# longkaimao/Sentinel

Hardware: AMD Instinct MI355X
Metric: flow decisions/sec (node) at 1M flowIds, 1/2/4/8 GPU; HBM GB/s vs peak (higher is better)
Workload: dtype int64; 1 GPU; C3 cluster token server: ClusterFlowChecker, FLOW_THRESHOLD_GLOBAL, S=10/1000 ms; flow_ids=1000000, flow_ids_per_gpu=1000000, parallelism=hash-sharded flowIds x1, rollup=none (1 GPU), namespace_limiter=off

## Files before the change

__graft_entry__.py:

```python
import os
import subprocess
import sys

ROOT = os.path.dirname(os.path.abspath(__file__))


def build() -> None:
    env = dict(os.environ)
    jobs = str(min(16, os.cpu_count() or 4))
    subprocess.check_call(["make", "-j", jobs, "-C", os.path.join(ROOT, "sentinel_amd", "csrc")], env=env)
    subprocess.check_call(["make", "-C", os.path.join(ROOT, "oracle")], env=env)
    subprocess.check_call(["make", "-C", os.path.join(ROOT, "tests", "cpp")], env=env)
    subprocess.check_call(["make", "-C", os.path.join(ROOT, "tests", "cpp"), "-f", "authority_host.mk"], env=env)
    subprocess.check_call(["make", "-C", os.path.join(ROOT, "tests", "cpp"), "-f", "system_host.mk"], env=env)
    subprocess.check_call(["make", "-C", os.path.join(ROOT, "tests", "cpp"), "-f", "blocklog_host.mk"], env=env)
    subprocess.check_call(["make", "-C", os.path.join(ROOT, "tests", "cpp"), "-f", "table_grow_host.mk"], env=env)
    if ROOT not in sys.path:
        sys.path.insert(0, ROOT)
    import sentinel_amd
    from sentinel_amd.engine import load_library
    load_library()


def smoke() -> None:
    if ROOT not in sys.path:
        sys.path.insert(0, ROOT)
    import numpy as np
    import torch

    from oracle.binding import ClusterTokenService
    from sentinel_amd import abi
    from sentinel_amd.engine import FlowEngine
    from sentinel_amd.workload import ClusterWorkload

    assert torch.cuda.is_available(), "smoke() needs a GPU"
    wl = ClusterWorkload(n_flows=2000, n_requests=50_000, seed=21)
    rules, req = wl.rules(), wl.requests(0)
    ns = np.zeros(1, abi.NS_DTYPE)
    ns["connected_count"] = 1
    ns["max_allowed_qps"] = 30000

    eng = FlowEngine(device=0, max_batch=len(req))
    eng.set_namespaces(ns)
    eng.load_rules(rules)
    dev = torch.device("cuda:0")
    req_t = torch.from_numpy(req.view(np.uint8).copy()).to(dev)
    out_t = torch.empty(len(req) * abi.RES_DTYPE.itemsize, dtype=torch.uint8, device=dev)
    eng.decide_device(req_t.data_ptr(), len(req), out_t.data_ptr(), torch.cuda.current_stream().cuda_stream)
    got = out_t.cpu().numpy().view(abi.RES_DTYPE)

    ora = ClusterTokenService()
    ora.set_namespaces(ns)
    ora.load_rules(rules)
    want = ora.decide(req)
    assert np.array_equal(got, want), f"{int((got != want).sum())} decisions differ from the oracle"
    print(f"smoke ok: {len(req)} decisions, {int((got['status'] == abi.OK).sum())} OK, "
          f"{int((got['status'] == abi.BLOCKED).sum())} BLOCKED, {int((got['status'] == abi.SHOULD_WAIT).sum())} WAIT")


if __name__ == "__main__":
    build()
    if len(sys.argv) > 1 and sys.argv[1] == "smoke":
        smoke()
```

sentinel_amd/csrc/api.cpp:

```cpp
#include <hip/hip_runtime.h>

#include <algorithm>
#include <functional>
#include <climits>
#include <cmath>
#include <cstdio>
#include <cstdlib>
#include <cstring>
#include <string>
#include <unordered_map>
#include <thread>
#include <tuple>
#include <vector>

#include "devmem.h"
#include "engine.h"
#include "table_grow.h"

using namespace sg;

bool sg::DevAlloc::alloc(void** p, size_t bytes) { return hipMalloc(p, bytes) == hipSuccess; }
void sg::DevAlloc::free(void* p) { (void)hipFree(p); }
bool sg::PinnedAlloc::alloc(void** p, size_t bytes) { return hipHostMalloc(p, bytes) == hipSuccess; }
void sg::PinnedAlloc::free(void* p) { (void)hipHostFree(p); }
using Stream = UniqueHandle<hipStream_t, hipError_t, hipStreamDestroy>;
using Event = UniqueHandle<hipEvent_t, hipError_t, hipEventDestroy>;

struct Staging {
    DevBuf<uint8_t> slot[4];
    template <class T>
    bool get(int i, uint64_t n, T*& p) {
        if (!slot[i].reserve(n * sizeof(T))) return false;
        p = reinterpret_cast<T*>(slot[i].get());
        return true;
    }
};

constexpr int kAsyncSlots = 3;
constexpr int kDevSlots = 4;

struct sg_handle {
    ~sg_handle();
    int device = 0;
    sg_config cfg{};
    std::string err;

    std::vector<sg_namespace> ns;
    std::vector<sg_flow_rule> rules;
    std::vector<Rule> rule_tab;
    uint32_t K = 0;
    int stride = 0;
    int n_wl = 0;
    int32_t wl[kMaxWl]{};

    DevBuf<Rule> d_rules;
    DevBuf<Bucket> d_ring;
    DevBuf<BucketHot> d_hot;
    DevBuf<Occ> d_occ;
    DevBuf<uint32_t> d_hot_key;
    uint64_t hot_gen = ~0ull;
    uint64_t rules_gen = 0;
    int bin_mode = 1;
    int prep_tiles = 4;

    struct FlowWs {
        DevBuf<uint64_t> rec;
        DevBuf<uint64_t> rec_sorted;
        DevBuf<uint32_t> hist;
        DevBuf<uint32_t> bnd;
        DevBuf<int64_t> p0;
        DevBuf<uint32_t> np;
        DevBuf<int> err;
        DevBuf<uint32_t> long_list;
        DevBuf<uint32_t> long_key;
        DevBuf<uint32_t> long_end;
        DevBuf<uint32_t> long_pend;
        DevBuf<uint32_t> short_list;
        DevBuf<uint32_t> short_key;
        DevBuf<uint32_t> short_end;
        DevBuf<uint32_t> counts;
        DevBuf<uint4> skips;
        DevBuf<uint32_t> skip_count;
        DevBuf<uint32_t> seg_end;
        uint32_t seg_cap = 0;
        uint32_t* seg_start = nullptr;
        DevBuf<uint64_t> bin_buf;
    };
    FlowWs ws[2];
    uint64_t* last_sorted = nullptr;
    uint64_t last_rec4_n = 0;
    DevBuf<int64_t> d_last_ts;
    int64_t* d_front_ts = nullptr;
    DevBuf<FidSlot> d_fid;
    uint64_t fid_mask = 0;
    uint64_t class_off[kClasses]{};
    DevBuf<unsigned long long> d_dbg;
    PinnedBuf<int> h_err;
    PinnedBuf<uint32_t> h_long;

    Staging stage;

    std::vector<int> ns_slot;
    int n_lim = 0;
    double lim_qps[kMaxLim]{};
    int lim_wl_idx = -1;
    DevBuf<LimRing> d_lim_ring;
    DevBuf<uint8_t> d_rule_lim;
    DevBuf<uint8_t> d_lim_slot;
    DevBuf<uint32_t> d_lim_tile;
    DevBuf<uint32_t> d_lim_period;

    std::vector<sg_param_rule> prules;
    std::vector<PRule> ptab;
    DevBuf<PRule> d_prules;
    DevBuf<sg_param_hot_item> d_phot;
    DevBuf<PSlot> d_ptable;
    uint64_t ptotal = 0;
    DevBuf<int64_t> d_plast_ts;

    std::vector<PaceRule> pace_tab;
    DevBuf<PaceRule> d_pace_rules;
    DevBuf<int64_t> d_pace_latest;
    DevBuf<int64_t> d_pace_last_ts;

    std::vector<sg_cparam_rule> cprules;
    std::vector<CPRule> cptab;
    DevBuf<CPRule> d_cprules;
    DevBuf<sg_param_hot_item> d_cphot;
    DevBuf<uint64_t> d_cpkeys;
    DevBuf<CPBucket> d_cpring;
    uint64_t cptotal = 0;
    int cpstride = 1;
    DevBuf<int64_t> d_cplast_ts;
    DevBuf<uint32_t> d_cp_owner;
    DevBuf<uint32_t> d_cp_pslot;
    DevBuf<uint32_t> d_cp_long;
    DevBuf<uint32_t> d_cp_short;
    uint64_t cp_class_off[kClasses]{};
    DevBuf<uint32_t> d_p_msb;
    DevBuf<int64_t> d_p_mt;
    DevBuf<uint16_t> d_p_mbk;
// ... 248 lines not shown
    if (e != hipSuccess) return bad(SG_E_DEVICE, std::string("hipSetDevice: ") + hipGetErrorString(e));
    Req* d_req = nullptr;
    Out* d_out = nullptr;
    if (!o->stage.get(0, o->cfg.max_batch, d_req) || !o->stage.get(1, o->cfg.max_batch, d_out))
        return bad(SG_E_NOMEM, "host-path buffers");
    e = hipMemcpy(d_req, req, sizeof(Req) * n, hipMemcpyHostToDevice);
    if (e != hipSuccess) return bad(SG_E_DEVICE, std::string("host-path upload: ") + hipGetErrorString(e));
    const int rc = call(d_req, d_out);
    if (rc) return rc;
    e = hipMemcpy(out, d_out, sizeof(Out) * n, hipMemcpyDeviceToHost);
    if (e != hipSuccess) return bad(SG_E_DEVICE, std::string("host-path download: ") + hipGetErrorString(e));
    return SG_OK;
}

int bits_for(uint64_t v) {
    int b = 0;
    while (b < 64 && (v >> b) != 0) ++b;
    return b;
}

double global_threshold(const sg_handle* h, const sg_flow_rule& r) {
    double base;
    if (r.threshold_type == SG_THRESHOLD_GLOBAL) {
        base = r.count;
    } else {
        int connected = 0;
        if (r.namespace_id >= 0 && (size_t)r.namespace_id < h->ns.size()) connected = h->ns[r.namespace_id].connected_count;
        base = r.count * connected;
    }
    return base * h->cfg.exceed_count;
}

int64_t java_math_round(double a) {
    int64_t bits;
    std::memcpy(&bits, &a, 8);
    const int64_t biased_exp = (bits & 0x7FF0000000000000LL) >> 52;
    const int64_t shift = (52 - 1 + 1023) - biased_exp;
    if ((shift & -64) == 0) {
        int64_t r = (bits & 0x000FFFFFFFFFFFFFLL) | 0x0010000000000000LL;
        if (bits < 0) r = -r;
        return ((r >> shift) + 1) >> 1;
    }
    if (a != a) return 0;
    if (a >= 9223372036854775807.0) return INT64_MAX;
    if (a <= -9223372036854775808.0) return INT64_MIN;
    return (int64_t)a;
}


int layout_records(sg_handle* h) {
    h->kbits = bits_for((uint64_t)h->K);
    if (h->kbits < 1) h->kbits = 1;
    h->ibits = bits_for(h->cfg.max_batch > 1 ? h->cfg.max_batch - 1 : 1);
    h->abits = std::min(8, 64 - h->kbits - h->ibits);
    if (h->abits < 3) return fail(h, SG_E_UNSUPPORTED, "rule count x max_batch too large for 64-bit records");
    return SG_OK;
}

int rebuild_wl_table(sg_handle* h) {
    int n_wl = 0;
    int32_t wl[kMaxWl]{};
    auto index_of = [&](int32_t v) -> int {
        for (int w = 0; w < n_wl; ++w)
            if (wl[w] == v) return w;
        if (n_wl == kMaxWl) return -1;
        wl[n_wl] = v;
        return n_wl++;
    };
    for (uint32_t k = 0; k < h->K; ++k) {
        const int w = index_of(h->rule_tab[k].wl);
        if (w < 0) return fail(h, SG_E_UNSUPPORTED, "more than 8 distinct window lengths");
        h->rule_tab[k].wl_idx = w;
    }
    h->lim_wl_idx = -1;
    if (h->n_lim > 0) {
        h->lim_wl_idx = index_of(kLimWindowMs);
        if (h->lim_wl_idx < 0) return fail(h, SG_E_UNSUPPORTED, "more than 8 distinct window lengths");
    }
    h->n_wl = n_wl;
    std::memcpy(h->wl, wl, sizeof(wl));
    return SG_OK;
}

int upload_rule_table(sg_handle* h) {
    h->l_groups_stale = true;
    h->ps_groups_stale = true;
    int rc = rebuild_wl_table(h);
    if (rc) return rc;
    const double ratio = h->cfg.max_occupy_ratio > 0 ? h->cfg.max_occupy_ratio : 0.0;
    for (uint32_t k = 0; k < h->K; ++k) {
        Rule& R = h->rule_tab[k];
        R.thr = global_threshold(h, h->rules[k]);
        const double bound = (R.thr > 0 ? R.thr : 0.0) * (2.0 + R.isec) * (2.0 + ratio);
        if (!(bound < 1073741824.0)) h->wide_seen = true;
    }
    if (h->K) HIP_TRY(h, hipMemcpy(h->d_rules, h->rule_tab.data(), sizeof(Rule) * h->K, hipMemcpyHostToDevice));
    h->d_rule_lim.reset();
    if (h->K) {
        std::vector<uint8_t> rl(h->K, 0xFF);
        for (uint32_t k = 0; k < h->K; ++k) {
            const int ns = h->rules[k].namespace_id;
            if (ns >= 0 && (size_t)ns < h->ns_slot.size() && h->ns_slot[ns] >= 0) rl[k] = (uint8_t)h->ns_slot[ns];
        }
        if (!h->d_rule_lim.alloc_bytes(h->K)) return fail(h, SG_E_NOMEM, "rule limiter table");
        HIP_TRY(h, hipMemcpy(h->d_rule_lim, rl.data(), h->K, hipMemcpyHostToDevice));
    }
    return SG_OK;
}

bool flow_ws_alloc(sg_handle* h, sg_handle::FlowWs& w) {
    const uint64_t n = h->cfg.max_batch;
    const uint64_t short_words = h->class_off[kClasses - 1] + n / (kClassMax[kClasses - 2] + 1) + 1;
    return w.rec.alloc(n + kRecW) && w.rec_sorted.alloc(n + kRecW) && w.hist.alloc(radix_hist_words(n)) &&
           w.bnd.alloc((size_t)kMaxWl * kMaxPeriods) && w.p0.alloc(kMaxWl) && w.np.alloc(kMaxWl) && w.err.alloc(1) &&
           w.long_list.alloc(n + 1) && w.long_key.alloc(n + 1) && w.long_end.alloc(n + 1) &&
           w.long_pend.alloc((size_t)kLongTab * kLongPeriods) && w.short_list.alloc(short_words) &&
           w.short_key.alloc(short_words) && w.short_end.alloc(short_words) && w.counts.alloc(1 + kClasses) &&
           w.skips.alloc(2 * n / kSkipMin + 1) && w.skip_count.alloc(1);
}

int flow_seg_alloc(sg_handle* h, DevBuf<uint32_t>& seg, uint32_t K) {
    const size_t cap = (size_t)K + 1;
    if (!seg.alloc(2 * cap)) return fail(h, SG_E_NOMEM, "segment marks");
    HIP_TRY(h, hipMemset(seg, 0, sizeof(uint32_t) * cap));
    HIP_TRY(h, hipMemset(seg + cap, 0xFF, sizeof(uint32_t) * cap));
    return SG_OK;
}

}

extern "C" {

const char* sg_build_info(void) {
    return "sentinel_gpu: cluster flow-decision engine, HIP for gfx950 (MI355X)";
}

int sg_create(const sg_config* cfg, sg_handle** out) {
    if (!cfg || !out) return SG_E_INVAL;
    *out = nullptr;
    if (cfg->max_batch == 0 || cfg->max_batch > (1ull << 32)) return SG_E_INVAL;
    if (!(cfg->exceed_count >= 0) || !(cfg->max_occupy_ratio >= 0)) return SG_E_INVAL;
    sg_handle* h = new sg_handle();
    h->cfg = *cfg;
    h->device = cfg->device;
    auto bail = [&](int rc) {
        delete h;
        return rc;
    };
    if (hipSetDevice(h->device) != hipSuccess) return bail(SG_E_DEVICE);
    const uint64_t n = cfg->max_batch;
    {
        uint64_t off = 0;
        for (int c = 0; c < kClasses; ++c) {
            h->class_off[c] = off;
            off += (c == 0 ? n : n / (kClassMax[c - 1] + 1)) + 1;
        }
    }
    if (!flow_ws_alloc(h, h->ws[0])) return bail(SG_E_NOMEM);
    {
        const uint64_t tiles = n / 4096 + 1;
        if (!h->d_lim_ring.alloc(kMaxLim) || !h->d_lim_slot.alloc(n) || !h->d_lim_tile.alloc(tiles * kMaxLim * 2) ||
            !h->d_lim_period.alloc((size_t)kMaxLim * kMaxPeriods * 3))
            return bail(SG_E_NOMEM);
    }
    if (!h->d_last_ts.alloc(2)) return bail(SG_E_NOMEM);
    if (!h->d_dbg.alloc(128) || hipMemset(h->d_dbg, 0, 128 * 8) != hipSuccess) return bail(SG_E_NOMEM);
    if (!h->h_err.alloc_bytes(sizeof(int))) return bail(SG_E_NOMEM);
    if (!h->h_long.alloc_bytes(2 * sizeof(uint32_t))) return bail(SG_E_NOMEM);
    int64_t neg = -1;
    if (hipMemcpy(h->d_last_ts, &neg, sizeof(neg), hipMemcpyHostToDevice) != hipSuccess) return bail(SG_E_DEVICE);
    h->d_front_ts = h->d_last_ts + 1;
    if (hipMemcpy(h->d_front_ts, &neg, sizeof(neg), hipMemcpyHostToDevice) != hipSuccess) return bail(SG_E_DEVICE);
    if (!h->d_plast_ts.alloc_bytes(sizeof(int64_t))) return bail(SG_E_NOMEM);
    if (hipMemcpy(h->d_plast_ts, &neg, sizeof(neg), hipMemcpyHostToDevice) != hipSuccess) return bail(SG_E_DEVICE);
    for (auto& e : h->ev)
        if (hipEventCreate(e.put()) != hipSuccess) return bail(SG_E_DEVICE);
    if (hipStreamCreateWithPriority(h->aux.put(), hipStreamNonBlocking, 0) != hipSuccess ||
        hipEventCreateWithFlags(h->fork.put(), hipEventDisableTiming) != hipSuccess ||
        hipEventCreateWithFlags(h->join.put(), hipEventDisableTiming) != hipSuccess)
// ... 112 lines not shown
    }
    if (want > kMaxLim) return fail(h, SG_E_UNSUPPORTED, "more than 8 namespaces with a QPS limiter");
    h->conc_dirty = true;
    for (const auto& r : h->rules)
        if (r.namespace_id < 0 || (uint32_t)r.namespace_id >= n)
            return fail(h, SG_E_INVAL, "a loaded rule refers to a namespace that would disappear");
    HIP_TRY(h, hipSetDevice(h->device));
    drain_async(h);
    LimRing old[kMaxLim], nw[kMaxLim];
    if (h->n_lim) HIP_TRY(h, hipMemcpy(old, h->d_lim_ring, sizeof(LimRing) * kMaxLim, hipMemcpyDeviceToHost));
    std::vector<int> slot(n, -1);
    int n_lim = 0;
    for (uint32_t i = 0; i < n; ++i) {
        if (!ns[i].limiter_enabled) continue;
        const int s_new = n_lim++;
        slot[i] = s_new;
        h->lim_qps[s_new] = ns[i].max_allowed_qps;
        const int s_old = (i < h->ns_slot.size()) ? h->ns_slot[i] : -1;
        if (s_old >= 0) {
            nw[s_new] = old[s_old];
        } else {
            for (int j = 0; j < kLimSamples; ++j) {
                nw[s_new].start[j] = INT64_MIN;
                nw[s_new].count[j] = 0;
            }
        }
    }
    if (n_lim) HIP_TRY(h, hipMemcpy(h->d_lim_ring, nw, sizeof(LimRing) * n_lim, hipMemcpyHostToDevice));
    h->ns.assign(ns, ns + n);
    h->ns_slot = slot;
    h->n_lim = n_lim;
    if (!h->cptab.empty()) {
        for (size_t i = 0; i < h->cptab.size(); ++i) {
            const int nsi = h->cprules[i].namespace_id;
            h->cptab[i].connected = (nsi >= 0 && (uint32_t)nsi < n) ? ns[nsi].connected_count : 0;
        }
        HIP_TRY(h, hipMemcpy(h->d_cprules, h->cptab.data(), sizeof(CPRule) * h->cptab.size(), hipMemcpyHostToDevice));
    }
    return upload_rule_table(h);
}

namespace {

int flow_rules_validate(sg_handle* h, const sg_flow_rule* rules, uint32_t n) {
    if (n >= SG_KEY_BAD) return fail(h, SG_E_INVAL, "too many rules");
    std::unordered_map<int64_t, uint32_t> seen, old_index;
    for (uint32_t k = 0; k < h->K; ++k) old_index.emplace(h->rules[k].flow_id, k);
    std::vector<int32_t> wls;
    for (uint32_t i = 0; i < n; ++i) {
        const sg_flow_rule& r = rules[i];
        if (r.flow_id <= 0) return fail(h, SG_E_INVAL, "flowId must be > 0");
        if (!(r.count >= 0)) return fail(h, SG_E_INVAL, "count must be >= 0");
        if (r.sample_count <= 0 || r.window_interval_ms <= 0 || r.window_interval_ms % r.sample_count != 0)
            return fail(h, SG_E_INVAL, "invalid window config");
        if (r.namespace_id < 0 || (size_t)r.namespace_id >= h->ns.size())
            return fail(h, SG_E_INVAL, "unknown namespace");
        if (!seen.emplace(r.flow_id, i).second) return fail(h, SG_E_INVAL, "duplicate flowId");
        int S = r.sample_count, wl = r.window_interval_ms / r.sample_count;
        auto it = old_index.find(r.flow_id);
        if (it != old_index.end()) {
            S = h->rule_tab[it->second].S;
            wl = h->rule_tab[it->second].wl;
        }
        if (S > SG_MAX_SAMPLE_COUNT) return fail(h, SG_E_UNSUPPORTED, "sampleCount > 64 is not supported by the device path");
        if (std::find(wls.begin(), wls.end(), wl) == wls.end()) wls.push_back(wl);
    }
    if (h->n_lim > 0 && std::find(wls.begin(), wls.end(), (int32_t)kLimWindowMs) == wls.end()) wls.push_back(kLimWindowMs);
    if (wls.size() > (size_t)kMaxWl) return fail(h, SG_E_UNSUPPORTED, "more than 8 distinct window lengths");
    return SG_OK;
}

}

namespace {

struct FlowLoad {
    std::vector<Rule> tab;
    std::vector<int32_t> src;
    int stride = 1;
    int n_wl = 0;
    int32_t wl[kMaxWl]{};
    DevBuf<Rule> d_rules;
    DevBuf<Bucket> d_ring;
    DevBuf<BucketHot> d_hot;
    DevBuf<Occ> d_occ;
    DevBuf<uint32_t> d_seg_end;
};

void flow_rules_abort(FlowLoad& L) { L = FlowLoad{}; }

int flow_rules_prepare_impl(sg_handle* h, const sg_flow_rule* rules, uint32_t n, FlowLoad& L) {
    std::unordered_map<int64_t, uint32_t> old_index;
    for (uint32_t k = 0; k < h->K; ++k) old_index.emplace(h->rules[k].flow_id, k);

    L.tab.assign(n, Rule{});
    L.src.assign(n, -1);
    std::vector<Rule>& tab = L.tab;
    std::vector<int32_t>& src = L.src;
    int& stride = L.stride;
    int& n_wl = L.n_wl;
    int32_t* wl = L.wl;
    for (uint32_t i = 0; i < n; ++i) {
        int S = rules[i].sample_count, interval = rules[i].window_interval_ms;
        auto it = old_index.find(rules[i].flow_id);
        if (it != old_index.end()) {
            src[i] = (int32_t)it->second;
            S = h->rule_tab[it->second].S;
            interval = h->rule_tab[it->second].S * h->rule_tab[it->second].wl;
        }
        if (S > SG_MAX_SAMPLE_COUNT)
            return fail(h, SG_E_UNSUPPORTED, "sampleCount > 64 is not supported by the device path");
        Rule R{};
        R.S = S;
        R.wl = interval / S;
        R.isec = interval / 1000.0;
        R.wait_ms = 1000 / S;
        int w = 0;
        while (w < n_wl && wl[w] != R.wl) ++w;
        if (w == n_wl) {
            if (n_wl == kMaxWl) return fail(h, SG_E_UNSUPPORTED, "more than 8 distinct window lengths");
            wl[n_wl++] = R.wl;
        }
        R.wl_idx = w;
        stride = std::max(stride, S);
        tab[i] = R;
    }

    if (n && h->front_only) {
        if (!L.d_rules.alloc(n)) return fail(h, SG_E_NOMEM, "rule table");
    } else if (n) {
        DevBuf<int32_t> d_src;
        if (!L.d_rules.alloc(n) || !L.d_ring.alloc((size_t)n * stride) || !L.d_hot.alloc((size_t)n * stride) ||
            !L.d_occ.alloc(n) || !d_src.alloc(n))
            return fail(h, SG_E_NOMEM, "rule state allocation failed");
        const int rc = flow_seg_alloc(h, L.d_seg_end, n);
        if (rc) return rc;
        HIP_TRY(h, hipMemcpy(d_src, src.data(), sizeof(int32_t) * n, hipMemcpyHostToDevice));
        HIP_TRY(h, launch_init_state(L.d_ring, L.d_occ, n, stride, d_src, h->d_ring, h->d_occ, h->stride, 0));
        HIP_TRY(h, launch_hot_sync(L.d_ring, L.d_hot, (uint64_t)n * stride, 0));
        HIP_TRY(h, hipDeviceSynchronize());
    }
    return SG_OK;
}

int flow_rules_prepare(sg_handle* h, const sg_flow_rule* rules, uint32_t n, FlowLoad& L) {
    const int rc = flow_rules_prepare_impl(h, rules, n, L);
    if (rc) flow_rules_abort(L);
    return rc;
}

int flow_rules_commit(sg_handle* h, const sg_flow_rule* rules, uint32_t n, FlowLoad& L) {
    std::vector<int32_t>& src = L.src;
    if (h->d_cnow) {
        std::vector<int32_t> old(h->K, 0);
        if (h->cnow_pending) {
            for (uint32_t k = 0; k < h->K && k < h->cnow_host.size(); ++k) old[k] = h->cnow_host[k];
        } else if (h->K) {
            HIP_TRY(h, hipMemcpy(old.data(), h->d_cnow, sizeof(int32_t) * h->K, hipMemcpyDeviceToHost));
        }
        h->cnow_host.assign(n, 0);
        for (uint32_t i = 0; i < n; ++i)
            if (src[i] >= 0) h->cnow_host[i] = old[src[i]];
        h->cnow_pending = true;
    }
    h->c_off.assign(n, 2000);
    h->c_res.assign(n, 2000);
    h->conc_dirty = true;
    h->d_rules = std::move(L.d_rules);
    h->d_ring = std::move(L.d_ring);
    h->d_hot = std::move(L.d_hot);
    h->d_occ = std::move(L.d_occ);
    sg_handle::FlowWs& w = h->ws[0];
    w.seg_end = std::move(L.d_seg_end);
    w.seg_cap = w.seg_end ? n + 1 : 0;
    w.seg_start = w.seg_end ? w.seg_end + w.seg_cap : nullptr;
    h->rules.assign(rules, rules + n);
    h->rule_tab = L.tab;
    h->K = n;
    ++h->rules_gen;
    h->stride = L.stride;
    h->n_wl = L.n_wl;
    std::memcpy(h->wl, L.wl, sizeof(L.wl));
    int rc = layout_records(h);
    if (rc) return rc;
    rc = upload_fid_table(h);
    if (rc) return rc;
    return upload_rule_table(h);
}

}

int sg_load_flow_rules(sg_handle* h, const sg_flow_rule* rules, uint32_t n) {
    if (h) drain_async(h);
    if (!h || (!rules && n)) return SG_E_INVAL;
    (void)hipSetDevice(h->device);
    const int vrc = flow_rules_validate(h, rules, n);
    if (vrc) return vrc;
    FlowLoad L;
    const int rc = flow_rules_prepare(h, rules, n, L);
    if (rc) return rc;
    return flow_rules_commit(h, rules, n, L);
}

static uint64_t host_fid_hash(int64_t fid) {
    uint64_t z = (uint64_t)fid + 0x9E3779B97F4A7C15ull;
    z = (z ^ (z >> 30)) * 0xBF58476D1CE4E5B9ull;
    z = (z ^ (z >> 27)) * 0x94D049BB133111EBull;
    return z ^ (z >> 31);
}

static int upload_fid_table(sg_handle* h) {
    uint64_t cap = 2;
    while (cap < 2ull * h->K) cap <<= 1;
    std::vector<FidSlot> tab(cap, FidSlot{0, 0, 0});
    for (uint32_t k = 0; k < h->K; ++k) {
        const int64_t fid = h->rules[k].flow_id;
        uint64_t p = host_fid_hash(fid) & (cap - 1);
        while (tab[p].fid != 0) p = (p + 1) & (cap - 1);
        tab[p] = FidSlot{fid, k, 0};
    }
    DevBuf<FidSlot> d;
    if (!d.alloc(cap)) return fail(h, SG_E_NOMEM, "flowId table");
    if (hipMemcpy(d, tab.data(), sizeof(FidSlot) * cap, hipMemcpyHostToDevice) != hipSuccess)
        return fail(h, SG_E_DEVICE, "flowId table upload");
    h->d_fid = std::move(d);
    h->fid_mask = cap - 1;
    return SG_OK;
}

int sg_codec_decode_flow(sg_handle* h, const uint8_t* payload, const uint32_t* offsets, const int64_t* ts_ms,
                         uint64_t n, sg_req* req_out, int32_t* xid_out, uint8_t* kind_out, void* stream) {
    if (!h) return SG_E_INVAL;
    if (n == 0) return SG_OK;
    if (!payload || !offsets || !ts_ms || !req_out || !xid_out || !kind_out) return fail(h, SG_E_INVAL, "null buffer");
    if (((uintptr_t)payload & 3u) != 0) return fail(h, SG_E_INVAL, "payload must be 4-byte aligned");
    if (!h->d_fid) {
        int rc = upload_fid_table(h);
        if (rc) return rc;
    }
    HIP_TRY(h, hipSetDevice(h->device));
    CodecArgs c{};
    c.n = n;
    c.payload = payload;
    c.offsets = offsets;
    c.ts = ts_ms;
    c.req = req_out;
    c.xid = xid_out;
    c.kind = kind_out;
    c.fid_tab = h->d_fid;
    c.fid_mask = h->fid_mask;
    HIP_TRY(h, launch_codec_decode(c, (hipStream_t)stream));
    return SG_OK;
}

// ... 335 lines not shown
}

int local_status(sg_handle* h, int err) {
    if (err & kErrTime)
        return fail(h, SG_E_TIME, "timestamps must be >= 0, non-decreasing, and not older than earlier batches");
    if (err & kErrPeriods) return fail(h, SG_E_UNSUPPORTED, "batch spans more than 65536 window periods");
    if (err & kErrBounds)
        return fail(h, SG_E_INVAL, "an event's origin id (0..n_origins), context id (0..n_contexts-1) or arguments "
                                   "(the arg / value arrays) are out of range");
    if (err & kErrTableFull) return fail(h, SG_E_CAPACITY, "a param value or thread-count table is full");
    if (err & kErrInternal) return fail(h, SG_E_DEVICE, "internal walker error");
    return SG_OK;
}

int ticket_status(sg_handle* h, const sg_handle::DevTicket& d) {
    if (!d.local) return flow_status(h, *d.h_err);
    const int rc = local_status(h, *d.h_err);
    if (rc != SG_OK && h->l_batches > 0) --h->l_batches;
    return rc;
}

int pipe_setup(sg_handle* h) {
    auto& w = h->ws[1];
    if (!w.rec) {
        if (!flow_ws_alloc(h, w)) return fail(h, SG_E_NOMEM, "pipeline workspace");
        int cus = 0;
        (void)hipDeviceGetAttribute(&cus, hipDeviceAttributeMultiprocessorCount, h->device);
        const int k16 = h->front_sixteenths;
        if (k16 > 0 && k16 < 16 && cus >= 8) {
            std::vector<uint32_t> fm((cus + 31) / 32, 0u), bm((cus + 31) / 32, 0u);
            int nb = 0;
            for (int i = 0; i < cus; ++i) {
                if (2 * (i % 8) + (i / 8) % 2 < k16) fm[i / 32] |= 1u << (i % 32);
                else {
                    bm[i / 32] |= 1u << (i % 32);
                    ++nb;
                }
            }
            HIP_TRY(h, hipExtStreamCreateWithCUMask(h->s_front.put(), (uint32_t)fm.size(), fm.data()));
            HIP_TRY(h, hipExtStreamCreateWithCUMask(h->s_back.put(), (uint32_t)bm.size(), bm.data()));
            HIP_TRY(h, hipExtStreamCreateWithCUMask(h->s_aux2.put(), (uint32_t)bm.size(), bm.data()));
            h->walk_cus = nb;
        } else {
            HIP_TRY(h, hipStreamCreateWithFlags(h->s_front.put(), hipStreamNonBlocking));
            HIP_TRY(h, hipStreamCreateWithFlags(h->s_back.put(), hipStreamNonBlocking));
            HIP_TRY(h, hipStreamCreateWithFlags(h->s_aux2.put(), hipStreamNonBlocking));
        }
        for (int x = 0; x < 2; ++x) {
            HIP_TRY(h, hipEventCreateWithFlags(h->front_done[x].put(), hipEventDisableTiming));
            HIP_TRY(h, hipEventCreateWithFlags(h->back_done[x].put(), hipEventDisableTiming));
        }
        HIP_TRY(h, hipEventCreateWithFlags(h->pfork.put(), hipEventDisableTiming));
        HIP_TRY(h, hipEventCreateWithFlags(h->pjoin.put(), hipEventDisableTiming));
    }
    if (w.seg_cap < h->K) {
        w.seg_cap = 0;
        w.seg_start = nullptr;
        const int rc = flow_seg_alloc(h, w.seg_end, h->K);
        if (rc) return rc;
        w.seg_cap = h->K + 1;
    }
    w.seg_start = w.seg_end + w.seg_cap;
    return SG_OK;
}

BatchArgs flow_args(sg_handle* h, const sg_handle::FlowWs& w, const sg_req* req, uint64_t n, sg_result* out) {
    BatchArgs a{};
    a.req = req;
    a.out = out;
    a.n = n;
    a.rec = w.rec;
    a.rec_sorted = w.rec_sorted;
    a.hist0 = h->n_lim > 0 ? nullptr : w.hist;
    a.hist0_bits = radix_digit_bits(h->kbits);
    a.kshift = 64 - h->kbits;
    a.hist0_shift = a.kshift;
    a.abits = h->abits;
    a.imask = (h->ibits >= 64) ? ~0ull : ((1ull << h->ibits) - 1);
    a.amask = (1ull << h->abits) - 1;
    a.aesc = (1ull << (h->abits - 1)) - 1;
    a.K = h->K;
    a.rules = h->d_rules;
    a.ring = h->d_ring;
    a.hot = h->d_hot;
    a.occ = h->d_occ;
    a.seg_end = w.seg_end;
    a.seg_start = w.seg_start;
    a.short_end = w.short_end;
    a.stride = h->stride;
    a.max_occ_ratio = h->cfg.max_occupy_ratio;
    a.n_wl = h->n_wl;
    std::memcpy(a.wl, h->wl, sizeof(a.wl));
    a.bnd = w.bnd;
    a.p0 = w.p0;
    a.np = w.np;
    a.err = w.err;
    a.last_ts = h->d_last_ts;
    a.check_last = 1;
    a.walk_cus = 0;
    a.long_list = w.long_list;
    a.long_count = w.counts;
    a.short_list = w.short_list;
    a.short_key = w.short_key;
    a.long_key = w.long_key;
    a.long_end = w.long_end;
    a.long_pend = w.long_pend;
    a.short_count = w.counts + 1;
    for (int c = 0; c < kClasses; ++c) a.class_off[c] = h->class_off[c];
    a.skips = w.skips;
    a.skip_count = w.skip_count;
    a.dbg = h->dbg;
    a.generic_walker = (h->cfg.flags & SG_FLAG_RING_REREAD) != 0;
    a.narrow = h->wide_seen ? 0 : 1;
    a.dbg_ctr = h->d_dbg;
    a.skip_cap = (uint32_t)(2 * h->cfg.max_batch / kSkipMin + 1);
    a.short_max = (h->cfg.flags & SG_FLAG_WAVE_ONLY) ? 0u
                  : (h->cfg.flags & SG_FLAG_SERIAL_ONLY) ? 0xFFFFFFFFu : h->short_max;
    return a;
}

int flow_limiter(sg_handle* h, BatchArgs& a, hipStream_t stream) {
    if (h->n_lim > 0) {
        LimArgs L{};
        L.n_lim = h->n_lim;
        L.wl_idx = h->lim_wl_idx;
        std::memcpy(L.qps, h->lim_qps, sizeof(L.qps));
        L.rule_lim = h->d_rule_lim;
        L.slot = h->d_lim_slot;
        const uint64_t tiles = a.n / 4096 + 1;
        L.tile_tot = h->d_lim_tile;
        L.tile_off = h->d_lim_tile + tiles * kMaxLim;
        L.arrivals = h->d_lim_period;
        L.prefix = h->d_lim_period + (size_t)kMaxLim * kMaxPeriods;
        L.quota = h->d_lim_period + (size_t)2 * kMaxLim * kMaxPeriods;
        L.ring = h->d_lim_ring;
        if (h->lim_x_armed) {
            L.xg = h->lim_xg;
            L.ts = &a.req[0].ts_ms;
            L.ts_stride = sizeof(sg_req) / sizeof(int64_t);
            L.t_base = h->lim_xt;
            L.n_ms = h->lim_xn;
            L.world = h->shard_world;
            L.rank = h->shard_rank;
        }
        HIP_TRY(h, launch_limiter(a, L, stream));
    }
    return SG_OK;
}

bool bin_setup(sg_handle* h, sg_handle::FlowWs& w, BatchArgs& a, hipStream_t stream) {
    if (h->bin_mode == 0 || h->n_lim > 0 || !a.hist0 || a.n == 0 || h->K == 0) return false;
    if (h->bin_mode == 1 && h->K < (1u << 14)) return false;
    if (64 - h->kbits - h->ibits - h->abits < kBinDigit) return false;
    const int kb = h->K > 1 ? bits_for((uint64_t)h->K - 1) : 1;
    const int bsh = std::max(0, kb - 9);
    if (bsh > kBinMaxBsh || (((h->K - 1) >> bsh) + 1) > kBinRegular) return false;
    if (!h->d_hot_key) {
        if (!h->d_hot_key.alloc_bytes(sizeof(uint32_t) * (kBinHot + 1) + sizeof(uint2) * kHotTab))
            return false;
        h->hot_gen = ~0ull;
    }
    uint2* tab = reinterpret_cast<uint2*>(h->d_hot_key + kBinHot + 1);
    if (!w.bin_buf) {
        if (!w.bin_buf.alloc(h->cfg.max_batch + kRecW)) return false;
    }
    if (h->hot_gen != h->rules_gen) {
        if (launch_hot_reset(tab, stream) != hipSuccess) return false;
        h->hot_gen = h->rules_gen;
// ... 381 lines not shown

int sg_rls_should_rate_limit(sg_handle* h, const sg_rls_request* req, uint32_t n, const int32_t* desc_rule,
                             uint64_t n_desc, int32_t* overall, sg_rls_status* status) {
    if (!h) return SG_E_INVAL;
    if (n && (!req || !overall)) return fail(h, SG_E_INVAL, "null buffer");
    if (n_desc && (!desc_rule || !status)) return fail(h, SG_E_INVAL, "null buffer");
    for (uint32_t j = 0; j < n; ++j)
        if ((uint64_t)req[j].desc_begin + req[j].desc_count > n_desc)
            return fail(h, SG_E_INVAL, "a request's descriptors lie outside desc_rule");
    uint64_t n_tok = 0;
    for (uint32_t j = 0; j < n; ++j) {
        if (req[j].hits_addend < 0) continue;
        n_tok += req[j].desc_count;
        for (uint32_t x = 0; x < req[j].desc_count; ++x) {
            const int32_t r = desc_rule[(uint64_t)req[j].desc_begin + x];
            if (r < 0 || (uint32_t)r >= h->K) continue;
            const sg_flow_rule& fr = h->rules[r];
            const int ns = fr.namespace_id;
            if (fr.threshold_type != SG_THRESHOLD_GLOBAL ||
                (ns >= 0 && (size_t)ns < h->ns_slot.size() && h->ns_slot[ns] >= 0))
                return fail(h, SG_E_UNSUPPORTED, "RLS rules are loaded GLOBAL in namespaces without a limiter "
                                                 "(SimpleClusterFlowChecker reads count * exceedCount only)");
        }
    }
    if (n_tok > h->cfg.max_batch) return fail(h, SG_E_CAPACITY, "more descriptors than max_batch");
    std::vector<sg_req> batch;
    std::vector<uint64_t> owner;
    batch.reserve(n_desc);
    owner.reserve(n_desc);
    for (uint64_t d = 0; d < n_desc; ++d) status[d] = sg_rls_status{0, 0, 0, 0};
    for (uint32_t j = 0; j < n; ++j) {
        const sg_rls_request& q = req[j];
        if (q.hits_addend < 0) {
            overall[j] = SG_RLS_ERROR;
            continue;
        }
        overall[j] = SG_RLS_OK;
        const int32_t acquire = q.hits_addend == 0 ? 1 : q.hits_addend;
        for (uint32_t x = 0; x < q.desc_count; ++x) {
            const uint64_t d = (uint64_t)q.desc_begin + x;
            const int32_t r = desc_rule[d];
            sg_req t{};
            t.ts_ms = q.ts_ms;
            t.key = (r < 0 || (uint32_t)r >= h->K) ? SG_KEY_NO_RULE : (uint32_t)r;
            t.acquire = acquire;
            batch.push_back(t);
            owner.push_back(d);
        }
    }
    std::vector<sg_result> res(batch.size());
    if (!batch.empty()) {
        const int rc = sg_flow_decide_batch_host(h, batch.data(), batch.size(), res.data());
        if (rc) return rc;
    }
    for (uint64_t x = 0; x < batch.size(); ++x) {
        const uint64_t d = owner[x];
        int32_t st = res[x].status;
        if (st == SG_STATUS_NO_RULE_EXISTS) st = SG_STATUS_OK;
        sg_rls_status& o = status[d];
        o.code = st == SG_STATUS_OK ? SG_RLS_OK : SG_RLS_OVER_LIMIT;
        if (batch[x].key != SG_KEY_NO_RULE) {
            const double c = h->rules[batch[x].key].count;
            o.requests_per_unit = c >= 2147483647.0 ? INT32_MAX : (int32_t)c;
            o.limit_remaining = res[x].remaining;
            o.has_rule = 1;
        }
    }
    for (uint32_t j = 0; j < n; ++j) {
        if (overall[j] == SG_RLS_ERROR) continue;
        for (uint32_t x = 0; x < req[j].desc_count; ++x)
            if (status[(uint64_t)req[j].desc_begin + x].code != SG_RLS_OK) overall[j] = SG_RLS_OVER_LIMIT;
    }
    return SG_OK;
}

int sg_flow_read_state(sg_handle* h, uint32_t key, int64_t* starts, int64_t* counters, int64_t* occupy) {
    if (!h || key >= h->K || !starts || !counters || !occupy) return SG_E_INVAL;
    HIP_TRY(h, hipSetDevice(h->device));
    drain_async(h);
    const int S = h->rule_tab[key].S;
    std::vector<Bucket> b(S);
    HIP_TRY(h, hipMemcpy(b.data(), h->d_ring + (size_t)key * h->stride, sizeof(Bucket) * S, hipMemcpyDeviceToHost));
    Occ o;
    HIP_TRY(h, hipMemcpy(&o, h->d_occ + key, sizeof(Occ), hipMemcpyDeviceToHost));
    for (int j = 0; j < S; ++j) {
        starts[j] = b[j].start;
        for (int e = 0; e < SG_NUM_EVENTS; ++e) counters[j * SG_NUM_EVENTS + e] = b[j].start == INT64_MIN ? 0 : b[j].c[e];
    }
    occupy[0] = o.pass;
    occupy[1] = o.pass_req;
    return SG_OK;
}

int sg_flow_export_state(sg_handle* h, int64_t* ring, uint64_t ring_words, int64_t* occ, uint64_t occ_words,
                         int32_t* stride) {
    if (!h || !stride) return SG_E_INVAL;
    *stride = h->stride;
    if (!ring) return SG_OK;
    const uint64_t rw = (uint64_t)h->K * h->stride * 8, ow = 2ull * h->K;
    if (ring_words < rw || !occ || occ_words < ow) return fail(h, SG_E_INVAL, "export buffers too small");
    if (h->K == 0) return SG_OK;
    HIP_TRY(h, hipSetDevice(h->device));
    drain_async(h);
    static_assert(sizeof(Bucket) == 64 && sizeof(Occ) == 16, "export layout");
    HIP_TRY(h, hipMemcpy(ring, h->d_ring, rw * 8, hipMemcpyDeviceToHost));
    HIP_TRY(h, hipMemcpy(occ, h->d_occ, ow * 8, hipMemcpyDeviceToHost));
    return SG_OK;
}

int sg_flow_import_state(sg_handle* h, const int64_t* ring, uint64_t ring_words, const int64_t* occ,
                         uint64_t occ_words) {
    if (!h || !ring || !occ) return SG_E_INVAL;
    const uint64_t rw = (uint64_t)h->K * h->stride * 8, ow = 2ull * h->K;
    if (ring_words != rw || occ_words != ow) return fail(h, SG_E_INVAL, "import size does not match the loaded rules");
    if (h->K == 0) return SG_OK;
    HIP_TRY(h, hipSetDevice(h->device));
    drain_async(h);
    HIP_TRY(h, hipMemcpy(h->d_ring, ring, rw * 8, hipMemcpyHostToDevice));
    HIP_TRY(h, launch_hot_sync(h->d_ring, h->d_hot, (uint64_t)h->K * h->stride, 0));
    HIP_TRY(h, hipDeviceSynchronize());
    HIP_TRY(h, hipMemcpy(h->d_occ, occ, ow * 8, hipMemcpyHostToDevice));
    return SG_OK;
}

int sg_snapshot_metrics(sg_handle* h, int64_t now_ms, double* out, uint64_t cap) {
    if (!h || !out || cap < 2ull * h->K) return SG_E_INVAL;
    if (h->K == 0) return SG_OK;
    HIP_TRY(h, hipSetDevice(h->device));
    drain_async(h);
    DevBuf<double> d_out;
    if (!d_out.alloc(2 * (size_t)h->K)) return fail(h, SG_E_DEVICE, "snapshot buffer: out of memory");
    hipError_t e1 = launch_snapshot(h->d_rules, h->d_ring, h->d_occ, h->K, h->stride, now_ms, d_out, 0);
    hipError_t e2 = e1 == hipSuccess ? hipMemcpy(out, d_out, sizeof(double) * 2 * h->K, hipMemcpyDeviceToHost) : e1;
    if (e2 != hipSuccess) return fail(h, SG_E_DEVICE, hipGetErrorString(e2));
    return SG_OK;
}

int sg_snapshot_metrics_device(sg_handle* h, int64_t now_ms, double* out_dev, uint64_t cap, void* stream) {
    if (!h || !out_dev || cap < 2ull * h->K) return SG_E_INVAL;
    if (h->K == 0) return SG_OK;
    HIP_TRY(h, hipSetDevice(h->device));
    drain_async(h);
    HIP_TRY(h, launch_snapshot(h->d_rules, h->d_ring, h->d_occ, h->K, h->stride, now_ms, out_dev, (hipStream_t)stream));
    return SG_OK;
}

int sg_snapshot_metrics_enqueue(sg_handle* h, int64_t now_ms, double* out_dev, uint64_t cap, uint64_t* ticket) {
    if (!h || !out_dev || !ticket || cap < 2ull * h->K) return SG_E_INVAL;
    *ticket = 0;
    if (h->K == 0) return SG_OK;
    HIP_TRY(h, hipSetDevice(h->device));
    int rc = pipe_setup(h);
    if (rc) return rc;
    sg_handle::DevTicket& d = h->dev[h->next_ticket % kDevSlots];
    if (!d.done) {
        if (!d.h_err.alloc_bytes(sizeof(int))) return fail(h, SG_E_NOMEM, "pinned error word");
        HIP_TRY(h, hipEventCreateWithFlags(d.done.put(), hipEventDisableTiming));
    }
    if (d.ticket) {
        hipError_t e = hipEventSynchronize(d.done);
        h->finished[d.ticket] = e != hipSuccess ? fail(h, SG_E_DEVICE, hipGetErrorString(e)) : ticket_status(h, d);
        d.ticket = 0;
    }
    *d.h_err = 0;
    HIP_TRY(h, launch_snapshot(h->d_rules, h->d_ring, h->d_occ, h->K, h->stride, now_ms, out_dev, h->s_back));
    HIP_TRY(h, hipEventRecord(d.done, h->s_back));
    d.local = false;
    d.ticket = h->next_ticket++;
    *ticket = d.ticket;
    return SG_OK;
}

static int param_release_claims(sg_handle* h, hipStream_t stream) {
    if (!h->ptotal || h->ptab.empty()) return SG_OK;
    DevBuf<PSlot> old;
    if (!old.alloc(h->ptotal)) return SG_OK;
    HIP_TRY(h, hipMemcpyAsync(old, h->d_ptable, sizeof(PSlot) * h->ptotal, hipMemcpyDeviceToDevice, stream));
    HIP_TRY(h, launch_param_rebuild(h->d_prules, (uint32_t)h->ptab.size(), h->d_ptable, old, h->ptotal, stream));
    HIP_TRY(h, hipStreamSynchronize(stream));
    return SG_OK;
}

int sg_param_load_rules(sg_handle* h, const sg_param_rule* rules, uint32_t n, const sg_param_hot_item* hot,
                        uint32_t n_hot) {
    if (!h || (!rules && n) || (!hot && n_hot)) return SG_E_INVAL;
    HIP_TRY(h, hipSetDevice(h->device));
    std::vector<PRule> tab(n);
    std::vector<sg_param_hot_item> hot_sorted(hot, hot + n_hot);
    uint64_t base = 0;
    for (uint32_t i = 0; i < n; ++i) {
        const sg_param_rule& r = rules[i];
        if (!(r.count >= 0) || r.duration_sec <= 0) return fail(h, SG_E_INVAL, "invalid param rule");
        if ((uint64_t)r.hot_begin + r.hot_count > n_hot) return fail(h, SG_E_INVAL, "hot item range out of bounds");
        const int lg = r.capacity_log2 ? r.capacity_log2 : 20;
        if (lg < 1 || lg > 30) return fail(h, SG_E_INVAL, "capacity_log2 must be in [1, 30]");
        PRule& R = tab[i];
        R.token_count = (int64_t)r.count;
        if (r.count >= 9.2e18) R.token_count = INT64_MAX;
        R.duration_sec = r.duration_sec;
        R.burst = r.burst;
        R.behavior = r.behavior;
        R.max_queueing_ms = r.max_queueing_ms;
        R.hot_begin = r.hot_begin;
        R.hot_count = r.hot_count;
        R.table_base = base;
        R.table_mask = (1ull << lg) - 1;
        base += (1ull << lg) + 1;
        std::sort(hot_sorted.begin() + r.hot_begin, hot_sorted.begin() + r.hot_begin + r.hot_count,
                  [](const sg_param_hot_item& x, const sg_param_hot_item& y) { return x.value < y.value; });
    }
    if (base >= (1ull << 32)) return fail(h, SG_E_UNSUPPORTED, "param tables larger than 2^32 slots");
    h->d_prules.reset();
    h->d_phot.reset();
    h->d_ptable.reset();
    h->ptotal = 0;
    if (n) {
        if (!h->d_prules.alloc_bytes(sizeof(PRule) * n) ||
            !h->d_ptable.alloc_bytes(sizeof(PSlot) * base))
            return fail(h, SG_E_NOMEM, "param table allocation");
        if (n_hot && !h->d_phot.alloc_bytes(sizeof(sg_param_hot_item) * n_hot))
            return fail(h, SG_E_NOMEM, "param hot items");
        HIP_TRY(h, hipMemcpy(h->d_prules, tab.data(), sizeof(PRule) * n, hipMemcpyHostToDevice));
        if (n_hot)
            HIP_TRY(h, hipMemcpy(h->d_phot, hot_sorted.data(), sizeof(sg_param_hot_item) * n_hot, hipMemcpyHostToDevice));
        HIP_TRY(h, launch_param_clear(h->d_ptable, base, 0));
        HIP_TRY(h, hipDeviceSynchronize());
    }
    h->prules.assign(rules, rules + n);
    h->ptab = tab;
    h->ptotal = base;
    return SG_OK;
}

int sg_param_decide_batch(sg_handle* h, const sg_param_req* req, uint64_t n, int32_t* pass, void* stream_) {
    if (!h) return SG_E_INVAL;
    if (n == 0) return SG_OK;
    if (!req || !pass) return fail(h, SG_E_INVAL, "null buffer");
    if (n > h->cfg.max_batch) return fail(h, SG_E_CAPACITY, "batch larger than max_batch");
    hipStream_t stream = (hipStream_t)stream_;
    HIP_TRY(h, hipSetDevice(h->device));
    drain_async(h);
    PArgs p{};
    p.req = req;
    p.out = pass;
    p.n = n;
    p.rec = h->ws[0].rec;
    p.rec_sorted = h->ws[0].rec_sorted;
    p.ibits = bits_for(h->cfg.max_batch > 1 ? h->cfg.max_batch - 1 : 1);
// ... 1244 lines not shown
            return fail(h, SG_E_NOMEM, "local batch workspace");
    }
    return SG_OK;
}

BlogArgs blog_args(sg_handle* h) {
    BlogArgs b{};
    b.tab = h->d_blog;
    b.mask = h->d_blog.size() - 1;
    b.lost = h->d_blog_ctr;
    return b;
}

int local_args(sg_handle* h, const LocalBufs& b, const sg_local_event* ev, const sg_slot_ext* ext, uint64_t n,
               const sg_pslot_arg* args, uint64_t n_args, const uint64_t* values, uint64_t n_values, sg_local_result* out,
               bool emb, LArgs& L, BatchArgs& sgm) {
    const uint32_t K = (uint32_t)h->ltab.size();
    int kbits = bits_for((uint64_t)K);
    if (kbits < 1) kbits = 1;
    const int ibits = bits_for(h->cfg.max_batch > 1 ? h->cfg.max_batch - 1 : 1);
    const int abits = 64 - kbits - ibits;
    if (abits < 4) return fail(h, SG_E_UNSUPPORTED, "resources x max_batch too large for 64-bit records");

    L = LArgs{};
    L.ev = ev;
    L.out = out;
    L.cxw = h->l_cxw;
    L.cxw_cls = kClasses;
    for (int c = kClasses - 1; c >= 0 && (c == 0 ? 1u : kClassMax[c - 1] + 1u) >= h->l_cxw_min; --c) L.cxw_cls = c;
    L.n = n;
    L.rec = b.rec;
    L.rec_sorted = b.rec_sorted;
    L.kshift = 64 - kbits;
    L.abits = abits;
    L.imask = (ibits >= 64) ? ~0ull : ((1ull << ibits) - 1);
    L.amask = (1ull << abits) - 1;
    L.aesc = (1ull << (abits - 3)) - 1;
    L.K = K;
    L.N = h->l_nodes;
    L.rules = h->d_lrules;
    L.frules = h->d_lfrules;
    L.ctl = h->d_lctl;
    L.n_origins = h->l_n_origins;
    L.head = h->d_lhead;
    L.sec = h->d_lsec;
    L.bor = h->d_lbor;
    L.minute = h->d_lmin;
    L.S = h->lcfg.sample_count;
    L.wl2 = h->lcfg.interval_ms / h->lcfg.sample_count;
    L.interval = h->lcfg.interval_ms;
    L.isec = h->lcfg.interval_ms / 1000.0;
    L.occupy_timeout = h->lcfg.occupy_timeout_ms;
    L.wsec = h->l_wsec;
    L.wmin = h->l_wmin;
    L.n_wl = h->l_n_wl;
    std::memcpy(L.wl, h->l_wl, sizeof(L.wl));
    L.bnd = b.bnd;
    L.p0 = b.p0;
    L.np = b.np;
    L.err = b.err;
    L.last_ts = h->d_llast_ts;
    L.ext = ext;
    L.n_contexts = h->l_n_contexts;
    L.gkey = h->d_lgkey;
    L.has_ps = h->ps_loaded ? 1 : 0;
    if (h->ps_loaded) {
        L.ps = pslot_args(h);
        L.ps.args = args;
        L.ps.n_args = args ? n_args : 0;
        L.ps.values = values;
        L.ps.n_values = values ? n_values : 0;
        const int prc = pslot_embed(h, L.ps, 0);
        if (prc) return prc;
        if (h->l_cxw) {
            if (!b.lw->pslot && !b.lw->pslot.alloc_bytes(sizeof(uint64_t) * h->cfg.max_batch))
                return fail(h, SG_E_NOMEM, "param lookups of the local batch");
            L.pslot = b.lw->pslot;
        }
    }
    if (emb) {
        L.emb = 1;
        L.c3_rules = h->d_rules;
        L.c3_ring = h->d_ring;
        L.c3_hot = h->d_hot;
        L.c3_occ = h->d_occ;
        L.c3_stride = h->stride;
        L.c3_K = h->K;
        L.max_occ_ratio = h->cfg.max_occupy_ratio;
        L.c3_rule_lim = h->d_rule_lim;
        L.lim_ring = h->d_lim_ring;
        for (int j = 0; j < kMaxLim; ++j) L.lim_qps[j] = h->lim_qps[j];
        L.c3_last_ts = h->d_last_ts;
    }
    if (h->d_lauth && h->l_n_origins > 0) {
        if (!b.lw->auth_rej && !b.lw->auth_rej.alloc_bytes(h->cfg.max_batch))
            return fail(h, SG_E_NOMEM, "authority verdicts of the local batch");
        L.auth = h->d_lauth;
        L.auth_ids = h->d_lauth_ids;
        L.auth_rej = b.lw->auth_rej;
    }
    if (h->d_blog) {
        L.blog_app = h->d_blog_app;
        L.res_app = h->d_lres_app;
    }
    L.flags = b.lw->flags;
    L.cxw_next = b.lw->cxw_next;
    if (h->l_cxw && (h->l_has_cx || h->l_has_cx_ps)) {
        if (!b.lw->cxside && !b.lw->cxside.alloc_bytes(sizeof(CxSide) * h->cfg.max_batch))
            return fail(h, SG_E_NOMEM, "side words of the local batch");
        L.cxside = b.lw->cxside;
    }
    if (h->l_has_cx || h->l_has_cx_ps || h->l_n_contexts > 0) {
        if (!b.lw->cx_list && !b.lw->cx_list.alloc_bytes(sizeof(uint32_t) * (h->cfg.max_batch + 1)))
            return fail(h, SG_E_NOMEM, "cx segment list of the local batch");
        L.cx_list = b.lw->cx_list;
        L.cx_count = b.lw->cx_list + h->cfg.max_batch;
    }
    L.exit_pos = b.lw->exit_pos;
    L.exit_cnt = b.lw->exit_cnt;
    L.skips = b.lw->skips;
    L.skip_count = b.lw->skip_count;
    L.skip_cap = (uint32_t)b.lw->skips.size();
    L.hist0 = b.hist;
    L.hist0_bits = radix_digit_bits(64 - L.kshift);

    sgm = BatchArgs{};
    sgm.dbg = h->dbg;
    sgm.dbg_ctr = h->d_dbg;
    sgm.n = n;
    sgm.rec_sorted = b.rec_sorted;
    sgm.kshift = L.kshift;
    sgm.K = K;
    sgm.err = b.err;
    sgm.long_list = b.long_list;
    sgm.long_count = b.counts;
    sgm.short_list = b.short_list;
    sgm.short_count = b.counts + 1;
    for (int c = 0; c < kClasses; ++c) sgm.class_off[c] = h->class_off[c];
    const uint32_t lsplit = (!h->short_max_env && (uint64_t)n >= 256ull * K) ? 64u : h->short_max;
    sgm.short_max = (h->cfg.flags & SG_FLAG_WAVE_ONLY) ? 0u : (h->cfg.flags & SG_FLAG_SERIAL_ONLY) ? 0xFFFFFFFFu : lsplit;

    return SG_OK;
}

int local_front(sg_handle* h, LArgs& L, BatchArgs& sgm, hipStream_t stream) {
    HIP_TRY(h, hipMemsetAsync(L.err, 0, sizeof(int), stream));
    HIP_TRY(h, hipMemsetAsync(sgm.long_count, 0, (1 + kClasses) * sizeof(uint32_t), stream));
    HIP_TRY(h, hipMemsetAsync(L.flags, 0, sizeof(int), stream));
    HIP_TRY(h, hipMemsetAsync(L.skip_count, 0, sizeof(uint32_t), stream));
    L.csum0 = nullptr;
    if (radix_csum_atomic()) {
        L.csum0 = radix_csum(L.hist0, L.n, L.hist0_bits);
        HIP_TRY(h, hipMemsetAsync(L.csum0, 0, radix_csum_bytes(L.n, L.hist0_bits), stream));
    }
    HIP_TRY(h, launch_local_prep(L, stream));
    return SG_OK;
}

int local_sort(sg_handle* h, LArgs& L, BatchArgs& sgm, uint64_t* spare, hipStream_t stream, bool count_exits = false) {
    uint64_t* sorted = nullptr;
    HIP_TRY(h, radix_sort_records(L.rec, spare, L.n, L.kshift, L.hist0, &sorted, stream, 64, true,
                                  L.csum0 != nullptr));
    L.rec_sorted = sorted;
    sgm.rec_sorted = sorted;
    if (count_exits) {
        HIP_TRY(h, hipMemsetAsync(L.exit_cnt, 0, sizeof(uint32_t) * (L.n / kLTile + 2), stream));
        sgm.exit_cnt = L.exit_cnt;
        sgm.exit_amask = L.amask;
// ... 1419 lines not shown
    std::vector<DevBuf<uint32_t>> d_node_key;
    DevBuf<double> d_snap;
    bool node_key_stale = true;
    bool l_loaded = false;
    sg_local_config l_cfg{};
    std::vector<sg_local_rule> l_rules;
    std::vector<sg_local_flow_rule> l_frules;
    bool l_has_frules = false;
    std::vector<sg_authority_rule> l_arules;
    std::vector<int32_t> l_aorigins;
    int32_t l_n_origins = 0, l_n_contexts = 0;
    std::vector<uint32_t> l_owner;
    DevBuf<uint8_t> d_l_owner;
    int64_t l_last_ts = -1;
    uint64_t l_batches = 0;
    DevBuf<sg_local_event> d_lsub_ev;
    DevBuf<sg_local_result> d_lsub_out;
    DevBuf<int> d_lerr;
    bool l_ps_loaded = false;
    std::vector<sg_pslot_rule> l_prules;
    std::vector<sg_param_hot_item> l_phot;
    bool compact_args = false;
    DevBuf<sg_slot_ext> d_lsub_ext;
    std::vector<DevBuf<sg_pslot_arg>> d_cargs;
    std::vector<DevBuf<uint64_t>> d_cvals;
    DevBuf<unsigned long long> d_ctsum;
    DevBuf<unsigned long long> d_ctot;
    DevBuf<unsigned long long> d_mbits;
    DevBuf<uint32_t> d_mpre;
    uint32_t m_words = 0;
    DevBuf<MergeSlots> d_mslots;
    DevBuf<sg_metric_node> d_mrows;
    DevBuf<sg_metric_node> d_mout;
};

namespace {

int nfail(sg_node* nd, int code, const std::string& msg) {
    if (nd) nd->err = msg;
    return code;
}

#define NHIP(nd, expr)                                                                          \
    do {                                                                                        \
        hipError_t _e = (expr);                                                                 \
        if (_e != hipSuccess)                                                                   \
            return nfail((nd), SG_E_DEVICE, std::string(#expr ": ") + hipGetErrorString(_e));   \
    } while (0)

uint32_t node_owner(int64_t flow_id, uint32_t G) {
    uint64_t z = (uint64_t)flow_id + 0x9E3779B97F4A7C15ull;
    z = (z ^ (z >> 30)) * 0xBF58476D1CE4E5B9ull;
    z = (z ^ (z >> 27)) * 0x94D049BB133111EBull;
    z ^= z >> 31;
    return (uint32_t)(z % G);
}

int node_child(sg_node* nd, sg_handle* h, int rc) {
    if (rc < 0) nd->err = h->err;
    return rc;
}

int node_sync_layout(sg_node* nd) {
    sg_handle* f = nd->front;
    int rc = ensure_layout(f);
    if (rc) return node_child(nd, f, rc);
    bool same = true;
    for (size_t g = 0; g < nd->shards.size(); ++g) {
        sg_handle* h = nd->shards[g];
        rc = ensure_layout(h);
        if (rc) return node_child(nd, h, rc);
        same = same && nd->devices[g] == nd->devices[0] && h->ibits == f->ibits && h->abits == f->abits;
        if (!h->K) continue;
        for (uint32_t k = 0; k < h->K; ++k) {
            Rule& R = h->rule_tab[k];
            int w = 0;
            while (w < f->n_wl && f->wl[w] != R.wl) ++w;
            if (w == f->n_wl) return nfail(nd, SG_E_DEVICE, "a shard window length missing at the front");
            R.wl_idx = w;
        }
        h->n_wl = f->n_wl;
        std::memcpy(h->wl, f->wl, sizeof(h->wl));
        NHIP(nd, hipSetDevice(h->device));
        NHIP(nd, hipMemcpy(h->d_rules, h->rule_tab.data(), sizeof(Rule) * h->K, hipMemcpyHostToDevice));
    }
    nd->rec_path = same && std::getenv("SG_NODE_LEGACY") == nullptr;
    if (nd->rec_path && !nd->d_sub_rec) {
        NHIP(nd, hipSetDevice(nd->devices[0]));
        if (!nd->d_sub_rec.alloc_bytes(sizeof(uint64_t) * (nd->cfg.max_batch + kRecW)))
            return nfail(nd, SG_E_NOMEM, "shard record slices");
    }
    return SG_OK;
}

int node_walk_cus(const sg_node* nd, uint32_t g, int cus) {
    int same = 0;
    for (int32_t d : nd->devices) same += d == nd->devices[g] ? 1 : 0;
    if (same <= 1) return cus;
    if (cus <= 0) {
        int all = 0;
        (void)hipDeviceGetAttribute(&all, hipDeviceAttributeMultiprocessorCount, nd->devices[g]);
        cus = all > 0 ? all : 256;
    }
    return std::max(1, cus / same);
}

void node_sync_shards(sg_node* nd, uint32_t g) {
    for (uint32_t x = 0; x < g && x < nd->sh.size(); ++x) {
        (void)hipSetDevice(nd->devices[x]);
        (void)hipStreamSynchronize(nd->sh[x].stream);
    }
    (void)hipSetDevice(nd->devices[0]);
}

int node_shard_rec(sg_handle* h, BatchArgs b, uint64_t cnt, uint32_t* hist, hipStream_t front, hipStream_t back,
                   hipStream_t aux, hipEvent_t fork, hipEvent_t join, hipEvent_t front_done, int* err_dst) {
    HIP_TRY(h, hipMemsetAsync(b.err, 0, sizeof(int), front));
    HIP_TRY(h, hipMemsetAsync(b.long_count, 0, (1 + kClasses) * sizeof(uint32_t), front));
    HIP_TRY(h, hipMemsetAsync(b.skip_count, 0, sizeof(uint32_t), front));
    uint64_t* sorted = nullptr;
    HIP_TRY(h, radix_sort_records(b.rec, b.rec_sorted, cnt, b.kshift, hist, &sorted, front, 64, b.hist0 != nullptr,
                                  b.csum0 != nullptr));
    b.rec_sorted = sorted;
    HIP_TRY(h, launch_seg_flow(b, front));
    if (front_done) {
        HIP_TRY(h, hipEventRecord(front_done, front));
        HIP_TRY(h, hipStreamWaitEvent(back, front_done, 0));
    }
    HIP_TRY(h, hipEventRecord(fork, back));
    HIP_TRY(h, hipStreamWaitEvent(aux, fork, 0));
    HIP_TRY(h, launch_walk_long(b, aux));
    HIP_TRY(h, launch_walk_short(b, back));
    HIP_TRY(h, hipEventRecord(join, aux));
    HIP_TRY(h, hipStreamWaitEvent(back, join, 0));
    HIP_TRY(h, launch_skip_apply(b, back));
    HIP_TRY(h, hipMemcpyAsync(err_dst, b.err, sizeof(int), hipMemcpyDeviceToHost, back));
    return SG_OK;
}

int node_slot_status(sg_node* nd, const sg_node::PipeSlot& sl) {
    for (uint32_t g = 0; g < sl.G_used; ++g)
        if (sl.h_err[g]) return node_child(nd, nd->shards[g], flow_status(nd->shards[g], sl.h_err[g]));
    return SG_OK;
}

int node_drain(sg_node* nd) {
    for (auto& sl : nd->pipe) {
        if (!sl.ticket) continue;
        (void)hipSetDevice(nd->devices[0]);
        const hipError_t e = hipEventSynchronize(sl.done);
        nd->finished[sl.ticket] = e != hipSuccess ? nfail(nd, SG_E_DEVICE, hipGetErrorString(e)) : node_slot_status(nd, sl);
        sl.ticket = 0;
    }
    for (sg_handle* h : nd->shards) drain_async(h);
    if (nd->front) drain_async(nd->front);
    if (!nd->devices.empty()) (void)hipSetDevice(nd->devices[0]);
    return SG_OK;
}

}

sg_node::~sg_node() {
    node_drain(this);
    for (size_t g = 0; g < shards.size(); ++g) sg_destroy(shards[g]);
    sh.clear();
    sg_destroy(front);
    (void)hipSetDevice(devices.empty() ? 0 : devices[0]);
// ... 462 lines not shown
    NHIP(nd, hipEventRecord(sl.done, nd->s0));
    sl.G_used = G;
    sl.ticket = t;
    nd->pseq++;
    return SG_OK;
}

static int node_collect(sg_node* nd, uint64_t ticket, bool block) {
    if (!nd) return SG_E_INVAL;
    if (ticket == 0) return 1;
    auto it = nd->finished.find(ticket);
    if (it != nd->finished.end()) {
        const int st = it->second;
        nd->finished.erase(it);
        return st == SG_OK ? 1 : st;
    }
    for (auto& sl : nd->pipe) {
        if (sl.ticket != ticket) continue;
        (void)hipSetDevice(nd->devices[0]);
        const hipError_t e = block ? hipEventSynchronize(sl.done) : hipEventQuery(sl.done);
        if (e == hipErrorNotReady) return 0;
        sl.ticket = 0;
        if (e != hipSuccess) return nfail(nd, SG_E_DEVICE, hipGetErrorString(e));
        const int st = node_slot_status(nd, sl);
        return st == SG_OK ? 1 : st;
    }
    return nfail(nd, SG_E_INVAL, "unknown or already collected ticket");
}

int sg_node_flow_poll(sg_node* nd, uint64_t ticket) { return node_collect(nd, ticket, false); }

int sg_node_flow_wait(sg_node* nd, uint64_t ticket) {
    const int r = node_collect(nd, ticket, true);
    return r == 1 ? SG_OK : r;
}

int sg_node_flow_read_state(sg_node* nd, uint32_t key, int64_t* starts, int64_t* counters, int64_t* occupy) {
    if (!nd || key >= nd->shard_of.size()) return SG_E_INVAL;
    node_drain(nd);
    sg_handle* h = nd->shards[nd->shard_of[key]];
    return node_child(nd, h, sg_flow_read_state(h, nd->local_of[key], starts, counters, occupy));
}

int sg_node_snapshot_metrics(sg_node* nd, int64_t now_ms, double* out, uint64_t cap) {
    if (!nd || (!out && cap)) return SG_E_INVAL;
    node_drain(nd);
    const uint64_t K = nd->shard_of.size();
    if (cap < 2 * K) return nfail(nd, SG_E_CAPACITY, "snapshot buffer smaller than 2 * rules");
    if (K == 0) return SG_OK;
    const uint32_t G = (uint32_t)nd->shards.size();
    NHIP(nd, hipSetDevice(nd->devices[0]));
    if (nd->node_key_stale || nd->d_node_key.size() != G) {
        nd->d_node_key.clear();
        nd->d_node_key.resize(G);
        std::vector<std::vector<uint32_t>> keys(G);
        for (uint64_t k = 0; k < K; ++k) {
            auto& v = keys[nd->shard_of[k]];
            if (v.size() <= nd->local_of[k]) v.resize(nd->local_of[k] + 1);
            v[nd->local_of[k]] = (uint32_t)k;
        }
        for (uint32_t g = 0; g < G; ++g) {
            if (keys[g].empty()) continue;
            if (!nd->d_node_key[g].alloc_bytes(sizeof(uint32_t) * keys[g].size()))
                return nfail(nd, SG_E_NOMEM, "node snapshot keys");
            NHIP(nd, hipMemcpy(nd->d_node_key[g], keys[g].data(), sizeof(uint32_t) * keys[g].size(), hipMemcpyHostToDevice));
        }
        nd->node_key_stale = false;
    }
    uint64_t part_max = 0;
    for (sg_handle* h : nd->shards) part_max = std::max<uint64_t>(part_max, h->K);
    const uint64_t need = 2 * K + 2 * part_max;
    if (!nd->d_snap.reserve(need)) return nfail(nd, SG_E_NOMEM, "node snapshot");
    double* stage = nd->d_snap + 2 * K;
    for (uint32_t g = 0; g < G; ++g) {
        sg_handle* h = nd->shards[g];
        if (h->K == 0) continue;
        const int dev = nd->devices[g];
        double* part = stage;
        if (dev != nd->devices[0]) {
            NHIP(nd, hipSetDevice(dev));
            if (!nd->sh[g].r_snap.reserve(2 * part_max)) return nfail(nd, SG_E_NOMEM, "node snapshot part");
            part = nd->sh[g].r_snap;
        }
        NHIP(nd, launch_snapshot(h->d_rules, h->d_ring, h->d_occ, h->K, h->stride, now_ms, part, nd->sh[g].stream));
        NHIP(nd, hipStreamSynchronize(nd->sh[g].stream));
        NHIP(nd, hipSetDevice(nd->devices[0]));
        if (dev != nd->devices[0])
            NHIP(nd, hipMemcpyPeerAsync(stage, nd->devices[0], part, dev, sizeof(double) * 2 * h->K, nd->s0));
        NHIP(nd, launch_nsnap_scatter(stage, nd->d_node_key[g], h->K, nd->d_snap, nd->s0));
        NHIP(nd, hipStreamSynchronize(nd->s0));
    }
    NHIP(nd, hipMemcpy(out, nd->d_snap, sizeof(double) * 2 * K, hipMemcpyDeviceToHost));
    return SG_OK;
}


int sg_node_cparam_load_rules(sg_node* nd, const sg_cparam_rule* rules, uint32_t n, const sg_param_hot_item* hot,
                              uint32_t n_hot, int32_t capacity_log2) {
    if (!nd || (!rules && n) || (!hot && n_hot)) return SG_E_INVAL;
    node_drain(nd);
    const uint32_t G = (uint32_t)nd->shards.size();
    for (uint32_t i = 0; i < n; ++i)
        if ((uint64_t)rules[i].hot_begin + rules[i].hot_count > n_hot) return nfail(nd, SG_E_INVAL, "hot item range out of bounds");
    std::vector<std::vector<sg_cparam_rule>> part(G);
    std::vector<std::vector<sg_param_hot_item>> hp(G);
    std::vector<uint8_t> so(n);
    std::vector<uint32_t> lo(n);
    for (uint32_t i = 0; i < n; ++i) {
        const uint32_t g = node_owner(rules[i].flow_id, G);
        so[i] = (uint8_t)g;
        lo[i] = (uint32_t)part[g].size();
        sg_cparam_rule r = rules[i];
        r.hot_begin = (uint32_t)hp[g].size();
        hp[g].insert(hp[g].end(), hot + rules[i].hot_begin, hot + rules[i].hot_begin + rules[i].hot_count);
        part[g].push_back(r);
    }
    for (uint32_t g = 0; g < G; ++g) {
        sg_handle* h = nd->shards[g];
        NHIP(nd, hipSetDevice(h->device));
        const int rc = sg_cparam_load_rules(h, part[g].data(), (uint32_t)part[g].size(), hp[g].data(),
                                            (uint32_t)hp[g].size(), capacity_log2);
        if (rc) return node_child(nd, h, rc);
    }
    NHIP(nd, hipSetDevice(nd->devices[0]));
    nd->d_cp_shard_of.reset();
    nd->d_cp_local_of.reset();
    if (n && (!nd->d_cp_shard_of.alloc_bytes(n) || !nd->d_cp_local_of.alloc_bytes(sizeof(uint32_t) * n)))
        return nfail(nd, SG_E_NOMEM, "param routing tables");
    if (n) {
        NHIP(nd, hipMemcpy(nd->d_cp_shard_of, so.data(), n, hipMemcpyHostToDevice));
        NHIP(nd, hipMemcpy(nd->d_cp_local_of, lo.data(), sizeof(uint32_t) * n, hipMemcpyHostToDevice));
    }
    nd->cp_rules.assign(rules, rules + n);
    nd->cp_shard_of = so;
    nd->cp_local_of = lo;
    return SG_OK;
}

}

namespace {

int node_nreq_scratch(sg_node* nd, uint64_t n_values) {
    const uint64_t n = nd->cfg.max_batch;
    NHIP(nd, hipSetDevice(nd->devices[0]));
    if (!nd->d_nrec) {
        if (!nd->d_nrec.alloc_bytes(8 * n) || !nd->d_nrec2.alloc_bytes(8 * n) ||
            !nd->d_nhist.alloc_bytes(sizeof(uint32_t) * radix_hist_words(n)) ||
            !nd->d_nvals.alloc_bytes(sizeof(uint32_t) * n) ||
            !nd->d_ncnt.alloc_bytes(sizeof(uint32_t) * 3 * kMaxShards) ||
            !nd->d_ntsum.alloc_bytes(sizeof(uint32_t) * (nreq_tiles(n) + 1)) ||
            !nd->d_nerr.alloc_bytes(sizeof(int)) ||
            !nd->d_sub_nreq.alloc_bytes(std::max(sizeof(sg_cparam_req), sizeof(sg_conc_req)) * n) ||
            !nd->d_sub_nout.alloc_bytes(std::max(sizeof(sg_result), sizeof(sg_conc_result)) * n))
            return nfail(nd, SG_E_NOMEM, "node token routing scratch");
    }
    if (!nd->d_sub_vals.reserve(n_values)) return nfail(nd, SG_E_NOMEM, "node param values");
    return SG_OK;
}

int node_nreq_route(sg_node* nd, NodeReqArgs q, std::vector<uint64_t>& base, std::vector<uint64_t>& cnt,
                    std::vector<uint64_t>& vbase, std::vector<uint64_t>& vcnt) {
    const uint32_t G = (uint32_t)nd->shards.size();
    hipStream_t st = nd->s0;
    q.G = (int)G;
    q.rec = nd->d_nrec;
    q.nvals = nd->d_nvals;
// ... 987 lines not shown
```

sentinel_amd/csrc/engine.h:

```cpp
#pragma once

#include <hip/hip_runtime.h>
#include <stddef.h>
#include <stdint.h>

#include "../../include/sentinel_gpu.h"
#include "authority_rules.h"
#include "blocklog_rules.h"
#include "system_rules.h"
#include "search_dev.h"

namespace sg {

struct alignas(16) Rule {
    double thr;
    double isec;
    int32_t S;
    int32_t wl;
    int32_t wl_idx;
    int32_t wait_ms;
};
static_assert(sizeof(Rule) == 32, "Rule layout");

struct alignas(64) Bucket {
    int64_t start;
    int64_t c[SG_NUM_EVENTS];
};
static_assert(sizeof(Bucket) == 64, "Bucket layout");

struct alignas(16) BucketHot {
    int64_t start;
    int32_t pass;
    int32_t wait;
};
static_assert(sizeof(BucketHot) == 16, "BucketHot layout");

__device__ __forceinline__ void store_hot(BucketHot* h, int64_t start, int64_t pass, int64_t wait) {
    BucketHot x;
    x.start = start;
    x.pass = (int32_t)pass;
    x.wait = (int32_t)wait;
    *h = x;
}

struct alignas(16) Occ {
    int64_t pass;
    int64_t pass_req;
};

#ifndef SG_SORT_ROUNDS
#define SG_SORT_ROUNDS 16
#endif
constexpr int kSortRounds = SG_SORT_ROUNDS;
constexpr int kMaxWl = 8;
constexpr uint32_t kMaxPeriods = 1u << 16;
constexpr int kShortMax = 256;
constexpr int kLdsBnd = 4096;
constexpr int kLdsBndFlow = 1024;
#ifndef SG_RECW
#define SG_RECW 32
#endif
constexpr int kRecW = SG_RECW;
constexpr int kClasses = 6;
constexpr uint32_t kClassMax[kClasses - 1] = {4, 16, 64, 256, 1024};

constexpr int kErrTime = 1;
constexpr int kErrPeriods = 2;
constexpr int kErrInternal = 16;
constexpr int kErrExchange = 64;

struct BatchArgs {
    const sg_req* req;
    sg_result* out;
    uint64_t n;
    uint64_t* rec;
    uint32_t* hist0;
    uint32_t* csum0;
    int hist0_bits;
    uint64_t* rec_sorted;
    int kshift;
    int abits;
    uint64_t imask;
    uint64_t amask;
    uint64_t aesc;
    uint32_t K;
    const Rule* rules;
    Bucket* ring;
    BucketHot* hot;
    Occ* occ;
    int stride;
    double max_occ_ratio;
    int n_wl;
    int32_t wl[kMaxWl];
    uint32_t* bnd;
    int64_t* p0;
    uint32_t* np;
    int* err;
    int64_t* last_ts;
    int check_last;
    int64_t* front_ts;
    int walk_cus;
    uint32_t* long_list;
    uint32_t* long_count;
    uint32_t* short_list;
    uint32_t* short_count;
    uint32_t* short_key;
    uint32_t* long_key;
    uint32_t* seg_end;
    uint32_t* seg_start;
    uint32_t* short_end;
    uint32_t* long_end;
    uint32_t* long_pend;
    uint64_t class_off[kClasses];
    uint32_t short_max;
    uint32_t* exit_cnt;
    uint64_t exit_amask;
    int dbg;
    int narrow;
    int generic_walker;
    unsigned long long* dbg_ctr;
    uint4* skips;
    uint32_t* skip_count;
    uint32_t skip_cap;
    int hist0_shift;
    int bin_on;
    int prep_tiles;
    int bin_dshift;
    int bin_bsh;
    uint32_t bin_R;
    uint2* hot_tab;
    uint32_t* hot_key;
    uint64_t* bin_buf;
    const uint32_t* bin_tot;
    int rec4;
};

constexpr int kBinDigit = 10;
constexpr uint32_t kBinRegular = 512;
constexpr uint32_t kBinHot = (1u << kBinDigit) - kBinRegular - 1;
constexpr uint32_t kBinDrop = (1u << kBinDigit) - 1;
constexpr int kBinMaxBsh = 11;
constexpr int kRec4Abits = 8;
constexpr int kRec4KeyShift = kRec4Abits;
constexpr int kRec4DigitShift = kRec4KeyShift + kBinMaxBsh;
static_assert(kRec4DigitShift + kBinDigit <= 32, "digit, key in bin and acquire code fit a 32-bit record");
static_assert(kBinHot + kBinRegular + 1 == (1u << kBinDigit), "hot slots, regular bins and kBinDrop fill the digit");
constexpr int kHotBucketBits = 9;
constexpr uint32_t kHotWays = 4;
constexpr uint32_t kHotTab = kHotWays << kHotBucketBits;
constexpr uint32_t kHotEmpty = 0xFFFFFFFFu;
__host__ __device__ __forceinline__ uint32_t hot_hash(uint32_t key) {
    return (key * 2654435761u) >> (32 - kHotBucketBits);
}

constexpr int kLongPeriods = 16;
constexpr uint32_t kLongTab = 65536;
constexpr uint32_t kSkipMin = 256;
constexpr uint32_t kSkipPiece = 4096;

constexpr int kMaxLim = 8;
constexpr int kLimSamples = 10;
constexpr int kLimWindowMs = 100;

struct LimRing {
    int64_t start[kLimSamples];
    int64_t count[kLimSamples];
};

static_assert(sizeof(sg_req) % sizeof(int64_t) == 0 && sizeof(sg_cparam_req) % sizeof(int64_t) == 0 &&
                  offsetof(sg_req, ts_ms) == 0 && offsetof(sg_cparam_req, ts_ms) == 0,
              "LimArgs::ts strides over the request records");
struct LimArgs {
    int n_lim;
    int wl_idx;
    double qps[kMaxLim];
    const uint8_t* rule_lim;
    uint8_t* slot;
    uint32_t* tile_tot;
    uint32_t* tile_off;
    uint32_t* arrivals;
    uint32_t* prefix;
    uint32_t* quota;
    LimRing* ring;
    const uint32_t* xg;
    const int64_t* ts;
    uint32_t ts_stride;
    int64_t t_base;
    uint32_t n_ms;
    int world, rank;
};

hipError_t launch_limiter(const BatchArgs& a, const LimArgs& L, hipStream_t stream);
hipError_t launch_limiter_plan_only(const BatchArgs& a, const LimArgs& L, hipStream_t stream);
hipError_t launch_lim_arrivals(const sg_req* req, uint64_t n, uint32_t K, const uint8_t* rule_lim, int64_t t_base,
                               uint32_t n_ms, uint32_t* counts, int* err, hipStream_t stream);
hipError_t launch_lim_arrivals_param(const sg_cparam_req* req, uint64_t n, uint32_t K, const uint8_t* rule_lim,
                                     int64_t t_base, uint32_t n_ms, uint32_t* counts, int* err, hipStream_t stream);

constexpr int kErrNonPositive = 4;
constexpr int kErrTableFull = 8;

struct PRule {
    int64_t token_count;
    int64_t duration_sec;
    int32_t burst;
    int32_t behavior;
    int32_t max_queueing_ms;
    uint32_t hot_begin, hot_count;
    uint32_t pad;
    uint64_t table_base;
    uint64_t table_mask;
};

struct alignas(16) CxSide {
    int64_t t;
    uint32_t psl;
    uint32_t node;
};
// ... 388 lines not shown
};

struct LSys {
    LSysConf conf;
    double load, cpu;
    int64_t threads;
    LBucket* sec;
    uint32_t unproven;
    uint32_t first_unproven;
    int64_t d_threads;
    unsigned long long* lastp;
    int64_t* acc;
};

struct LArgs {
    const sg_local_event* ev;
    sg_local_result* out;
    uint64_t n;
    uint64_t* rec;
    uint64_t* rec_sorted;
    uint32_t* hist0;
    uint32_t* csum0;
    int hist0_bits;
    int kshift, abits;
    uint64_t imask, amask, aesc;
    uint32_t K;
    uint32_t N;
    const LRule* rules;
    const LFlowRule* frules;
    LCtl* ctl;
    int32_t n_origins;
    LHead* head;
    LBucket* sec;
    LFuture* bor;
    LBucket* minute;
    int S;
    int32_t wl2;
    int32_t interval;
    double isec;
    int32_t occupy_timeout;
    int wsec, wmin;
    int n_wl;
    int32_t wl[kMaxWl];
    uint32_t* bnd;
    int64_t* p0;
    uint32_t* np;
    int* err;
    int64_t* last_ts;
    int32_t defer_last;
    const sg_slot_ext* ext;
    int32_t n_contexts;
    const uint32_t* gkey;
    PSArgs ps;
    int32_t has_ps;
    int* flags;
    uint32_t* exit_pos;
    uint32_t* exit_cnt;
    struct LSkip* skips;
    uint32_t* skip_count;
    uint32_t skip_cap;
    uint64_t* nkeys;
    uint32_t* nvals;
    uint64_t nmask;
    uint32_t node_base;
    uint32_t* node_new;
    uint2* ev_node;
    uint32_t* dyn;
    uint32_t epoch;
    int32_t track_ctx;
    int32_t cxw;
    int32_t cxw_cls;
    uint32_t* cxw_next;
    uint32_t* cx_list;
    uint32_t* cx_count;
    uint64_t* pslot;
    CxSide* cxside;
    const LAuth* auth;
    const int32_t* auth_ids;
    uint8_t* auth_rej;
    LSys* sys;
    int32_t emb;
    const Rule* c3_rules;
    Bucket* c3_ring;
    BucketHot* c3_hot;
    Occ* c3_occ;
    int c3_stride;
    uint32_t c3_K;
    double max_occ_ratio;
    const uint8_t* c3_rule_lim;
    LimRing* lim_ring;
    double lim_qps[kMaxLim];
    int64_t* c3_last_ts;
    int64_t* last_fetch;
    const uint8_t* inbound;
    LBucket* entry_acc;
    int64_t* entry_fetch;
    int32_t* blog_app;
    const int32_t* res_app;
};

constexpr uint64_t kPsUnknown = ~0ull;
constexpr uint64_t kPsNoCheck = ~0ull - 1;
constexpr uint64_t kPsEarlyFail = ~0ull - 2;
constexpr uint64_t kPsNoCheckInit = ~0ull - 3;
constexpr int kLFlagPrio = 1;
constexpr int kLFlagNonPos = 2;
constexpr uint32_t kLTile = 4096;

struct LSkip {
    uint32_t k, qs, qm, b0, b1, pad[3];
};

hipError_t launch_local_prep(const LArgs& L, hipStream_t stream);
hipError_t launch_local_walk(const LArgs& L, const BatchArgs& seg, bool has_cx, hipStream_t aux, hipStream_t stream,
                             hipEvent_t fork, hipEvent_t join);
hipError_t launch_local_exits(const LArgs& L, hipStream_t stream, bool counted);
hipError_t launch_local_back(const LArgs& L, const BatchArgs& seg, bool has_cx, hipStream_t aux, hipStream_t stream,
                             hipEvent_t fork, hipEvent_t join);
hipError_t launch_local_init(const LArgs& L, hipStream_t stream);
hipError_t launch_local_init_range(const LArgs& L, uint64_t lo, uint64_t hi, hipStream_t stream);
hipError_t launch_lnode_assign(const LArgs& L, hipStream_t stream);
hipError_t launch_lnode_find(const uint64_t* keys, const uint32_t* vals, uint64_t mask, uint64_t key, uint32_t* out,
                             hipStream_t stream);
hipError_t launch_entry_acc_reset(LBucket* acc, hipStream_t stream);
hipError_t launch_metrics_gate(const unsigned long long* cnt, uint64_t cap, unsigned long long* count_out, int* gate,
                               hipStream_t stream);
hipError_t launch_local_entry_rows(const LArgs& L, int64_t now, sg_metric_node* out, unsigned long long* count, int emit,
                                   int raw, hipStream_t stream, const int* gate = nullptr);
hipError_t launch_local_metrics(const LArgs& L, int64_t now, sg_metric_node* out, unsigned long long* count, int emit,
                                int raw, hipStream_t stream, const int* gate = nullptr);

constexpr uint64_t kBlogBusy = 1;
struct alignas(16) BlogSlot {
    uint64_t tag;
    int64_t ts;
    uint64_t app;
    uint64_t ro;
    uint32_t status, kind;
    int64_t count;
};
static_assert(sizeof(BlogSlot) == 48, "BlogSlot layout");
struct BlogArgs {
    BlogSlot* tab;
    uint64_t mask;
    unsigned long long* lost;
};
hipError_t launch_blog_add(const LArgs& L, const BlogArgs& b, hipStream_t stream);
hipError_t launch_blog_take(const BlogArgs& b, int64_t limit, int emit, sg_block_row* rows, sg_block_row* keep,
                            unsigned long long* count, unsigned long long* n_keep, hipStream_t stream);
hipError_t launch_blog_put(const BlogArgs& b, const sg_block_row* keep, const unsigned long long* n_keep,
                           hipStream_t stream);

struct SysArgs {
    const sg_local_event* ev;
    const sg_local_result* out;
    uint64_t n;
    uint32_t K;
    const uint8_t* inbound;
    const uint8_t* auth_rej;
    LSys* sys;
    int S;
    int32_t wl;
    double isec;
    int64_t* pb;
    const int* err;
};
hipError_t launch_sys_scan(const SysArgs& s, hipStream_t stream);
hipError_t launch_sys_apply(const SysArgs& s, hipStream_t stream);
// ... 77 lines not shown
    const sg_slot_ext* ext;
    sg_slot_ext* sub_ext;
    int32_t n_contexts;
    int32_t has_ps;
    const sg_pslot_arg* args;
    uint64_t n_args, n_values;
};
constexpr int kErrExt = 128;
hipError_t launch_lroute(const LRouteArgs& r, hipStream_t stream);
struct LCompactArgs {
    const sg_local_event* ev;
    sg_slot_ext* ext;
    uint64_t n;
    uint32_t K;
    const sg_pslot_arg* args;
    const uint64_t* values;
    sg_pslot_arg* out_args;
    uint64_t* out_vals;
    unsigned long long* tsum;
    unsigned long long* tot;
};
hipError_t launch_lcompact_count(const LCompactArgs& c, hipStream_t stream);
hipError_t launch_lcompact_gather(const LCompactArgs& c, hipStream_t stream);
uint64_t lcompact_tiles(uint64_t n);
hipError_t launch_route_gather8(const sg_local_result* sub_out, const uint32_t* sub_pos, uint64_t total,
                                sg_local_result* out, hipStream_t stream);
constexpr uint64_t kMergeNoTs = ~0ull;
constexpr int kMergeBad = 1;
constexpr int kMergeCap = 2;
struct MergeSlots {
    unsigned long long ts[kMinuteS];
    unsigned long long acc[kMinuteS][5];
    unsigned long long base[kMinuteS];
    uint32_t res_cnt[kMinuteS];
    uint32_t has_entry[kMinuteS];
    unsigned long long n_out;
    unsigned long long n_res;
    int err;
};
struct MergeArgs {
    const sg_metric_node* rows;
    uint64_t n;
    uint32_t K, W;
    unsigned long long* bits;
    uint32_t* pre;
    MergeSlots* st;
    sg_metric_node* out;
    uint64_t cap;
};
hipError_t launch_merge_rows(const MergeArgs& m, hipStream_t stream);
size_t radix_hist_words(uint64_t n);
int radix_digit_bits(int bits);
#ifndef SG_CHUNK_TILES
#define SG_CHUNK_TILES 32
#endif
constexpr uint32_t kChunkTiles = SG_CHUNK_TILES;
bool radix_csum_atomic();
uint32_t* radix_csum(uint32_t* hist_ws, uint64_t n, int D);
size_t radix_csum_bytes(uint64_t n, int D);
hipError_t radix_sort_records(uint64_t* a, uint64_t* b, uint64_t n, int lo_bit, uint32_t* hist_ws,
                              uint64_t** result, hipStream_t stream, int hi_bit = 64, bool first_hist_ready = false,
                              bool first_csum_ready = false);
const uint32_t* radix_tot(const uint32_t* hist_ws, uint64_t n, int D);
hipError_t radix_bin_pass(uint64_t* src, uint64_t* out, uint64_t* reg, uint32_t R, uint64_t n, int shift,
                          uint32_t* hist_ws, bool hist_ready, bool csum_ready, hipStream_t stream);
struct Bin4 {
    uint64_t* reg;
    uint32_t R;
    int kshift, bsh, dshift;
};
hipError_t radix_bin_pass4(const uint32_t* src, uint32_t* out, const Bin4& b4, uint64_t n, uint32_t* hist_ws,
                           bool csum_ready, hipStream_t stream);
hipError_t launch_seg(const BatchArgs& a, hipStream_t stream);
hipError_t launch_seg_flow(const BatchArgs& a, hipStream_t stream);
hipError_t launch_bin_front(const BatchArgs& a, uint32_t* hist_ws, bool hist_ready, bool csum_ready, hipStream_t stream);
hipError_t launch_hot_reset(uint2* hot_tab, hipStream_t stream);
hipError_t launch_rec4_expand(const BatchArgs& a, uint64_t* out, hipStream_t stream);
hipError_t launch_walk_long(const BatchArgs& a, hipStream_t stream);
hipError_t launch_walk_short(const BatchArgs& a, hipStream_t stream);
hipError_t launch_check_last(const BatchArgs& a, hipStream_t stream);
hipError_t launch_finish(const BatchArgs& a, hipStream_t stream);
hipError_t launch_front_ts(const BatchArgs& a, hipStream_t stream);
hipError_t launch_skip_apply(const BatchArgs& a, hipStream_t stream);
hipError_t launch_hot_sync(const Bucket* ring, BucketHot* hot, uint64_t buckets, hipStream_t stream);
hipError_t launch_init_state(Bucket* ring, Occ* occ, uint32_t K, int stride, const int32_t* src_map,
                             const Bucket* old_ring, const Occ* old_occ, int old_stride, hipStream_t stream);
hipError_t launch_snapshot(const Rule* rules, const Bucket* ring, const Occ* occ, uint32_t K, int stride,
                           int64_t now, double* out, hipStream_t stream);


struct CodecArgs {
    uint64_t n;
    const uint8_t* payload;
    const uint32_t* offsets;
    const int64_t* ts;
    sg_req* req;
    int32_t* xid;
    uint8_t* kind;
    const FidSlot* fid_tab;
    uint64_t fid_mask;
    const int32_t* xid_in;
    const uint8_t* kind_in;
    const sg_result* res;
    uint8_t* frames;
};

hipError_t launch_codec_decode(const CodecArgs& c, hipStream_t stream);
hipError_t launch_codec_encode(const CodecArgs& c, hipStream_t stream);


struct alignas(8) VEntry {
    uint64_t hash;
    uint64_t data;
    uint32_t len;
    uint32_t type;
};
static_assert(sizeof(VEntry) == 24, "VEntry layout");

struct alignas(16) VDesc {
    uint64_t inl;
    uint32_t off;
    uint32_t tl;
};
static_assert(sizeof(VDesc) == 16, "VDesc layout");

constexpr uint32_t kVdEmpty = 0xFFFFFFFFu;

struct VDictArgs {
    uint64_t* tab;
    uint64_t tab_mask;
    VEntry* entries;
    uint8_t* arena;
    uint64_t count;
    uint64_t arena_used;
    uint64_t m;
    const uint8_t* src;
    VDesc* desc;
    uint64_t* hash;
    uint64_t* ids;
    uint32_t* slot_of;
    uint32_t* dedupe;
    uint64_t dedupe_mask;
    uint64_t* scan;
    unsigned long long* n_miss;
    const uint8_t* types;
    const uint32_t* offsets;
};

struct PCodecArgs {
    uint64_t n;
    const uint8_t* payload;
    const uint32_t* offsets;
    const int64_t* ts;
    sg_cparam_req* req;
    int32_t* xid;
    uint8_t* kind;
    const FidSlot* fid_tab;
    uint64_t fid_mask;
    uint64_t* cnt;
    VDictArgs vd;
    const int32_t* xid_in;
    const uint8_t* kind_in;
    const sg_result* res;
    uint8_t* frames;
};

constexpr uint32_t kScanTile = 2048;
inline uint64_t scan_blocks(uint64_t n) { return (n + kScanTile - 1) / kScanTile; }
hipError_t launch_scan_u64(uint64_t* v, uint64_t n, uint64_t* sums, uint64_t* total, hipStream_t stream);
hipError_t launch_pcodec_count(const PCodecArgs& c, hipStream_t stream);
// ... 12 lines not shown
```

sentinel_amd/csrc/engine.hip:

```cpp
#include "engine.h"

#include <algorithm>
#include <cstdlib>
#include <mutex>

namespace sg {


__device__ __forceinline__ int32_t java_d2i(double x) {
    if (x != x) return 0;
    if (x >= 2147483647.0) return INT32_MAX;
    if (x <= -2147483648.0) return INT32_MIN;
    return (int32_t)x;
}

__device__ __forceinline__ int lane_id() { return (int)__lane_id(); }

__device__ __forceinline__ double qps_of(int64_t sum, double isec) { return avg_div((double)sum, isec); }

__device__ __forceinline__ int64_t wave_sum(int64_t v) {
#pragma unroll
    for (int o = 32; o > 0; o >>= 1) v += __shfl_xor((long long)v, o, 64);
    return v;
}
// ... 230 lines not shown

__shared__ uint32_t g_sbnd[kLdsBndFlow];
__shared__ uint32_t g_boff[kMaxWl];
__shared__ int g_blds;
__shared__ int64_t g_p0[kMaxWl];
__shared__ uint32_t g_np[kMaxWl];
constexpr int kModS = 64;
__shared__ uint8_t g_p0mod[kMaxWl][kModS + 1];

__device__ __forceinline__ int period_slot(int w, uint32_t q, int S) {
    if (S <= kModS) return (int)(((uint32_t)g_p0mod[w][S] + q) % (uint32_t)S);
    return (int)((g_p0[w] + (int64_t)q) % S);
}

template <bool L>
struct PeriodCursor {
    const uint32_t* gbnd;
    uint32_t base;
    uint32_t np;
    uint32_t q;
    uint32_t next_b;

    __device__ __forceinline__ void init(const BatchArgs& a, int w) {
        gbnd = a.bnd + (size_t)w * kMaxPeriods;
        base = g_boff[w];
        np = g_np[w];
        q = 0xFFFFFFFFu;
        next_b = 0;
    }
    __device__ __forceinline__ uint32_t at(uint32_t i) const {
        if constexpr (L) return g_sbnd[base + i];
        else return gbnd[i];
    }
    __device__ __forceinline__ void seek(uint32_t qq) {
        q = qq;
        next_b = (qq + 1 < np) ? at(qq + 1) : 0xFFFFFFFFu;
    }
    __device__ __forceinline__ uint32_t of(uint32_t idx) const {
        if (q != 0xFFFFFFFFu && idx < next_b) return q;
        uint32_t lo = 0, hi = np;
        while (hi - lo > 1) {
            const uint32_t mid = (lo + hi) >> 1;
            if (at(mid) <= idx) lo = mid;
            else hi = mid;
        }
        return lo;
    }
};

__device__ __forceinline__ void open_period_serial(PeriodState& ps, const Bucket* ring, const Rule& R, int64_t P,
                                                   int* I_out, int64_t* ws_out) {
    const int S = R.S;
    const int I = (int)(P % S);
    const int64_t ws = P * R.wl;
    const int64_t lo = ws - (int64_t)(S - 1) * R.wl;
    const int h = (int)((P + 1) % S);
    ps.wo_pass = ps.wo_wait = ps.head_other = 0;
    int64_t cI[SG_NUM_EVENTS];
    int64_t stI = INT64_MIN;
#pragma unroll 4
    for (int q = 0; q < S; ++q) {
        const int64_t st = ring[q].start;
        const int64_t pp = ring[q].c[SG_EV_PASS];
        const int64_t ww = ring[q].c[SG_EV_WAITING];
        const bool v = (q != I) && st != INT64_MIN && st >= lo;
        ps.wo_pass += v ? pp : 0;
        ps.wo_wait += v ? ww : 0;
        if (q == h && v) ps.head_other = pp;
        if (q == I) stI = st;
    }
    if (stI == ws) {
#pragma unroll
        for (int ev = 0; ev < SG_NUM_EVENTS; ++ev) cI[ev] = ring[I].c[ev];
    }
    open_bucket(ps, stI, cI, ws);
    *I_out = I;
    *ws_out = ws;
}


template <bool L, bool R4 = false>
__device__ uint32_t walk_serial(const BatchArgs& a, uint32_t k, uint64_t s, uint64_t e) {
    uint32_t opened = 0;
    const Rule R = a.rules[k];
    Bucket* ring = a.ring + (size_t)k * a.stride;
    BucketHot* hot = a.hot + (size_t)k * a.stride;
    PeriodCursor<L> pc;
    pc.init(a, R.wl_idx);
    const int64_t P0 = g_p0[R.wl_idx];
    PeriodState ps;
    {
        const Occ o = a.occ[k];
        ps.occ_pass = o.pass;
        ps.occ_req = o.pass_req;
    }
    int64_t ws = 0;
    int I = -1;
    const typename RecOf<R4>::T* rs = sorted_recs<R4>(a);
    typename RecOf<R4>::T nxt = rs[s];
    for (uint64_t j = s; j < e; ++j) {
        const typename RecOf<R4>::T cur = nxt;
        if (j + 1 < e) nxt = rs[j + 1];
        const Decoded d = decode(a, cur);
        const uint32_t q = pc.of(d.idx);
        if (q != pc.q) {
            if (I >= 0) {
                ring[I].start = ws;
#pragma unroll
                for (int ev = 0; ev < SG_NUM_EVENTS; ++ev) ring[I].c[ev] = ps.cur[ev];
                store_hot(hot + I, ws, ps.cur[SG_EV_PASS], ps.cur[SG_EV_WAITING]);
            }
            pc.seek(q);
            open_period_serial(ps, ring, R, P0 + (int64_t)q, &I, &ws);
            ++opened;
        }
        const double latest = qps_of(ps.wo_pass + ps.cur[SG_EV_PASS], R.isec);
        const double next_remaining = R.thr - latest - (double)d.acq;
        if (next_remaining >= 0) {
            ps.cur[SG_EV_PASS] += d.acq;
            ps.cur[SG_EV_PASS_REQUEST] += 1;
            if (d.prio) ps.cur[SG_EV_OCCUPIED_PASS] += d.acq;
            store_result(a.out, d.idx, SG_STATUS_OK, java_d2i(next_remaining), 0);
        } else {
            int32_t wait;
            const int32_t st = decide_fail(R, a.max_occ_ratio, ps, d.acq, d.prio, &wait);
            if (st != SG_STATUS_BLOCKED) store_result(a.out, d.idx, st, 0, wait);
        }
    }
    if (I >= 0) {
        ring[I].start = ws;
#pragma unroll
        for (int ev = 0; ev < SG_NUM_EVENTS; ++ev) ring[I].c[ev] = ps.cur[ev];
        store_hot(hot + I, ws, ps.cur[SG_EV_PASS], ps.cur[SG_EV_WAITING]);
    }
    Occ o;
    o.pass = ps.occ_pass;
    o.pass_req = ps.occ_req;
    a.occ[k] = o;
    return opened;
}


#ifndef SG_WAVE_UNROLL
#define SG_WAVE_UNROLL 4
#endif
constexpr int kWaveUnroll = SG_WAVE_UNROLL;

template <bool L>
struct WaveWalker {
    const BatchArgs& a;
    const Rule R;
    const int lane;
    Bucket* ring;
    BucketHot* hot;
    PeriodCursor<L> pc;
    int64_t P0;
    int64_t st;
    int64_t c[SG_NUM_EVENTS];
    PeriodState ps;
    int64_t ws;
    int I;
    int64_t d_blk, d_blkn, d_oblk;
    bool dead;

    __device__ WaveWalker(const BatchArgs& a_, uint32_t k)
        : a(a_), R(a_.rules[k]), lane(lane_id()) {
        ring = a.ring + (size_t)k * a.stride;
        hot = a.hot + (size_t)k * a.stride;
        pc.init(a, R.wl_idx);
        P0 = g_p0[R.wl_idx];
        st = INT64_MIN;
#pragma unroll
        for (int ev = 0; ev < SG_NUM_EVENTS; ++ev) c[ev] = 0;
        if (lane < R.S) {
            st = ring[lane].start;
#pragma unroll
            for (int ev = 0; ev < SG_NUM_EVENTS; ++ev) c[ev] = ring[lane].c[ev];
        }
        const Occ o = a.occ[k];
        ps.occ_pass = o.pass;
        ps.occ_req = o.pass_req;
#pragma unroll
        for (int ev = 0; ev < SG_NUM_EVENTS; ++ev) ps.cur[ev] = 0;
        ps.wo_pass = ps.wo_wait = ps.head_other = 0;
        ws = 0;
        I = -1;
        d_blk = d_blkn = d_oblk = 0;
        dead = false;
    }

    __device__ void close_period() {
        if (I < 0) return;
        ps.cur[SG_EV_BLOCK] += wave_sum(d_blk);
        ps.cur[SG_EV_BLOCK_REQUEST] += wave_sum(d_blkn);
        ps.cur[SG_EV_OCCUPIED_BLOCK] += wave_sum(d_oblk);
        d_blk = d_blkn = d_oblk = 0;
        if (lane == I) {
            st = ws;
#pragma unroll
            for (int ev = 0; ev < SG_NUM_EVENTS; ++ev) c[ev] = ps.cur[ev];
        }
    }

    __device__ void open_period(uint32_t q) {
        close_period();
        dead = false;
        pc.seek(q);
        const int64_t P = P0 + (int64_t)q;
        const int S = R.S;
        I = period_slot(R.wl_idx, q, S);
        ws = P * R.wl;
        int64_t cI[SG_NUM_EVENTS];
#pragma unroll
        for (int ev = 0; ev < SG_NUM_EVENTS; ++ev) cI[ev] = bcast64(c[ev], I);
        open_bucket(ps, bcast64(st, I), cI, ws);
        const int64_t lo = ws - (int64_t)(S - 1) * R.wl;
        const bool valid = lane < S && lane != I && st != INT64_MIN && st >= lo;
        ps.wo_pass = wave_sum(valid ? c[SG_EV_PASS] : 0);
        ps.wo_wait = wave_sum(valid ? c[SG_EV_WAITING] : 0);
        const int h = I + 1 == S ? 0 : I + 1;
        ps.head_other = (h != I) ? bcast64(valid ? c[SG_EV_PASS] : 0, h) : 0;
    }

    __device__ __forceinline__ bool occupy_possible(double latest) const {
        const double occupy_avg = qps_of(ps.wo_wait + ps.cur[SG_EV_WAITING], R.isec);
        if (!(occupy_avg <= a.max_occ_ratio * R.thr)) return false;
        const int64_t head = (R.S == 1) ? ps.cur[SG_EV_PASS] : ps.head_other;
        return latest + (double)(1 + ps.occ_pass) - (double)head <= R.thr;
    }

    __device__ void run(uint64_t run_mask, const Decoded& d) {
        const double latest0 = qps_of(ps.wo_pass + ps.cur[SG_EV_PASS], R.isec);
        if (!(R.thr - latest0 - 1.0 >= 0)) {
            const bool in = (run_mask >> lane) & 1ull;
            uint64_t pm = __ballot(in && d.prio);
            bool occ_ok = pm != 0 && occupy_possible(latest0);
            while (pm && occ_ok) {
                const int x = __builtin_ctzll(pm);
                pm &= pm - 1;
                const int64_t ax = bcast64(d.acq, x);
                int32_t wait;
                const int32_t stx = decide_fail(R, a.max_occ_ratio, ps, ax, true, &wait);
                if (lane == x && stx != SG_STATUS_BLOCKED) store_result(a.out, d.idx, stx, 0, wait);
                occ_ok = occupy_possible(latest0);
            }
            const bool rest = in && (!d.prio || ((pm >> lane) & 1ull));
            d_blk += rest ? d.acq : 0;
            d_blkn += rest ? 1 : 0;
            d_oblk += (rest && d.prio) ? d.acq : 0;
            dead = !occupy_possible(latest0);
            return;
        }
        uint64_t pending = run_mask;
        int guard = 0;
        while (pending) {
            if (++guard > 64) {
                atomicOr(a.err, kErrInternal);
                break;
            }
            const bool pl = (pending >> lane) & 1ull;
            const int64_t av = pl ? d.acq : 0;
            const int64_t ex = wave_excl_scan(av, lane);
// ... 1 lines not shown
            const double latest_l = qps_of(W + ex, R.isec);
            const double nr_l = R.thr - latest_l - (double)d.acq;
            const uint64_t fails = __ballot(pl && !(nr_l >= 0));
            const uint64_t pass_mask = fails ? (pending & below(__builtin_ctzll(fails))) : pending;
            if (pass_mask) {
                const bool pm = (pass_mask >> lane) & 1ull;
                if (pm) store_result(a.out, d.idx, SG_STATUS_OK, java_d2i(nr_l), 0);
                ps.cur[SG_EV_PASS] += wave_sum(pm ? d.acq : 0);
                ps.cur[SG_EV_PASS_REQUEST] += (int64_t)__popcll(pass_mask);
                ps.cur[SG_EV_OCCUPIED_PASS] += wave_sum((pm && d.prio) ? d.acq : 0);
            }
            if (!fails) break;
            int x = __builtin_ctzll(fails);
            pending &= ~below(x + 1);
            for (;;) {
                {
                    const int64_t ax = bcast64(d.acq, x);
                    const bool px = bcast32((int)d.prio, x) != 0;
                    int32_t wait;
                    const int32_t stx = decide_fail(R, a.max_occ_ratio, ps, ax, px, &wait);
                    if (lane == x && stx != SG_STATUS_BLOCKED) store_result(a.out, d.idx, stx, 0, wait);
                }
                if (!pending) break;
                const bool pl2 = (pending >> lane) & 1ull;
                const double latest = qps_of(ps.wo_pass + ps.cur[SG_EV_PASS], R.isec);
                const bool fit = pl2 && (R.thr - latest - (double)d.acq >= 0);
                const uint64_t fitm = __ballot(fit);
                const uint64_t stop = fitm | __ballot(pl2 && d.prio);
                const uint64_t blk = stop ? (pending & below(__builtin_ctzll(stop))) : pending;
                const bool b = (blk >> lane) & 1ull;
                d_blk += b ? d.acq : 0;
                d_blkn += b ? 1 : 0;
                if (!stop) {
                    pending = 0;
                    break;
                }
                const int g = __builtin_ctzll(stop);
                pending &= ~below(g);
                if ((fitm >> g) & 1ull) break;
                x = g;
                pending &= ~(1ull << g);
            }
        }
    }

    template <class RT>
    __device__ void chunk(RT rec, bool act) {
        Decoded d;
        d.idx = 0;
        d.acq = 0;
        d.prio = false;
        uint32_t q = 0xFFFFFFFFu;
        if (act) {
            d = decode(a, rec);
            q = pc.of(d.idx);
        }
        uint64_t todo = __ballot(act);
        int guard = 0;
        while (todo) {
            if (++guard > 64) {
                atomicOr(a.err, kErrInternal);
                break;
            }
            const uint32_t qrun = (uint32_t)bcast32((int)q, __builtin_ctzll(todo));
            if (qrun != pc.q) open_period(qrun);
            const uint64_t rm = __ballot(act && q == qrun) & todo;
            todo &= ~rm;
            run(rm, d);
        }
    }

    __device__ void finish(uint32_t k) {
        close_period();
        if (lane < R.S) {
            ring[lane].start = st;
#pragma unroll
            for (int ev = 0; ev < SG_NUM_EVENTS; ++ev) ring[lane].c[ev] = c[ev];
            store_hot(hot + lane, st, c[SG_EV_PASS], c[SG_EV_WAITING]);
        }
        if (lane == 0) {
            Occ o;
            o.pass = ps.occ_pass;
            o.pass_req = ps.occ_req;
            a.occ[k] = o;
        }
    }
};

template <class Pred>
__device__ __forceinline__ uint64_t wave_search(uint64_t lo, uint64_t hi, Pred pred, int lane) {
    while (hi - lo > 64) {
        const uint64_t step = (hi - lo + 63) / 64;
        const uint64_t p = lo + (uint64_t)lane * step;
        const uint64_t m = __ballot(p >= hi || pred(p));
        if (m == 0) {
            lo = lo + 63 * step + 1;
            continue;
        }
        const int f = __builtin_ctzll(m);
        if (f == 0) return lo;
        const uint64_t nhi = lo + (uint64_t)f * step;
        lo = lo + (uint64_t)(f - 1) * step + 1;
        hi = nhi < hi ? nhi : hi;
    }
    const uint64_t p = lo + (uint64_t)lane;
    const uint64_t m = __ballot(p < hi && pred(p));
    return m ? lo + (uint64_t)__builtin_ctzll(m) : hi;
}

template <bool L, bool R4 = false>
__device__ __forceinline__ void walk_wave(const BatchArgs& a, uint32_t k, uint64_t s, uint64_t e, uint32_t item) {
    using RT = typename RecOf<R4>::T;
    WaveWalker<L> w(a, k);
    const int lane = w.lane;
    const bool tab = a.long_pend != nullptr && item < kLongTab && w.pc.np <= (uint32_t)kLongPeriods;
    uint32_t pend_l = 0;
    if (tab && lane < kLongPeriods) pend_l = a.long_pend[(size_t)item * kLongPeriods + lane];
    const RT* rec = sorted_recs<R4>(a);
    constexpr uint64_t kBlock = 64ull * kWaveUnroll;
    RT cur[kWaveUnroll];
#pragma unroll
    for (int u = 0; u < kWaveUnroll; ++u) {
        const uint64_t j = s + (uint64_t)u * 64 + lane;
        cur[u] = j < e ? rec[j] : (RT)0;
    }
    uint32_t skip_tried_q = 0xFFFFFFFFu;
    uint64_t pos = s;
    while (pos < e) {
        uint64_t npos = pos + kBlock;
        RT nxt[kWaveUnroll];
#pragma unroll
        for (int u = 0; u < kWaveUnroll; ++u) {
            const uint64_t j = npos + (uint64_t)u * 64 + lane;
            nxt[u] = j < e ? rec[j] : (RT)0;
        }
        bool skipped = false;
#pragma unroll
        for (int u = 0; u < kWaveUnroll; ++u) {
            const uint64_t cb = pos + (uint64_t)u * 64;
            if (skipped || cb >= e) continue;
            w.chunk(cur[u], cb + lane < e);
            const uint64_t after = cb + 64;
            if (w.dead && after < e && w.pc.q != skip_tried_q) {
                skip_tried_q = w.pc.q;
                const uint32_t nb = w.pc.next_b;
                uint64_t pe;
                if (tab) {
                    pe = w.pc.q + 1 >= w.pc.np ? e : (uint64_t)(uint32_t)bcast32((int)pend_l, (int)w.pc.q);
                    pe = pe < after ? after : pe;
                } else {
                    pe = gallop_search(after, e, [&](uint64_t p) {
                        return rec_index(a, rec[p]) >= nb;
                    }, lane);
                }
                if (pe - after >= kSkipMin) {
                    const uint32_t np = (uint32_t)((pe - after + kSkipPiece - 1) / kSkipPiece);
                    uint32_t slot = 0;
                    if (lane == 0) slot = atomicAdd(a.skip_count, np);
#pragma unroll
                    for (int v = 0; v < kWaveUnroll; ++v) {
                        const uint64_t j = pe + (uint64_t)v * 64 + lane;
                        nxt[v] = j < e ? rec[j] : (RT)0;
                    }
                    slot = (uint32_t)bcast32((int)slot, 0);
                    if (slot + np <= a.skip_cap) {
                        for (uint32_t pi = lane; pi < np; pi += 64) {
                            const uint64_t b0 = after + (uint64_t)pi * kSkipPiece;
// ... 642 lines not shown
        }
    }
}

template <bool R4>
__global__ void __launch_bounds__(256) k_long_bounds(BatchArgs a) {
    if (*a.err) return;
    const typename RecOf<R4>::T* rs = sorted_recs<R4>(a);
    const uint32_t n_long = min(*a.long_count, kLongTab);
    const uint32_t total = n_long * (uint32_t)kLongPeriods;
    for (uint32_t t = blockIdx.x * blockDim.x + threadIdx.x; t < total; t += gridDim.x * blockDim.x) {
        const uint32_t item = t / kLongPeriods, q = t % kLongPeriods;
        const uint32_t k = a.long_key[item];
        const int w = a.rules[k].wl_idx;
        const uint32_t npw = a.np[w];
        if (npw > (uint32_t)kLongPeriods || q + 1 >= npw) continue;
        const uint32_t nb = a.bnd[(size_t)w * kMaxPeriods + q + 1];
        uint64_t lo = a.long_list[item], hi = a.long_end ? a.long_end[item] : a.seg_end[k];
        while (lo < hi) {
            const uint64_t mid = (lo + hi) >> 1;
            if (rec_index(a, rs[mid]) >= nb) hi = mid;
            else lo = mid + 1;
        }
        a.long_pend[t] = (uint32_t)lo;
    }
}

#ifndef SG_WLONG_BLOCKS
#define SG_WLONG_BLOCKS 2
#endif
template <bool R4>
__global__ void __launch_bounds__(256, SG_WLONG_BLOCKS) k_walk_long(BatchArgs a) {
    if (*a.err) return;
    stage_periods(a);
    if (g_blds) walk_long_body<true, R4>(a);
    else walk_long_body<false, R4>(a);
}


struct SlotSnap {
    int32_t st, pass, wait;
};
constexpr int32_t kSnapOld = -(1 << 30);

__device__ __forceinline__ int32_t rel32(int64_t x) {
    return x > (int64_t)INT32_MAX ? INT32_MAX : x < (int64_t)INT32_MIN ? INT32_MIN : (int32_t)x;
}

__device__ __forceinline__ int32_t snap_rel(int64_t start, int64_t T0) {
    if (start == INT64_MIN) return INT32_MIN;
    const int64_t d = start - T0;
    return d < (int64_t)kSnapOld ? kSnapOld : d > (int64_t)(1 << 30) ? (1 << 30) : (int32_t)d;
}

__device__ __forceinline__ bool narrow_span(const BatchArgs& a, int64_t T0) {
    bool ok = true;
    for (int w = 0; w < a.n_wl; ++w) {
        const int64_t wl = a.wl[w];
        const int64_t b = a.p0[w] * wl;
        ok = ok && (b + ((int64_t)a.np[w] + 1) * wl - T0 < (1ll << 29)) &&
             (b - ((int64_t)a.stride + 1) * wl - T0 > -(1ll << 29));
    }
    return ok;
}

__device__ __forceinline__ void store_bucket(Bucket* b, BucketHot* h, int64_t start, const int64_t* c) {
    ulonglong2* p = reinterpret_cast<ulonglong2*>(b);
    p[0] = make_ulonglong2((unsigned long long)start, (unsigned long long)c[0]);
    p[1] = make_ulonglong2((unsigned long long)c[1], (unsigned long long)c[2]);
    p[2] = make_ulonglong2((unsigned long long)c[3], (unsigned long long)c[4]);
    p[3] = make_ulonglong2((unsigned long long)c[5], (unsigned long long)c[6]);
    store_hot(h, start, c[SG_EV_PASS], c[SG_EV_WAITING]);
}

constexpr int kBlk = 4;

template <int SM, bool L, bool R4 = false>
__device__ __forceinline__ void walk_reg(const BatchArgs& a, bool act, uint32_t k, uint64_t s, uint64_t e,
                                         const Rule& R, const Occ& occ, SlotSnap* snap, typename RecOf<R4>::T* buf,
                                         int64_t T0) {
    using RT = typename RecOf<R4>::T;
    const RT* rs = sorted_recs<R4>(a);
    Bucket* ring = a.ring + (size_t)k * a.stride;
    BucketHot* hot = a.hot + (size_t)k * a.stride;
    const int S = R.S;
    const int64_t wl = R.wl;
    PeriodCursor<L> pc;
    pc.init(a, act ? R.wl_idx : 0);
    const int64_t P0 = g_p0[act ? R.wl_idx : 0];
    PeriodState ps;
    ps.occ_pass = occ.pass;
    ps.occ_req = occ.pass_req;
#pragma unroll
    for (int ev = 0; ev < SG_NUM_EVENTS; ++ev) ps.cur[ev] = 0;
    ps.wo_pass = ps.wo_wait = ps.head_other = 0;
    int I = -1;
    int64_t ws = 0;
    const uint64_t n1 = a.n - 1;
    RT nb[kBlk];
    uint64_t p = s;
    int left = kBlk;
    bool more = act && p + kBlk < e;
#pragma unroll
    for (int u = 0; u < kBlk; ++u) nb[u] = rs[min(p + kBlk + u, n1)];
    bool live = act;
    uint32_t qn = 0;
    Decoded dn;
    auto peek = [&]() {
        if (p + (uint64_t)(kBlk - left) >= e) {
            live = false;
            return;
        }
        dn = decode(a, buf[0]);
        qn = pc.of(dn.idx);
    };
    auto advance = [&]() {
#pragma unroll
        for (int v = 0; v < kBlk - 1; ++v) buf[v] = buf[v + 1];
        buf[kBlk - 1] = (RT)~0ull;
        if (--left == 0) {
            if (!more) {
                live = false;
                return;
            }
#pragma unroll
            for (int u = 0; u < kBlk; ++u) buf[u] = nb[u];
            p += kBlk;
            left = kBlk;
            more = p + kBlk < e;
#pragma unroll
            for (int u = 0; u < kBlk; ++u) nb[u] = rs[min(p + kBlk + u, n1)];
        }
    };
    if (live) peek();
    while (__ballot(live)) {
        if (live && qn != pc.q) {
            if (I >= 0) {
                store_bucket(ring + I, hot + I, ws, ps.cur);
                snap[I].st = (int32_t)(ws - T0);
                snap[I].pass = (int32_t)ps.cur[SG_EV_PASS];
                snap[I].wait = (int32_t)ps.cur[SG_EV_WAITING];
            }
            const uint32_t qprev = pc.q;
            pc.seek(qn);
            const int64_t P = P0 + (int64_t)qn;
            I = I < 0 ? period_slot(R.wl_idx, qn, S) : (int)((uint32_t)(I + (int)(qn - qprev)) % (uint32_t)S);
            ws = P * wl;
            const int64_t lo_rel = ws - (int64_t)S * wl - T0;
            const int32_t lo32 = rel32(lo_rel);
            const int h = I + 1 == S ? 0 : I + 1;
            int32_t sx[SM], px[SM], wx[SM];
#pragma unroll
            for (int x = 0; x < SM; ++x) {
                sx[x] = snap[x].st;
                px[x] = snap[x].pass;
                wx[x] = snap[x].wait;
            }
            uint32_t wp = 0, ww = 0, ho = 0;
#pragma unroll
            for (int x = 0; x < SM; ++x) {
                const bool v = (x < S) & (x != I) & (sx[x] > lo32);
                const uint32_t m = v ? 0xFFFFFFFFu : 0u;
                wp += (uint32_t)px[x] & m;
                ww += (uint32_t)wx[x] & m;
                ho = (x == h) ? ((uint32_t)px[x] & m) : ho;
            }
            ps.wo_pass = (int64_t)wp;
            ps.wo_wait = (int64_t)ww;
            ps.head_other = (int64_t)ho;
            const int32_t stI_rel = snap[I].st;
            const int64_t stI = stI_rel == INT32_MIN ? INT64_MIN : T0 + (int64_t)stI_rel;
            int64_t cI[SG_NUM_EVENTS];
            if (stI == ws) {
#pragma unroll
                for (int ev = 0; ev < SG_NUM_EVENTS; ++ev) cI[ev] = ring[I].c[ev];
            }
            open_bucket(ps, stI, cI, ws);
        }
        while (live && qn == pc.q) {
            const double latest = qps_of(ps.wo_pass + ps.cur[SG_EV_PASS], R.isec);
            const double next_remaining = R.thr - latest - (double)dn.acq;
            if (next_remaining >= 0) {
                ps.cur[SG_EV_PASS] += dn.acq;
                ps.cur[SG_EV_PASS_REQUEST] += 1;
                if (dn.prio) ps.cur[SG_EV_OCCUPIED_PASS] += dn.acq;
                store_result(a.out, dn.idx, SG_STATUS_OK, java_d2i(next_remaining), 0);
            } else {
                int32_t wait;
                const int32_t stt = decide_fail(R, a.max_occ_ratio, ps, dn.acq, dn.prio, &wait);
                if (stt != SG_STATUS_BLOCKED) store_result(a.out, dn.idx, stt, 0, wait);
            }
            advance();
            if (live) peek();
        }
    }

    if (act) {
        if (I >= 0) store_bucket(ring + I, hot + I, ws, ps.cur);
        if (ps.occ_pass != occ.pass || ps.occ_req != occ.pass_req) {
            Occ o;
            o.pass = ps.occ_pass;
            o.pass_req = ps.occ_req;
            a.occ[k] = o;
        }
    }
}

__device__ __forceinline__ void wait_vm0() { __builtin_amdgcn_s_waitcnt(0x0F70); }

template <int R, int W>
__device__ __forceinline__ void glds_rows(const uint32_t* src, uint32_t* wrecs) {
    if constexpr (R > 0) {
        glds_rows<R - 1, W>(src, wrecs);
        __builtin_amdgcn_global_load_lds((const __attribute__((address_space(1))) void*)src,
                                         (__attribute__((address_space(3))) void*)(wrecs + (R - 1) * 64 - W * (R - 1)),
                                         4, 4 * W * (R - 1), 0);
    }
}

template <int R, bool R4>
__device__ __forceinline__ void stage_records(const BatchArgs& a, uint32_t* wrecs, uint64_t p) {
    glds_rows<R, R4 ? 1 : 2>(reinterpret_cast<const uint32_t*>(sorted_recs<R4>(a) + p), wrecs);
}

template <int SM, bool L, bool R4>
__device__ __forceinline__ void walk_lds(const BatchArgs& a, bool act, uint32_t k, uint64_t s, uint64_t e,
                                         const Rule& R, const Occ& occ, SlotSnap* snap, uint32_t* wrecs, int lane,
                                         int64_t T0, int rows) {
    Bucket* ring = a.ring + (size_t)k * a.stride;
    BucketHot* hot = a.hot + (size_t)k * a.stride;
    const int S = R.S;
    const int64_t wl = R.wl;
    PeriodCursor<L> pc;
    pc.init(a, act ? R.wl_idx : 0);
    const int64_t P0 = g_p0[act ? R.wl_idx : 0];
    PeriodState ps;
    ps.occ_pass = occ.pass;
    ps.occ_req = occ.pass_req;
#pragma unroll
    for (int ev = 0; ev < SG_NUM_EVENTS; ++ev) ps.cur[ev] = 0;
    ps.wo_pass = ps.wo_wait = ps.head_other = 0;
    int I = -1;
    int64_t ws = 0;
    uint64_t wb = s;
    uint64_t p = s;
    bool live = act && p < e;
    bool park = false;
    uint32_t win = (uint32_t)rows;
    uint32_t qn = 0;
    Decoded dn;
    auto peek = [&]() {
        if (p >= e) {
            live = false;
            return;
        }
        if (p - wb >= (uint64_t)win) {
            park = true;
            return;
        }
        dn = decode_c(a, wrecs[(uint32_t)(p - wb) * 64 + lane]);
        qn = pc.of(dn.idx);
    };
    if (live) peek();
    for (;;) {
        if (!__ballot(live && !park)) {
            if (!__ballot(live)) break;
            if (park) {
                stage_records<kRecW, R4>(a, wrecs, p);
                wb = p;
                win = kRecW;
            }
            wait_vm0();
            __builtin_amdgcn_wave_barrier();
            if (park) {
                park = false;
                peek();
            }
            continue;
        }
        if (live && !park && qn != pc.q) {
            if (I >= 0) {
                store_bucket(ring + I, hot + I, ws, ps.cur);
                snap[I].st = (int32_t)(ws - T0);
                snap[I].pass = (int32_t)ps.cur[SG_EV_PASS];
                snap[I].wait = (int32_t)ps.cur[SG_EV_WAITING];
            }
            const uint32_t qprev = pc.q;
            pc.seek(qn);
            const int64_t P = P0 + (int64_t)qn;
            I = I < 0 ? period_slot(R.wl_idx, qn, S) : (int)((uint32_t)(I + (int)(qn - qprev)) % (uint32_t)S);
            ws = P * wl;
            const int64_t lo_rel = ws - (int64_t)S * wl - T0;
            const int32_t lo32 = rel32(lo_rel);
            const int h = I + 1 == S ? 0 : I + 1;
            int32_t sx[SM], px[SM], wx[SM];
#pragma unroll
            for (int x = 0; x < SM; ++x) {
                sx[x] = snap[x].st;
                px[x] = snap[x].pass;
                wx[x] = snap[x].wait;
            }
            uint32_t wp = 0, ww = 0, ho = 0;
#pragma unroll
            for (int x = 0; x < SM; ++x) {
                const bool v = (x < S) & (x != I) & (sx[x] > lo32);
                const uint32_t m = v ? 0xFFFFFFFFu : 0u;
                wp += (uint32_t)px[x] & m;
                ww += (uint32_t)wx[x] & m;
                ho = (x == h) ? ((uint32_t)px[x] & m) : ho;
            }
            ps.wo_pass = (int64_t)wp;
            ps.wo_wait = (int64_t)ww;
            ps.head_other = (int64_t)ho;
            const int32_t stI_rel = snap[I].st;
            const int64_t stI = stI_rel == INT32_MIN ? INT64_MIN : T0 + (int64_t)stI_rel;
            int64_t cI[SG_NUM_EVENTS];
            if (stI == ws) {
#pragma unroll
                for (int ev = 0; ev < SG_NUM_EVENTS; ++ev) cI[ev] = ring[I].c[ev];
            }
            open_bucket(ps, stI, cI, ws);
        }
        while (live && !park && qn == pc.q) {
            const double latest = qps_of(ps.wo_pass + ps.cur[SG_EV_PASS], R.isec);
            const double next_remaining = R.thr - latest - (double)dn.acq;
            if (next_remaining >= 0) {
                ps.cur[SG_EV_PASS] += dn.acq;
                ps.cur[SG_EV_PASS_REQUEST] += 1;
                if (dn.prio) ps.cur[SG_EV_OCCUPIED_PASS] += dn.acq;
                store_result(a.out, dn.idx, SG_STATUS_OK, java_d2i(next_remaining), 0);
            } else {
                int32_t wait;
                const int32_t stt = decide_fail(R, a.max_occ_ratio, ps, dn.acq, dn.prio, &wait);
                if (stt != SG_STATUS_BLOCKED) store_result(a.out, dn.idx, stt, 0, wait);
            }
            ++p;
            peek();
        }
    }
    if (act) {
        if (I >= 0) store_bucket(ring + I, hot + I, ws, ps.cur);
        if (ps.occ_pass != occ.pass || ps.occ_req != occ.pass_req) {
            Occ o;
            o.pass = ps.occ_pass;
            o.pass_req = ps.occ_req;
            a.occ[k] = o;
        }
    }
}

constexpr int kGatherMaxS = 10;
#ifndef SG_SHORT_BLOCKS
#define SG_SHORT_BLOCKS 3
#endif
constexpr int kShortBlocksPerCu = SG_SHORT_BLOCKS;

template <int SM, bool L, bool R4>
__device__ __forceinline__ void walk_short_lds(const BatchArgs& a, SlotSnap* snap_all, uint32_t* recs_all) {
    static_assert(SM > 0, "LDS ring snapshot");
    const int lane = lane_id();
    SlotSnap* snap = snap_all + (threadIdx.x / 64) * (64 * SM);
    uint32_t* wrecs = recs_all + (threadIdx.x / 64) * (kRecW * 64);
    const bool none = a.n == 0;
    uint32_t cnt[kClasses], grp_end[kClasses];
    uint32_t total = 0;
#pragma unroll
    for (int c = kClasses - 1; c >= 0; --c) {
        cnt[c] = (c == 0 && none) ? 0u : a.short_count[c];
        total += (cnt[c] + 63) / 64;
        grp_end[c] = total;
    }
    const uint32_t wave = blockIdx.x * (blockDim.x / 64) + threadIdx.x / 64;
    const uint32_t nwaves = gridDim.x * (blockDim.x / 64);
    if (wave >= total) return;
    const int64_t T0 = a.p0[0] * (int64_t)a.wl[0];
    auto desc = [&](uint32_t g, int& c, bool& act, uint32_t& s, uint32_t& k, uint32_t& e) {
        c = kClasses - 1;
        uint32_t g0 = 0;
        while (g >= grp_end[c]) {
            g0 = grp_end[c];
            --c;
        }
        c = __builtin_amdgcn_readfirstlane(c);
        const uint32_t i = (g - g0) * 64 + (uint32_t)lane;
        act = i < cnt[c];
        const uint64_t li = a.class_off[c] + (act ? i : 0u);
        s = a.short_list[li];
        k = a.short_key[li];
        e = a.short_end[li];
    };
    int c_n;
    bool act_n;
    uint32_t s_n, k_n, e_n;
    desc(wave, c_n, act_n, s_n, k_n, e_n);
    for (uint32_t g = wave; g < total; g += nwaves) {
        const uint64_t tw0 = (a.dbg & 64) ? __builtin_amdgcn_s_memrealtime() : 0;
        const int c = c_n;
        const bool act = act_n;
        const uint64_t s = s_n;
        const uint32_t k = k_n;
        const uint64_t e = e_n;
        const Rule R = a.rules[k];
        const Occ occ = a.occ[k];
        static_assert(kRecW >= (int)kClassMax[1], "the first window of class 1 must fit the lane's LDS rows");
        const int rows = c == 0 ? (int)kClassMax[0] : c == 1 ? (int)kClassMax[1] : kRecW;
        if (c == 0) stage_records<kClassMax[0], R4>(a, wrecs, s);
        else if (c == 1) stage_records<kClassMax[1], R4>(a, wrecs, s);
        else stage_records<kRecW, R4>(a, wrecs, s);
        desc(min(g + nwaves, total - 1), c_n, act_n, s_n, k_n, e_n);
        {
            constexpr int kT = SM;
            int gl = lane;
            asm volatile("" : "+v"(gl));
            ulonglong2 v[kT];
#pragma unroll
            for (int t = 0; t < kT; ++t) {
                const int pc = t * 64 + gl;
                const int j = pc / kT;
                const int q = pc % kT;
                const uint32_t kj = (uint32_t)__shfl((int)k, j, 64);
                const int qq = q < a.stride ? q : 0;
                v[t] = *reinterpret_cast<const ulonglong2*>(a.hot + (size_t)kj * a.stride + qq);
            }
            __builtin_amdgcn_sched_barrier(0);
#pragma unroll
            for (int t = 0; t < kT; ++t) asm volatile("" ::"v"(v[t].x), "v"(v[t].y));
#pragma unroll
            for (int t = 0; t < kT; ++t) {
                const int pc = t * 64 + gl;
                SlotSnap& d = snap[pc];
                d.st = snap_rel((int64_t)v[t].x, T0);
                d.pass = (int32_t)(uint32_t)v[t].y;
                d.wait = (int32_t)(uint32_t)(v[t].y >> 32);
            }
        }
        wait_vm0();
        __builtin_amdgcn_fence(__ATOMIC_RELEASE, "wavefront");
        __builtin_amdgcn_wave_barrier();
        __builtin_amdgcn_fence(__ATOMIC_ACQUIRE, "wavefront");
        const uint64_t tw1 = (a.dbg & 64) ? __builtin_amdgcn_s_memrealtime() : 0;
        walk_lds<SM, L, R4>(a, act, k, s, e, R, occ, snap + lane * SM, wrecs, lane, T0, rows);
        if (a.dbg & 64) {
            const uint64_t tw2 = __builtin_amdgcn_s_memrealtime();
            if (lane == 0) {
                atomicAdd(&a.dbg_ctr[0], (unsigned long long)(tw2 - tw0));
                atomicAdd(&a.dbg_ctr[1 + c], 1ull);
                atomicAdd(&a.dbg_ctr[7 + c], (unsigned long long)(tw1 - tw0));
                atomicAdd(&a.dbg_ctr[7 + c], (unsigned long long)(tw2 - tw1) << 32);
            }
        }
    }
}

template <int SM, bool L, bool C, bool R4>
__device__ __forceinline__ void walk_short_body(const BatchArgs& a, SlotSnap* snap_all, uint32_t* recs_all) {
    using RT = typename RecOf<R4>::T;
    if constexpr (SM > 0 && C) {
        const int64_t T0 = a.p0[0] * (int64_t)a.wl[0];
        if (a.narrow && narrow_span(a, T0)) {
            walk_short_lds<SM, L, R4>(a, snap_all, recs_all);
            return;
        }
    }
    constexpr int kSnapPerWave = SM > 0 ? 64 * SM : 1;
    const int lane = lane_id();
    SlotSnap* snap = snap_all + (threadIdx.x / 64) * kSnapPerWave;
    const bool none = a.n == 0 && a.narrow && narrow_span(a, a.p0[0] * (int64_t)a.wl[0]);
    uint32_t cnt[kClasses], grp_end[kClasses];
    uint32_t total = 0;
#pragma unroll
    for (int c = kClasses - 1; c >= 0; --c) {
        cnt[c] = (c == 0 && none) ? 0u : a.short_count[c];
        total += (cnt[c] + 63) / 64;
        grp_end[c] = total;
    }
    const uint32_t wave = blockIdx.x * (blockDim.x / 64) + threadIdx.x / 64;
    const uint32_t nwaves = gridDim.x * (blockDim.x / 64);
    const int64_t T0 = a.p0[0] * (int64_t)a.wl[0];
    const bool snap_ok = SM > 0 && a.narrow && narrow_span(a, T0);
    for (uint32_t g = wave; g < total; g += nwaves) {
        int c = kClasses - 1;
        uint32_t g0 = 0;
        while (g >= grp_end[c]) {
            g0 = grp_end[c];
            --c;
        }
        c = __builtin_amdgcn_readfirstlane(c);
        const uint32_t i = (g - g0) * 64 + (uint32_t)lane;
        const bool act = i < cnt[c];
        if constexpr (SM > 0 && !C) if (snap_ok) {
            const uint64_t tw0 = (a.dbg & 64) ? __builtin_amdgcn_s_memrealtime() : 0;
            const uint64_t li = a.class_off[c] + (act ? i : 0u);
            const uint64_t s = a.short_list[li];
            const uint32_t k = a.short_key[li];
            const uint64_t e = a.short_end ? a.short_end[li] : a.seg_end[k];
            const Rule R = a.rules[k];
            const Occ occ = a.occ[k];
            RT buf[kBlk];
#pragma unroll
            for (int u = 0; u < kBlk; ++u) buf[u] = sorted_recs<R4>(a)[min(s + u, a.n - 1)];
            {
                constexpr int kT = SM;
                int gl = lane;
                asm volatile("" : "+v"(gl));
                {
                    ulonglong2 v[SM];
#pragma unroll
                    for (int t = 0; t < SM; ++t) {
                        const int pc = t * 64 + gl;
                        const int j = pc / kT;
                        const int q = pc % kT;
                        const uint32_t kj = (uint32_t)__shfl((int)k, j, 64);
                        const int qq = q < a.stride ? q : 0;
                        v[t] = *reinterpret_cast<const ulonglong2*>(a.hot + (size_t)kj * a.stride + qq);
                    }
#pragma unroll
                    for (int t = 0; t < SM; ++t) {
                        SlotSnap& d = snap[t * 64 + gl];
                        d.st = snap_rel((int64_t)v[t].x, T0);
                        d.pass = (int32_t)(uint32_t)v[t].y;
                        d.wait = (int32_t)(uint32_t)(v[t].y >> 32);
                    }
                }
                __builtin_amdgcn_fence(__ATOMIC_RELEASE, "wavefront");
                __builtin_amdgcn_wave_barrier();
                __builtin_amdgcn_fence(__ATOMIC_ACQUIRE, "wavefront");
            }
            const uint64_t tw1 = (a.dbg & 64) ? __builtin_amdgcn_s_memrealtime() : 0;
            walk_reg<SM, L, R4>(a, act, k, s, e, R, occ, snap + lane * SM, buf, T0);
            if (a.dbg & 64) {
                const uint64_t tw2 = __builtin_amdgcn_s_memrealtime();
                if (lane == 0) {
                    atomicAdd(&a.dbg_ctr[0], (unsigned long long)(tw2 - tw0));
                    atomicAdd(&a.dbg_ctr[1 + c], 1ull);
                    atomicAdd(&a.dbg_ctr[7 + c], (unsigned long long)(tw1 - tw0));
                    atomicAdd(&a.dbg_ctr[7 + c], (unsigned long long)(tw2 - tw1) << 32);
                }
            }
            continue;
        }
        if (!act) continue;
        const uint64_t s = a.short_list[a.class_off[c] + i];
        if constexpr (R4) {
            walk_serial<L, true>(a, a.short_key[a.class_off[c] + i], s, a.short_end[a.class_off[c] + i]);
        } else {
            const uint32_t k = (uint32_t)(a.rec_sorted[s] >> a.kshift);
            const uint64_t lim = s + (uint64_t)min(a.short_max, c < kClasses - 1 ? kClassMax[c] : 0xFFFFFFFFu) + 1;
            uint64_t e = s + 1;
            while (e < a.n && e < lim && (uint32_t)(a.rec_sorted[e] >> a.kshift) == k) ++e;
            walk_serial<L>(a, k, s, e);
        }
    }
}

template <int SM, bool C, bool R4 = false>
#ifndef SG_SHORT_C_BLOCKS
#define SG_SHORT_C_BLOCKS 2
#endif
__global__ void __launch_bounds__(256, C ? SG_SHORT_C_BLOCKS : kShortBlocksPerCu) k_walk_short(BatchArgs a) {
    static_assert(SM <= kGatherMaxS, "LDS budget of the ring snapshot");
    __shared__ SlotSnap snap_all[4 * (SM > 0 ? 64 * SM : 1)];
    __shared__ uint32_t recs_all[SM > 0 && C ? 4 * kRecW * 64 : 1];
    if (*a.err) return;
    stage_periods(a);
    if (g_blds) walk_short_body<SM, true, C, R4>(a, snap_all, recs_all);
    else walk_short_body<SM, false, C, R4>(a, snap_all, recs_all);
}

constexpr int kSkipU = 8;
template <bool R4>
__global__ void __launch_bounds__(256) k_skip_apply(BatchArgs a) {
    using RT = typename RecOf<R4>::T;
    if (*a.err) return;
    const RT* rs = sorted_recs<R4>(a);
    const uint32_t cnt = min(*a.skip_count, a.skip_cap);
    const int lane = lane_id();
    const uint32_t wave = blockIdx.x * (blockDim.x / 64) + threadIdx.x / 64;
    const uint32_t nwaves = gridDim.x * (blockDim.x / 64);
    for (uint32_t i = wave; i < cnt; i += nwaves) {
        const uint4 sk = a.skips[i];
        int64_t sa = 0, spa = 0;
        for (uint64_t j0 = (uint64_t)sk.z; j0 < sk.w; j0 += 64ull * kSkipU) {
            RT r[kSkipU];
#pragma unroll
            for (int u = 0; u < kSkipU; ++u) {
                const uint64_t j = j0 + (uint64_t)u * 64 + lane;
                r[u] = j < sk.w ? rs[j] : (RT)0;
            }
#pragma unroll
            for (int u = 0; u < kSkipU; ++u) {
                if (j0 + (uint64_t)u * 64 + lane >= sk.w) continue;
                const Decoded d = decode(a, r[u]);
                sa += d.acq;
                spa += d.prio ? d.acq : 0;
            }
        }
        sa = wave_sum(sa);
        spa = wave_sum(spa);
        if (lane == 0) {
            const Rule R = a.rules[sk.x];
            const int64_t P = a.p0[R.wl_idx] + (int64_t)sk.y;
            Bucket& bk = a.ring[(size_t)sk.x * a.stride + (int)(P % R.S)];
            if (bk.start == P * R.wl) {
                atomicAdd((unsigned long long*)&bk.c[SG_EV_BLOCK], (unsigned long long)sa);
                atomicAdd((unsigned long long*)&bk.c[SG_EV_BLOCK_REQUEST], (unsigned long long)(sk.w - sk.z));
                atomicAdd((unsigned long long*)&bk.c[SG_EV_OCCUPIED_BLOCK], (unsigned long long)spa);
            }
        }
    }
}

__global__ void k_check_last(BatchArgs a) {
    if (a.n > 0 && a.req[0].ts_ms < *a.last_ts) atomicOr(a.err, kErrTime);
}

__global__ void k_finish(BatchArgs a) {
    if (*a.err == 0 && a.n > 0) *a.last_ts = a.req[a.n - 1].ts_ms;
}

__global__ void k_front_ts(BatchArgs a) {
    if (*a.err == 0 && a.n > 0) *a.front_ts = a.req[a.n - 1].ts_ms;
}


__global__ void __launch_bounds__(256) k_hot_sync(const Bucket* ring, BucketHot* hot, uint64_t buckets) {
    for (uint64_t i = (uint64_t)blockIdx.x * blockDim.x + threadIdx.x; i < buckets; i += (uint64_t)gridDim.x * blockDim.x)
        store_hot(hot + i, ring[i].start, ring[i].c[SG_EV_PASS], ring[i].c[SG_EV_WAITING]);
}

__global__ void __launch_bounds__(256) k_init_state(Bucket* ring, Occ* occ, uint32_t K, int stride,
                                                    const int32_t* src_map, const Bucket* old_ring,
                                                    const Occ* old_occ, int old_stride) {
    const uint64_t total = (uint64_t)K * stride;
    for (uint64_t i = (uint64_t)blockIdx.x * blockDim.x + threadIdx.x; i < total; i += (uint64_t)gridDim.x * blockDim.x) {
        const uint32_t k = (uint32_t)(i / stride);
        const int q = (int)(i % stride);
        const int32_t src = src_map ? src_map[k] : -1;
        Bucket b;
        if (src >= 0 && q < old_stride) {
            b = old_ring[(size_t)src * old_stride + q];
        } else {
            b.start = INT64_MIN;
#pragma unroll
            for (int ev = 0; ev < SG_NUM_EVENTS; ++ev) b.c[ev] = 0;
        }
        ring[i] = b;
        if (q == 0) {
            Occ o;
            if (src >= 0) o = old_occ[src];
            else o.pass = o.pass_req = 0;
            occ[k] = o;
        }
    }
}

__global__ void __launch_bounds__(256) k_snapshot(const Rule* rules, const Bucket* ring, const Occ* occ, uint32_t K,
                                                  int stride, int64_t now, double* out) {
    for (uint32_t k = blockIdx.x * blockDim.x + threadIdx.x; k < K; k += gridDim.x * blockDim.x) {
        const Rule R = rules[k];
        const Bucket* rg = ring + (size_t)k * stride;
        const int64_t P = now / R.wl;
        const int I = (int)(P % R.S);
        const int64_t ws = P * R.wl;
        int64_t pass = 0, block = 0;
        for (int q = 0; q < R.S; ++q) {
            const int64_t s0 = rg[q].start;
            if (q == I) {
                if (s0 == ws) {
                    pass += rg[q].c[SG_EV_PASS];
                    block += rg[q].c[SG_EV_BLOCK];
                } else if (s0 != INT64_MIN && s0 < ws && occ[k].pass_req > 0) {
                    pass += occ[k].pass;
                }
                continue;
            }
            if (s0 != INT64_MIN && now - s0 <= (int64_t)R.S * R.wl) {
                pass += rg[q].c[SG_EV_PASS];
                block += rg[q].c[SG_EV_BLOCK];
            }
        }
        out[2 * (size_t)k] = (double)pass / R.isec;
        out[2 * (size_t)k + 1] = (double)block / R.isec;
    }
}


static unsigned grid_for(uint64_t n, unsigned block, unsigned cap) {
    uint64_t g = (n + block - 1) / block;
    if (g < 1) g = 1;
    if (g > cap) g = cap;
    return (unsigned)g;
}


hipError_t launch_prep(const BatchArgs& a, hipStream_t stream) {
    lds_poison(stream);
    if (a.bin_on) {
        const uint64_t tiles = (a.n + kPrepTile - 1) / kPrepTile;
        hipLaunchKernelGGL(k_prep<true>, dim3((unsigned)((tiles + a.prep_tiles - 1) / a.prep_tiles)), dim3(256), 0,
                           stream, a);
    }
    else hipLaunchKernelGGL(k_prep<false>, dim3((unsigned)((a.n + kPrepTile - 1) / kPrepTile)), dim3(256), 0, stream, a);
    return hipGetLastError();
}

hipError_t launch_seg(const BatchArgs& a, hipStream_t stream) {
    lds_poison(stream);
    hipLaunchKernelGGL(k_seg, dim3(grid_for(a.n, kSegTile, 8192)), dim3(kSegThreads), 0, stream, a);
    return hipGetLastError();
}

__global__ void __launch_bounds__(256) k_lds_poison() {
    extern __shared__ uint32_t lds_all[];
    volatile uint32_t* p = lds_all;
    for (uint32_t i = threadIdx.x; i < kPoisonBytes / 4; i += 256) p[i] = 0xA5A5A5A5u;
}

void lds_poison(hipStream_t stream) {
    struct Cfg {
        int mode;
        unsigned blocks;
    };
    static const Cfg cfg = [] {
        const char* e = std::getenv("SG_LDS_POISON");
        Cfg c{e ? std::atoi(e) : 0, 0u};
        int dev = 0, cus = 0;
        (void)hipGetDevice(&dev);
        (void)hipDeviceGetAttribute(&cus, hipDeviceAttributeMultiprocessorCount, dev);
        c.blocks = 2u * (unsigned)(cus > 0 ? cus : 256);
        if (c.mode) (void)hipFuncSetAttribute((const void*)k_lds_poison, hipFuncAttributeMaxDynamicSharedMemorySize,
                                              (int)kPoisonBytes);
        return c;
    }();
    if (cfg.mode) hipLaunchKernelGGL(k_lds_poison, dim3(cfg.blocks), dim3(256), kPoisonBytes, stream);
}

hipError_t launch_bin_front(const BatchArgs& a, uint32_t* hist_ws, bool hist_ready, bool csum_ready, hipStream_t stream) {
    hipError_t e;
    if (a.rec4) {
        if (!hist_ready || a.abits != kRec4Abits) return hipErrorInvalidValue;
        e = radix_bin_pass4(reinterpret_cast<const uint32_t*>(a.rec), reinterpret_cast<uint32_t*>(a.rec_sorted),
                            Bin4{a.bin_buf, a.bin_R, a.kshift, a.bin_bsh, a.bin_dshift}, a.n, hist_ws, csum_ready,
                            stream);
    } else {
        e = radix_bin_pass(a.rec, a.rec_sorted, a.bin_buf, a.bin_R, a.n, a.bin_dshift, hist_ws, hist_ready, csum_ready,
                           stream);
    }
    if (e != hipSuccess) return e;
    BatchArgs b = a;
    b.bin_tot = radix_tot(hist_ws, a.n, kBinDigit);
    lds_poison(stream);
    if (a.rec4) hipLaunchKernelGGL(k_bin_sort<true>, dim3(a.bin_R + 1), dim3(kBinThreads), 0, stream, b);
    else hipLaunchKernelGGL(k_bin_sort<false>, dim3(a.bin_R + 1), dim3(kBinThreads), 0, stream, b);
    lds_poison(stream);
    hipLaunchKernelGGL(k_hot_update, dim3(1), dim3(1024), 0, stream, b);
// ... 61 lines not shown

static unsigned walker_grid(const void* kern, int walk_cus) {
    struct Entry {
        const void* k;
        int cus;
        unsigned blocks;
    };
    static std::mutex mu;
    static Entry cache[64];
    static int used = 0;
    std::lock_guard<std::mutex> lock(mu);
    for (int i = 0; i < used; ++i)
        if (cache[i].k == kern && cache[i].cus == walk_cus) return cache[i].blocks;
    const unsigned b = resident_blocks(kern, 256, walk_cus);
    if (used < 64) cache[used++] = Entry{kern, walk_cus, b};
    return b;
}

hipError_t launch_walk_long(const BatchArgs& a, hipStream_t stream) {
    if (a.rec4) {
        if (!a.long_key || !a.long_end) return hipErrorInvalidValue;
        if (a.long_pend) hipLaunchKernelGGL(k_long_bounds<true>, dim3(1024), dim3(256), 0, stream, a);
        hipLaunchKernelGGL(k_walk_long<true>, dim3(walker_grid((const void*)k_walk_long<true>, a.walk_cus)), dim3(256),
                           0, stream, a);
        return hipGetLastError();
    }
    if (a.long_pend && a.long_key && a.seg_end)
        hipLaunchKernelGGL(k_long_bounds<false>, dim3(1024), dim3(256), 0, stream, a);
    hipLaunchKernelGGL(k_walk_long<false>, dim3(walker_grid((const void*)k_walk_long<false>, a.walk_cus)), dim3(256), 0,
                       stream, a);
    return hipGetLastError();
}

static bool short_compact(const BatchArgs& a) { return a.abits == 8 && a.imask <= 0xFFFFFFull; }

template <int SM>
static hipError_t launch_short_sm(const BatchArgs& a, hipStream_t stream) {
    const bool c = SM > 0 && short_compact(a);
    if (a.rec4) {
        if (!a.short_key || !a.short_end) return hipErrorInvalidValue;
        const void* kern4 = c ? (const void*)k_walk_short<SM, true, true> : (const void*)k_walk_short<SM, false, true>;
        const unsigned blocks4 = walker_grid(kern4, a.walk_cus);
        if (c) hipLaunchKernelGGL((k_walk_short<SM, true, true>), dim3(blocks4), dim3(256), 0, stream, a);
        else hipLaunchKernelGGL((k_walk_short<SM, false, true>), dim3(blocks4), dim3(256), 0, stream, a);
        return hipGetLastError();
    }
    const void* kern = c ? (const void*)k_walk_short<SM, true> : (const void*)k_walk_short<SM, false>;
    const unsigned blocks = walker_grid(kern, a.walk_cus);
    if (c) hipLaunchKernelGGL((k_walk_short<SM, true>), dim3(blocks), dim3(256), 0, stream, a);
    else hipLaunchKernelGGL((k_walk_short<SM, false>), dim3(blocks), dim3(256), 0, stream, a);
    return hipGetLastError();
}

hipError_t launch_walk_short(const BatchArgs& a, hipStream_t stream) {
    if (a.generic_walker) return launch_short_sm<0>(a, stream);
    if (a.stride <= 2) return launch_short_sm<2>(a, stream);
    if (a.stride <= 4) return launch_short_sm<4>(a, stream);
    if (a.stride <= 8) return launch_short_sm<8>(a, stream);
    if (a.stride <= 10) return launch_short_sm<10>(a, stream);
    return launch_short_sm<0>(a, stream);
}

hipError_t launch_skip_apply(const BatchArgs& a, hipStream_t stream) {
    if (a.rec4) hipLaunchKernelGGL(k_skip_apply<true>, dim3(2048), dim3(256), 0, stream, a);
    else hipLaunchKernelGGL(k_skip_apply<false>, dim3(2048), dim3(256), 0, stream, a);
    return hipGetLastError();
}

hipError_t launch_check_last(const BatchArgs& a, hipStream_t stream) {
    hipLaunchKernelGGL(k_check_last, dim3(1), dim3(1), 0, stream, a);
    return hipGetLastError();
}

hipError_t launch_front_ts(const BatchArgs& a, hipStream_t stream) {
    hipLaunchKernelGGL(k_front_ts, dim3(1), dim3(1), 0, stream, a);
    return hipGetLastError();
}

hipError_t launch_finish(const BatchArgs& a, hipStream_t stream) {
    hipLaunchKernelGGL(k_finish, dim3(1), dim3(1), 0, stream, a);
    return hipGetLastError();
}

hipError_t launch_hot_sync(const Bucket* ring, BucketHot* hot, uint64_t buckets, hipStream_t stream) {
    if (buckets == 0) return hipSuccess;
    hipLaunchKernelGGL(k_hot_sync, dim3(grid_for(buckets, 256, 8192)), dim3(256), 0, stream, ring, hot, buckets);
    return hipGetLastError();
}

hipError_t launch_init_state(Bucket* ring, Occ* occ, uint32_t K, int stride, const int32_t* src_map,
                             const Bucket* old_ring, const Occ* old_occ, int old_stride, hipStream_t stream) {
    if (K == 0) return hipSuccess;
    hipLaunchKernelGGL(k_init_state, dim3(grid_for((uint64_t)K * stride, 256, 8192)), dim3(256), 0, stream, ring, occ,
                       K, stride, src_map, old_ring, old_occ, old_stride);
    return hipGetLastError();
}

hipError_t launch_snapshot(const Rule* rules, const Bucket* ring, const Occ* occ, uint32_t K, int stride,
                           int64_t now, double* out, hipStream_t stream) {
    if (K == 0) return hipSuccess;
    hipLaunchKernelGGL(k_snapshot, dim3(grid_for(K, 256, 4096)), dim3(256), 0, stream, rules, ring, occ, K, stride,
                       now, out);
    return hipGetLastError();
}

}
```

sentinel_amd/csrc/local.hip:

```cpp
#include "pslot_dev.h"

namespace sg {

namespace {

__device__ __forceinline__ int lane_id() { return (int)__lane_id(); }

__device__ __forceinline__ int32_t java_d2i(double x) {
    if (x != x) return 0;
    if (x >= 2147483647.0) return INT32_MAX;
    if (x <= -2147483648.0) return INT32_MIN;
    return (int32_t)x;
}

__device__ __forceinline__ double qps_of(int64_t sum, double isec) { return avg_div((double)sum, isec); }

__device__ __forceinline__ int64_t wave_sum(int64_t v) {
#pragma unroll
    for (int o = 32; o > 0; o >>= 1) v += __shfl_xor((long long)v, o, 64);
    return v;
}

__device__ __forceinline__ int64_t wave_min(int64_t v) {
#pragma unroll
// ... 1089 lines not shown
    const uint32_t wave = blockIdx.x * (blockDim.x / 64) + threadIdx.x / 64;
    const uint32_t nwaves = gridDim.x * (blockDim.x / 64);
    for (uint32_t item = wave; item < n_long; item += nwaves) {
        const uint64_t s = sg.long_list[item];
        const uint32_t k = (uint32_t)(a.rec_sorted[s] >> a.kshift);
        if (a.rules[k].cx || (a.dyn && a.dyn[k] == a.epoch)) continue;
        const uint64_t e = gallop_search(s + (sg.short_max ? sg.short_max : 1), a.n, [&](uint64_t p) {
            return (uint32_t)(a.rec_sorted[p] >> a.kshift) != k;
        }, lane);
        lwalk_wave(a, bndp, k, s, e);
    }
}


namespace {

__device__ __forceinline__ int64_t java_d2l(double x) {
    if (x != x) return 0;
    if (x >= 9223372036854775807.0) return INT64_MAX;
    if (x <= -9223372036854775808.0) return INT64_MIN;
    return (int64_t)x;
}

__device__ __forceinline__ int64_t java_round(double a) {
    const int64_t bits = __double_as_longlong(a);
    const int64_t shift = (52 - 1 + 1023) - ((bits & 0x7FF0000000000000LL) >> 52);
    if ((shift & -64) == 0) {
        int64_t r = (bits & 0x000FFFFFFFFFFFFFLL) | 0x0010000000000000LL;
        if (bits < 0) r = -r;
        return ((r >> shift) + 1) >> 1;
    }
    return java_d2l(a);
}

__device__ int64_t warm_cool_down(const LFlowRule& r, const LCtl& c, int64_t ct, int64_t pass_qps) {
    const int64_t old = c.stored;
    int64_t nv = old;
    if (old < r.warning_token || (old > r.warning_token && pass_qps < java_d2i(r.count) / r.cold))
        nv = java_d2l((double)old + (double)(ct - c.last_filled) * r.count / 1000);
    return nv < r.max_token ? nv : (int64_t)r.max_token;
}

__device__ void warm_sync(const LFlowRule& r, LCtl& c, int64_t now, int64_t pass_qps) {
    const int64_t ct = now - now % 1000;
    if (ct <= c.last_filled) return;
    const int64_t cur = (int64_t)((uint64_t)warm_cool_down(r, c, ct, pass_qps) - (uint64_t)pass_qps);
    c.stored = cur < 0 ? 0 : cur;
    c.last_filled = ct;
}

__device__ __forceinline__ double warm_qps(const LFlowRule& r, int64_t above) {
    return nextafter(1.0 / ((double)above * r.slope + 1.0 / r.count), (double)INFINITY);
}

__device__ bool pace_step(const LFlowRule& r, LCtl& c, int64_t now, int64_t cost, int64_t* wait) {
    *wait = 0;
    if (cost + c.latest <= now) {
        c.latest = now;
        return true;
    }
    if (cost + c.latest - now > r.max_queue_ms) return false;
    c.latest += cost;
    const int64_t w = c.latest - now;
    if (w > r.max_queue_ms) {
        c.latest -= cost;
        return false;
    }
    *wait = w > 0 ? w : 0;
    return true;
}


__device__ __forceinline__ double c3_qps(int64_t sum, double isec) { return avg_div((double)sum, isec); }

__device__ int32_t embedded_token(const LArgs& a, uint32_t key, int64_t t, int32_t acq, bool prio, int32_t* wait) {
    *wait = 0;
    key &= SG_KEY_INDEX;
    if (key == SG_KEY_BAD || acq <= 0) return SG_STATUS_BAD_REQUEST;
    if (key >= a.c3_K) return SG_STATUS_NO_RULE_EXISTS;
    const uint8_t ls = a.c3_rule_lim ? a.c3_rule_lim[key] : (uint8_t)0xFF;
    if (ls != 0xFF && !emb_lim_try_pass(a.lim_ring + ls, t, a.lim_qps[ls])) return SG_STATUS_TOO_MANY_REQUEST;
    const Rule R = a.c3_rules[key];
    Bucket* ring = a.c3_ring + (size_t)key * a.c3_stride;
    const Occ o = a.c3_occ[key];
    int64_t occ_pass = o.pass, occ_req = o.pass_req;
    const int64_t P = t / R.wl;
    const int S = R.S;
    const int I = (int)(P % S);
    const int64_t ws = P * R.wl;
    const int64_t lo = ws - (int64_t)(S - 1) * R.wl;
    const int h = (int)((P + 1) % S);
    int64_t wo_pass = 0, wo_wait = 0, head_other = 0;
    for (int q = 0; q < S; ++q) {
        const int64_t st = ring[q].start;
        const bool v = q != I && st != INT64_MIN && st >= lo;
        wo_pass += v ? ring[q].c[SG_EV_PASS] : 0;
        wo_wait += v ? ring[q].c[SG_EV_WAITING] : 0;
        if (q == h && v) head_other = ring[q].c[SG_EV_PASS];
    }
    int64_t cur[SG_NUM_EVENTS];
    const int64_t stI = ring[I].start;
    if (stI == ws) {
        for (int e = 0; e < SG_NUM_EVENTS; ++e) cur[e] = ring[I].c[e];
    } else {
        for (int e = 0; e < SG_NUM_EVENTS; ++e) cur[e] = 0;
        if (stI != INT64_MIN && occ_req > 0) {
            cur[SG_EV_OCCUPIED_PASS] += occ_pass;
            cur[SG_EV_PASS] += occ_pass;
            cur[SG_EV_PASS_REQUEST] += occ_req;
            occ_pass = occ_req = 0;
        }
    }
    int32_t st = SG_STATUS_BLOCKED;
    const double latest = c3_qps(wo_pass + cur[SG_EV_PASS], R.isec);
    const double next_remaining = R.thr - latest - (double)acq;
    if (next_remaining >= 0) {
        cur[SG_EV_PASS] += acq;
        cur[SG_EV_PASS_REQUEST] += 1;
        if (prio) cur[SG_EV_OCCUPIED_PASS] += acq;
        st = SG_STATUS_OK;
    } else {
        bool waited = false;
        if (prio) {
            const double occupy_avg = c3_qps(wo_wait + cur[SG_EV_WAITING], R.isec);
            if (occupy_avg <= a.max_occ_ratio * R.thr) {
                const int64_t head = (S == 1) ? cur[SG_EV_PASS] : head_other;
                if (latest + (double)(acq + occ_pass) - (double)head <= R.thr) {
                    occ_pass += acq;
                    occ_req += 1;
                    cur[SG_EV_WAITING] += acq;
                    if (R.wait_ms > 0) {
                        *wait = R.wait_ms;
                        st = SG_STATUS_SHOULD_WAIT;
                        waited = true;
                    }
                }
            }
        }
        if (!waited) {
            cur[SG_EV_BLOCK] += acq;
            cur[SG_EV_BLOCK_REQUEST] += 1;
            if (prio) cur[SG_EV_OCCUPIED_BLOCK] += acq;
        }
    }
    ring[I].start = ws;
    for (int e = 0; e < SG_NUM_EVENTS; ++e) ring[I].c[e] = cur[e];
    store_hot(a.c3_hot + (size_t)key * a.c3_stride + I, ws, cur[SG_EV_PASS], cur[SG_EV_WAITING]);
    if (occ_pass != o.pass || occ_req != o.pass_req) {
        Occ no;
        no.pass = occ_pass;
        no.pass_req = occ_req;
        a.c3_occ[key] = no;
    }
    return st;
}

template <class RefExists>
__device__ int cx_select(const LArgs& a, const LRule& R, const LFlowRule& r, int origin, int ctx, RefExists&& ref_exists) {
    int matched;
    if (origin > 0 && r.limit_app == origin) {
        matched = 1;
    } else if (r.limit_app == SG_LIMIT_APP_DEFAULT) {
        matched = 0;
    } else if (r.limit_app == SG_LIMIT_APP_OTHER && origin > 0) {
        for (uint32_t i = 0; i < R.fr_n; ++i)
            if (a.frules[R.fr_begin + i].limit_app == origin) return -1;
        matched = 1;
    } else {
        return -1;
    }
    if (r.strategy == SG_STRATEGY_DIRECT) return matched;
    if (r.ref < 0) return -1;
    if (r.strategy == SG_STRATEGY_RELATE) return ref_exists() ? 3 : -1;
    if (r.strategy == SG_STRATEGY_CHAIN) return r.ref == ctx ? 2 : -1;
    return -1;
}

__device__ int cx_rule(const LArgs& a, LNode& n, const LFlowRule& r, LCtl& c, const LEvent& e, int64_t t,
                       uint32_t qs, uint32_t qm, int64_t* wait) {
    *wait = 0;
    switch (r.behavior) {
    case SG_CONTROL_WARM_UP: {
        n.at_s(qs);
        n.at_m(qm);
        const int64_t pass_qps = java_d2l(n.pass_qps());
        warm_sync(r, c, t, java_d2l((double)n.prev_pass(t)));
        const int64_t sum = (int64_t)((uint64_t)pass_qps + (uint64_t)(int64_t)e.count);
        const double lim = c.stored >= r.warning_token ? warm_qps(r, c.stored - r.warning_token) : r.count;
        return (double)sum <= lim ? 1 : 0;
    }
    case SG_CONTROL_RATE_LIMITER:
        if (e.count <= 0) return 1;
        if (r.count <= 0) return 0;
        return pace_step(r, c, t, java_round(1.0 * (double)e.count / r.count * 1000), wait) ? 1 : 0;
    case SG_CONTROL_WARM_UP_RATE_LIMITER: {
        n.at_m(qm);
        warm_sync(r, c, t, java_d2l((double)n.prev_pass(t)));
        const double q = c.stored >= r.warning_token ? warm_qps(r, c.stored - r.warning_token) : r.count;
        return pace_step(r, c, t, java_round(1.0 * (double)e.count / q * 1000), wait) ? 1 : 0;
    }
    default: {
        if (r.grade != 0) n.at_s(qs);
        const int32_t cur = r.grade == 0 ? (int32_t)n.threads : java_d2i(n.pass_qps());
        if (!((double)(int32_t)((uint32_t)cur + (uint32_t)e.count) > r.count)) return 1;
        if (e.prio && r.grade == 1) {
            n.at_m(qm);
            const int64_t w = n.try_occupy_next(t, e.count, r.count);
            if (w < a.occupy_timeout) {
                const int s = n.bor_window(t + w);
                if (s >= 0) n.bor[s].pass += e.count;
                n.mc[kLOccPass] += e.count;
                n.mc[kLPass] += e.count;
                *wait = w;
                return 2;
            }
        }
        return 0;
    }
    }
}

__device__ __forceinline__ uint2 event_nodes(const LArgs& a, uint32_t idx) {
    if (!a.nkeys) return make_uint2(kNoNode, kNoNode);
    return a.ev_node[idx];
}

constexpr uint32_t kCxNdBytes = (uint32_t)((sizeof(LNode) + 15) / 16 * 16);
constexpr uint32_t kCxLdsBytes = 256 * kCxNdBytes;

template <bool W>
struct CxNodes;
template <>
struct CxNodes<false> {
    LNode on, cn;
    __device__ CxNodes(const LArgs& a, const LNode& nd, uint32_t on_idx, uint32_t cn_idx, unsigned char*)
// ... 1527 lines not shown
```

Measured before the change: 24.62 billion decisions/s.

## Pack per-flow occupancy, rule and hot buckets into one aligned line

Replaces the separate hot-bucket and occupancy arrays with one per-flow line, 128-byte aligned, holding Occ, a copy of the Rule, and the BucketHot ring. The walker kernels now read rule, occupancy and hot state from that single line, so each flow touches fewer distinct cache lines during a batch. In exchange the rule table is duplicated and kept in sync with strided 2D copies, the hot ring is padded to line size, and host export and import paths are adjusted.

```diff
diff --git a/__graft_entry__.py b/__graft_entry__.py
--- a/__graft_entry__.py
+++ b/__graft_entry__.py
@@ -15,6 +15,7 @@
     subprocess.check_call(["make", "-C", os.path.join(ROOT, "tests", "cpp"), "-f", "system_host.mk"], env=env)
     subprocess.check_call(["make", "-C", os.path.join(ROOT, "tests", "cpp"), "-f", "blocklog_host.mk"], env=env)
     subprocess.check_call(["make", "-C", os.path.join(ROOT, "tests", "cpp"), "-f", "table_grow_host.mk"], env=env)
+    subprocess.check_call(["make", "-C", os.path.join(ROOT, "tests", "cpp"), "-f", "flowline_host.mk"], env=env)
     if ROOT not in sys.path:
         sys.path.insert(0, ROOT)
     import sentinel_amd
diff --git a/sentinel_amd/csrc/api.cpp b/sentinel_amd/csrc/api.cpp
--- a/sentinel_amd/csrc/api.cpp
+++ b/sentinel_amd/csrc/api.cpp
@@ -55,8 +55,7 @@
 
     DevBuf<Rule> d_rules;
     DevBuf<Bucket> d_ring;
-    DevBuf<BucketHot> d_hot;
-    DevBuf<Occ> d_occ;
+    DevBuf<unsigned char> d_line;
     DevBuf<uint32_t> d_hot_key;
     uint64_t hot_gen = ~0ull;
     uint64_t rules_gen = 0;
@@ -471,6 +470,17 @@
     return SG_OK;
 }
 
+hipError_t upload_rules(sg_handle* h) {
+    if (!h->K) return hipSuccess;
+    hipError_t e = hipMemcpy(h->d_rules, h->rule_tab.data(), sizeof(Rule) * h->K, hipMemcpyHostToDevice);
+    if (e == hipSuccess && h->d_line) {
+        const LineCopy c = line_copy_rule(h->stride, h->K);
+        e = hipMemcpy2D(h->d_line + c.off, c.pitch, h->rule_tab.data(), c.width, c.width, c.rows,
+                        hipMemcpyHostToDevice);
+    }
+    return e;
+}
+
 int upload_rule_table(sg_handle* h) {
     h->l_groups_stale = true;
     h->ps_groups_stale = true;
@@ -483,7 +493,7 @@
         const double bound = (R.thr > 0 ? R.thr : 0.0) * (2.0 + R.isec) * (2.0 + ratio);
         if (!(bound < 1073741824.0)) h->wide_seen = true;
     }
-    if (h->K) HIP_TRY(h, hipMemcpy(h->d_rules, h->rule_tab.data(), sizeof(Rule) * h->K, hipMemcpyHostToDevice));
+    HIP_TRY(h, upload_rules(h));
     h->d_rule_lim.reset();
     if (h->K) {
         std::vector<uint8_t> rl(h->K, 0xFF);
@@ -762,8 +772,7 @@
     int32_t wl[kMaxWl]{};
     DevBuf<Rule> d_rules;
     DevBuf<Bucket> d_ring;
-    DevBuf<BucketHot> d_hot;
-    DevBuf<Occ> d_occ;
+    DevBuf<unsigned char> d_line;
     DevBuf<uint32_t> d_seg_end;
 };
 
@@ -810,14 +819,14 @@
         if (!L.d_rules.alloc(n)) return fail(h, SG_E_NOMEM, "rule table");
     } else if (n) {
         DevBuf<int32_t> d_src;
-        if (!L.d_rules.alloc(n) || !L.d_ring.alloc((size_t)n * stride) || !L.d_hot.alloc((size_t)n * stride) ||
-            !L.d_occ.alloc(n) || !d_src.alloc(n))
+        if (!L.d_rules.alloc(n) || !L.d_ring.alloc((size_t)n * stride) || !L.d_line.alloc((size_t)n * line_bytes(stride)) ||
+            !d_src.alloc(n))
             return fail(h, SG_E_NOMEM, "rule state allocation failed");
         const int rc = flow_seg_alloc(h, L.d_seg_end, n);
         if (rc) return rc;
         HIP_TRY(h, hipMemcpy(d_src, src.data(), sizeof(int32_t) * n, hipMemcpyHostToDevice));
-        HIP_TRY(h, launch_init_state(L.d_ring, L.d_occ, n, stride, d_src, h->d_ring, h->d_occ, h->stride, 0));
-        HIP_TRY(h, launch_hot_sync(L.d_ring, L.d_hot, (uint64_t)n * stride, 0));
+        HIP_TRY(h, launch_init_state(L.d_ring, L.d_line, n, stride, d_src, h->d_ring, h->d_line, h->stride, 0));
+        HIP_TRY(h, launch_hot_sync(L.d_ring, L.d_line, n, stride, 0));
         HIP_TRY(h, hipDeviceSynchronize());
     }
     return SG_OK;
@@ -848,8 +857,7 @@
     h->conc_dirty = true;
     h->d_rules = std::move(L.d_rules);
     h->d_ring = std::move(L.d_ring);
-    h->d_hot = std::move(L.d_hot);
-    h->d_occ = std::move(L.d_occ);
+    h->d_line = std::move(L.d_line);
     sg_handle::FlowWs& w = h->ws[0];
     w.seg_end = std::move(L.d_seg_end);
     w.seg_cap = w.seg_end ? n + 1 : 0;
@@ -1351,8 +1359,8 @@
     a.K = h->K;
     a.rules = h->d_rules;
     a.ring = h->d_ring;
-    a.hot = h->d_hot;
-    a.occ = h->d_occ;
+    a.line = h->d_line;
+    a.line_sz = (uint32_t)line_bytes(h->stride);
     a.seg_end = w.seg_end;
     a.seg_start = w.seg_start;
     a.short_end = w.short_end;
@@ -1900,7 +1908,8 @@
     std::vector<Bucket> b(S);
     HIP_TRY(h, hipMemcpy(b.data(), h->d_ring + (size_t)key * h->stride, sizeof(Bucket) * S, hipMemcpyDeviceToHost));
     Occ o;
-    HIP_TRY(h, hipMemcpy(&o, h->d_occ + key, sizeof(Occ), hipMemcpyDeviceToHost));
+    HIP_TRY(h, hipMemcpy(&o, h->d_line + (size_t)key * line_bytes(h->stride) + line_occ_off(), sizeof(Occ),
+                         hipMemcpyDeviceToHost));
     for (int j = 0; j < S; ++j) {
         starts[j] = b[j].start;
         for (int e = 0; e < SG_NUM_EVENTS; ++e) counters[j * SG_NUM_EVENTS + e] = b[j].start == INT64_MIN ? 0 : b[j].c[e];
@@ -1922,7 +1931,8 @@
     drain_async(h);
     static_assert(sizeof(Bucket) == 64 && sizeof(Occ) == 16, "export layout");
     HIP_TRY(h, hipMemcpy(ring, h->d_ring, rw * 8, hipMemcpyDeviceToHost));
-    HIP_TRY(h, hipMemcpy(occ, h->d_occ, ow * 8, hipMemcpyDeviceToHost));
+    const LineCopy c = line_copy_occ(h->stride, h->K);
+    HIP_TRY(h, hipMemcpy2D(occ, c.width, h->d_line + c.off, c.pitch, c.width, c.rows, hipMemcpyDeviceToHost));
     return SG_OK;
 }
 
@@ -1935,9 +1945,10 @@
     HIP_TRY(h, hipSetDevice(h->device));
     drain_async(h);
     HIP_TRY(h, hipMemcpy(h->d_ring, ring, rw * 8, hipMemcpyHostToDevice));
-    HIP_TRY(h, launch_hot_sync(h->d_ring, h->d_hot, (uint64_t)h->K * h->stride, 0));
+    HIP_TRY(h, launch_hot_sync(h->d_ring, h->d_line, h->K, h->stride, 0));
     HIP_TRY(h, hipDeviceSynchronize());
-    HIP_TRY(h, hipMemcpy(h->d_occ, occ, ow * 8, hipMemcpyHostToDevice));
+    const LineCopy c = line_copy_occ(h->stride, h->K);
+    HIP_TRY(h, hipMemcpy2D(h->d_line + c.off, c.pitch, occ, c.width, c.width, c.rows, hipMemcpyHostToDevice));
     return SG_OK;
 }
 
@@ -1948,7 +1959,7 @@
     drain_async(h);
     DevBuf<double> d_out;
     if (!d_out.alloc(2 * (size_t)h->K)) return fail(h, SG_E_DEVICE, "snapshot buffer: out of memory");
-    hipError_t e1 = launch_snapshot(h->d_rules, h->d_ring, h->d_occ, h->K, h->stride, now_ms, d_out, 0);
+    hipError_t e1 = launch_snapshot(h->d_rules, h->d_ring, h->d_line, h->K, h->stride, now_ms, d_out, 0);
     hipError_t e2 = e1 == hipSuccess ? hipMemcpy(out, d_out, sizeof(double) * 2 * h->K, hipMemcpyDeviceToHost) : e1;
     if (e2 != hipSuccess) return fail(h, SG_E_DEVICE, hipGetErrorString(e2));
     return SG_OK;
@@ -1959,7 +1970,7 @@
     if (h->K == 0) return SG_OK;
     HIP_TRY(h, hipSetDevice(h->device));
     drain_async(h);
-    HIP_TRY(h, launch_snapshot(h->d_rules, h->d_ring, h->d_occ, h->K, h->stride, now_ms, out_dev, (hipStream_t)stream));
+    HIP_TRY(h, launch_snapshot(h->d_rules, h->d_ring, h->d_line, h->K, h->stride, now_ms, out_dev, (hipStream_t)stream));
     return SG_OK;
 }
 
@@ -1981,7 +1992,7 @@
         d.ticket = 0;
     }
     *d.h_err = 0;
-    HIP_TRY(h, launch_snapshot(h->d_rules, h->d_ring, h->d_occ, h->K, h->stride, now_ms, out_dev, h->s_back));
+    HIP_TRY(h, launch_snapshot(h->d_rules, h->d_ring, h->d_line, h->K, h->stride, now_ms, out_dev, h->s_back));
     HIP_TRY(h, hipEventRecord(d.done, h->s_back));
     d.local = false;
     d.ticket = h->next_ticket++;
@@ -3392,8 +3403,8 @@
         L.emb = 1;
         L.c3_rules = h->d_rules;
         L.c3_ring = h->d_ring;
-        L.c3_hot = h->d_hot;
-        L.c3_occ = h->d_occ;
+        L.c3_line = h->d_line;
+        L.c3_line_sz = (uint32_t)line_bytes(h->stride);
         L.c3_stride = h->stride;
         L.c3_K = h->K;
         L.max_occ_ratio = h->cfg.max_occupy_ratio;
@@ -4979,7 +4990,7 @@
         h->n_wl = f->n_wl;
         std::memcpy(h->wl, f->wl, sizeof(h->wl));
         NHIP(nd, hipSetDevice(h->device));
-        NHIP(nd, hipMemcpy(h->d_rules, h->rule_tab.data(), sizeof(Rule) * h->K, hipMemcpyHostToDevice));
+        NHIP(nd, upload_rules(h));
     }
     nd->rec_path = same && std::getenv("SG_NODE_LEGACY") == nullptr;
     if (nd->rec_path && !nd->d_sub_rec) {
@@ -5608,7 +5619,7 @@
             if (!nd->sh[g].r_snap.reserve(2 * part_max)) return nfail(nd, SG_E_NOMEM, "node snapshot part");
             part = nd->sh[g].r_snap;
         }
-        NHIP(nd, launch_snapshot(h->d_rules, h->d_ring, h->d_occ, h->K, h->stride, now_ms, part, nd->sh[g].stream));
+        NHIP(nd, launch_snapshot(h->d_rules, h->d_ring, h->d_line, h->K, h->stride, now_ms, part, nd->sh[g].stream));
         NHIP(nd, hipStreamSynchronize(nd->sh[g].stream));
         NHIP(nd, hipSetDevice(nd->devices[0]));
         if (dev != nd->devices[0])
diff --git a/sentinel_amd/csrc/engine.h b/sentinel_amd/csrc/engine.h
--- a/sentinel_amd/csrc/engine.h
+++ b/sentinel_amd/csrc/engine.h
@@ -7,6 +7,7 @@
 #include "../../include/sentinel_gpu.h"
 #include "authority_rules.h"
 #include "blocklog_rules.h"
+#include "flowline.h"
 #include "system_rules.h"
 #include "search_dev.h"
 
@@ -47,6 +48,13 @@
     int64_t pass;
     int64_t pass_req;
 };
+static_assert(sizeof(Occ) == 16, "Occ layout");
+
+static_assert(sizeof(Occ) == kLineOccBytes && sizeof(Rule) == kLineRuleBytes && sizeof(BucketHot) == kLineHotBytes,
+              "walker line parts");
+static_assert(line_rule_off() % alignof(Rule) == 0 && line_hot_off() % alignof(BucketHot) == 0 &&
+                  kLineAlign % alignof(Occ) == 0,
+              "walker line alignment");
 
 #ifndef SG_SORT_ROUNDS
 #define SG_SORT_ROUNDS 16
@@ -86,8 +94,8 @@
     uint32_t K;
     const Rule* rules;
     Bucket* ring;
-    BucketHot* hot;
-    Occ* occ;
+    unsigned char* line;
+    uint32_t line_sz;
     int stride;
     double max_occ_ratio;
     int n_wl;
@@ -134,6 +142,19 @@
     const uint32_t* bin_tot;
     int rec4;
 };
+
+__host__ __device__ __forceinline__ unsigned char* line_of(const BatchArgs& a, uint32_t k) {
+    return a.line + (size_t)k * a.line_sz;
+}
+__host__ __device__ __forceinline__ Occ* occ_of(const BatchArgs& a, uint32_t k) {
+    return reinterpret_cast<Occ*>(line_of(a, k) + line_occ_off());
+}
+__host__ __device__ __forceinline__ const Rule* line_rule(const BatchArgs& a, uint32_t k) {
+    return reinterpret_cast<const Rule*>(line_of(a, k) + line_rule_off());
+}
+__host__ __device__ __forceinline__ BucketHot* hot_of(const BatchArgs& a, uint32_t k) {
+    return reinterpret_cast<BucketHot*>(line_of(a, k) + line_hot_off());
+}
 
 constexpr int kBinDigit = 10;
 constexpr uint32_t kBinRegular = 512;
@@ -688,8 +709,8 @@
     int32_t emb;
     const Rule* c3_rules;
     Bucket* c3_ring;
-    BucketHot* c3_hot;
-    Occ* c3_occ;
+    unsigned char* c3_line;
+    uint32_t c3_line_sz;
     int c3_stride;
     uint32_t c3_K;
     double max_occ_ratio;
@@ -933,10 +954,11 @@
 hipError_t launch_finish(const BatchArgs& a, hipStream_t stream);
 hipError_t launch_front_ts(const BatchArgs& a, hipStream_t stream);
 hipError_t launch_skip_apply(const BatchArgs& a, hipStream_t stream);
-hipError_t launch_hot_sync(const Bucket* ring, BucketHot* hot, uint64_t buckets, hipStream_t stream);
-hipError_t launch_init_state(Bucket* ring, Occ* occ, uint32_t K, int stride, const int32_t* src_map,
-                             const Bucket* old_ring, const Occ* old_occ, int old_stride, hipStream_t stream);
-hipError_t launch_snapshot(const Rule* rules, const Bucket* ring, const Occ* occ, uint32_t K, int stride,
+hipError_t launch_hot_sync(const Bucket* ring, unsigned char* line, uint32_t K, int stride, hipStream_t stream);
+hipError_t launch_init_state(Bucket* ring, unsigned char* line, uint32_t K, int stride, const int32_t* src_map,
+                             const Bucket* old_ring, const unsigned char* old_line, int old_stride,
+                             hipStream_t stream);
+hipError_t launch_snapshot(const Rule* rules, const Bucket* ring, const unsigned char* line, uint32_t K, int stride,
                            int64_t now, double* out, hipStream_t stream);
 
 
diff --git a/sentinel_amd/csrc/engine.hip b/sentinel_amd/csrc/engine.hip
--- a/sentinel_amd/csrc/engine.hip
+++ b/sentinel_amd/csrc/engine.hip
@@ -336,15 +336,15 @@
 template <bool L, bool R4 = false>
 __device__ uint32_t walk_serial(const BatchArgs& a, uint32_t k, uint64_t s, uint64_t e) {
     uint32_t opened = 0;
-    const Rule R = a.rules[k];
+    const Rule R = *line_rule(a, k);
     Bucket* ring = a.ring + (size_t)k * a.stride;
-    BucketHot* hot = a.hot + (size_t)k * a.stride;
+    BucketHot* hot = hot_of(a, k);
     PeriodCursor<L> pc;
     pc.init(a, R.wl_idx);
     const int64_t P0 = g_p0[R.wl_idx];
     PeriodState ps;
     {
-        const Occ o = a.occ[k];
+        const Occ o = *occ_of(a, k);
         ps.occ_pass = o.pass;
         ps.occ_req = o.pass_req;
     }
@@ -390,7 +390,7 @@
     Occ o;
     o.pass = ps.occ_pass;
     o.pass_req = ps.occ_req;
-    a.occ[k] = o;
+    *occ_of(a, k) = o;
     return opened;
 }
 
@@ -418,9 +418,9 @@
     bool dead;
 
     __device__ WaveWalker(const BatchArgs& a_, uint32_t k)
-        : a(a_), R(a_.rules[k]), lane(lane_id()) {
+        : a(a_), R(*line_rule(a_, k)), lane(lane_id()) {
         ring = a.ring + (size_t)k * a.stride;
-        hot = a.hot + (size_t)k * a.stride;
+        hot = hot_of(a, k);
         pc.init(a, R.wl_idx);
         P0 = g_p0[R.wl_idx];
         st = INT64_MIN;
@@ -431,7 +431,7 @@
 #pragma unroll
             for (int ev = 0; ev < SG_NUM_EVENTS; ++ev) c[ev] = ring[lane].c[ev];
         }
-        const Occ o = a.occ[k];
+        const Occ o = *occ_of(a, k);
         ps.occ_pass = o.pass;
         ps.occ_req = o.pass_req;
 #pragma unroll
@@ -599,7 +599,7 @@
             Occ o;
             o.pass = ps.occ_pass;
             o.pass_req = ps.occ_req;
-            a.occ[k] = o;
+            *occ_of(a, k) = o;
         }
     }
 };
@@ -1408,7 +1408,7 @@
     using RT = typename RecOf<R4>::T;
     const RT* rs = sorted_recs<R4>(a);
     Bucket* ring = a.ring + (size_t)k * a.stride;
-    BucketHot* hot = a.hot + (size_t)k * a.stride;
+    BucketHot* hot = hot_of(a, k);
     const int S = R.S;
     const int64_t wl = R.wl;
     PeriodCursor<L> pc;
@@ -1527,7 +1527,7 @@
             Occ o;
             o.pass = ps.occ_pass;
             o.pass_req = ps.occ_req;
-            a.occ[k] = o;
+            *occ_of(a, k) = o;
         }
     }
 }
@@ -1554,7 +1554,7 @@
                                          const Rule& R, const Occ& occ, SlotSnap* snap, uint32_t* wrecs, int lane,
                                          int64_t T0, int rows) {
     Bucket* ring = a.ring + (size_t)k * a.stride;
-    BucketHot* hot = a.hot + (size_t)k * a.stride;
+    BucketHot* hot = hot_of(a, k);
     const int S = R.S;
     const int64_t wl = R.wl;
     PeriodCursor<L> pc;
@@ -1670,7 +1670,7 @@
             Occ o;
             o.pass = ps.occ_pass;
             o.pass_req = ps.occ_req;
-            a.occ[k] = o;
+            *occ_of(a, k) = o;
         }
     }
 }
@@ -1726,8 +1726,8 @@
         const uint64_t s = s_n;
         const uint32_t k = k_n;
         const uint64_t e = e_n;
-        const Rule R = a.rules[k];
-        const Occ occ = a.occ[k];
+        const Rule R = *line_rule(a, k);
+        const Occ occ = *occ_of(a, k);
         static_assert(kRecW >= (int)kClassMax[1], "the first window of class 1 must fit the lane's LDS rows");
         const int rows = c == 0 ? (int)kClassMax[0] : c == 1 ? (int)kClassMax[1] : kRecW;
         if (c == 0) stage_records<kClassMax[0], R4>(a, wrecs, s);
@@ -1746,7 +1746,7 @@
                 const int q = pc % kT;
                 const uint32_t kj = (uint32_t)__shfl((int)k, j, 64);
                 const int qq = q < a.stride ? q : 0;
-                v[t] = *reinterpret_cast<const ulonglong2*>(a.hot + (size_t)kj * a.stride + qq);
+                v[t] = *reinterpret_cast<const ulonglong2*>(hot_of(a, kj) + qq);
             }
             __builtin_amdgcn_sched_barrier(0);
 #pragma unroll
@@ -1820,8 +1820,8 @@
             const uint64_t s = a.short_list[li];
             const uint32_t k = a.short_key[li];
             const uint64_t e = a.short_end ? a.short_end[li] : a.seg_end[k];
-            const Rule R = a.rules[k];
-            const Occ occ = a.occ[k];
+            const Rule R = *line_rule(a, k);
+            const Occ occ = *occ_of(a, k);
             RT buf[kBlk];
 #pragma unroll
             for (int u = 0; u < kBlk; ++u) buf[u] = sorted_recs<R4>(a)[min(s + u, a.n - 1)];
@@ -1838,7 +1838,7 @@
                         const int q = pc % kT;
                         const uint32_t kj = (uint32_t)__shfl((int)k, j, 64);
                         const int qq = q < a.stride ? q : 0;
-                        v[t] = *reinterpret_cast<const ulonglong2*>(a.hot + (size_t)kj * a.stride + qq);
+                        v[t] = *reinterpret_cast<const ulonglong2*>(hot_of(a, kj) + qq);
                     }
 #pragma unroll
                     for (int t = 0; t < SM; ++t) {
@@ -1949,14 +1949,19 @@
 }
 
 
-__global__ void __launch_bounds__(256) k_hot_sync(const Bucket* ring, BucketHot* hot, uint64_t buckets) {
-    for (uint64_t i = (uint64_t)blockIdx.x * blockDim.x + threadIdx.x; i < buckets; i += (uint64_t)gridDim.x * blockDim.x)
-        store_hot(hot + i, ring[i].start, ring[i].c[SG_EV_PASS], ring[i].c[SG_EV_WAITING]);
-}
-
-__global__ void __launch_bounds__(256) k_init_state(Bucket* ring, Occ* occ, uint32_t K, int stride,
+__global__ void __launch_bounds__(256) k_hot_sync(const Bucket* ring, unsigned char* line, uint32_t K, int stride) {
+    const uint64_t buckets = (uint64_t)K * stride;
+    const size_t lsz = line_bytes(stride);
+    for (uint64_t i = (uint64_t)blockIdx.x * blockDim.x + threadIdx.x; i < buckets; i += (uint64_t)gridDim.x * blockDim.x) {
+        BucketHot* hot = reinterpret_cast<BucketHot*>(line + (i / stride) * lsz + line_hot_off());
+        store_hot(hot + i % stride, ring[i].start, ring[i].c[SG_EV_PASS], ring[i].c[SG_EV_WAITING]);
+    }
+}
+
+__global__ void __launch_bounds__(256) k_init_state(Bucket* ring, unsigned char* line, uint32_t K, int stride,
                                                     const int32_t* src_map, const Bucket* old_ring,
-                                                    const Occ* old_occ, int old_stride) {
+                                                    const unsigned char* old_line, int old_stride) {
+    const size_t lsz = line_bytes(stride), old_lsz = line_bytes(old_stride);
     const uint64_t total = (uint64_t)K * stride;
     for (uint64_t i = (uint64_t)blockIdx.x * blockDim.x + threadIdx.x; i < total; i += (uint64_t)gridDim.x * blockDim.x) {
         const uint32_t k = (uint32_t)(i / stride);
@@ -1973,16 +1978,18 @@
         ring[i] = b;
         if (q == 0) {
             Occ o;
-            if (src >= 0) o = old_occ[src];
+            if (src >= 0) o = *reinterpret_cast<const Occ*>(old_line + (size_t)src * old_lsz + line_occ_off());
             else o.pass = o.pass_req = 0;
-            occ[k] = o;
-        }
-    }
-}
-
-__global__ void __launch_bounds__(256) k_snapshot(const Rule* rules, const Bucket* ring, const Occ* occ, uint32_t K,
-                                                  int stride, int64_t now, double* out) {
+            *reinterpret_cast<Occ*>(line + (size_t)k * lsz + line_occ_off()) = o;
+        }
+    }
+}
+
+__global__ void __launch_bounds__(256) k_snapshot(const Rule* rules, const Bucket* ring, const unsigned char* line,
+                                                  uint32_t K, int stride, int64_t now, double* out) {
+    const size_t lsz = line_bytes(stride);
     for (uint32_t k = blockIdx.x * blockDim.x + threadIdx.x; k < K; k += gridDim.x * blockDim.x) {
+        const Occ* occ = reinterpret_cast<const Occ*>(line + (size_t)k * lsz + line_occ_off());
         const Rule R = rules[k];
         const Bucket* rg = ring + (size_t)k * stride;
         const int64_t P = now / R.wl;
@@ -1995,8 +2002,8 @@
                 if (s0 == ws) {
                     pass += rg[q].c[SG_EV_PASS];
                     block += rg[q].c[SG_EV_BLOCK];
-                } else if (s0 != INT64_MIN && s0 < ws && occ[k].pass_req > 0) {
-                    pass += occ[k].pass;
+                } else if (s0 != INT64_MIN && s0 < ws && occ->pass_req > 0) {
+                    pass += occ->pass;
                 }
                 continue;
             }
@@ -2224,24 +2231,26 @@
     return hipGetLastError();
 }
 
-hipError_t launch_hot_sync(const Bucket* ring, BucketHot* hot, uint64_t buckets, hipStream_t stream) {
-    if (buckets == 0) return hipSuccess;
-    hipLaunchKernelGGL(k_hot_sync, dim3(grid_for(buckets, 256, 8192)), dim3(256), 0, stream, ring, hot, buckets);
+hipError_t launch_hot_sync(const Bucket* ring, unsigned char* line, uint32_t K, int stride, hipStream_t stream) {
+    if (K == 0) return hipSuccess;
+    hipLaunchKernelGGL(k_hot_sync, dim3(grid_for((uint64_t)K * stride, 256, 8192)), dim3(256), 0, stream, ring, line, K,
+                       stride);
     return hipGetLastError();
 }
 
-hipError_t launch_init_state(Bucket* ring, Occ* occ, uint32_t K, int stride, const int32_t* src_map,
-                             const Bucket* old_ring, const Occ* old_occ, int old_stride, hipStream_t stream) {
+hipError_t launch_init_state(Bucket* ring, unsigned char* line, uint32_t K, int stride, const int32_t* src_map,
+                             const Bucket* old_ring, const unsigned char* old_line, int old_stride,
+                             hipStream_t stream) {
     if (K == 0) return hipSuccess;
-    hipLaunchKernelGGL(k_init_state, dim3(grid_for((uint64_t)K * stride, 256, 8192)), dim3(256), 0, stream, ring, occ,
-                       K, stride, src_map, old_ring, old_occ, old_stride);
+    hipLaunchKernelGGL(k_init_state, dim3(grid_for((uint64_t)K * stride, 256, 8192)), dim3(256), 0, stream, ring, line,
+                       K, stride, src_map, old_ring, old_line, old_stride);
     return hipGetLastError();
 }
 
-hipError_t launch_snapshot(const Rule* rules, const Bucket* ring, const Occ* occ, uint32_t K, int stride,
+hipError_t launch_snapshot(const Rule* rules, const Bucket* ring, const unsigned char* line, uint32_t K, int stride,
                            int64_t now, double* out, hipStream_t stream) {
     if (K == 0) return hipSuccess;
-    hipLaunchKernelGGL(k_snapshot, dim3(grid_for(K, 256, 4096)), dim3(256), 0, stream, rules, ring, occ, K, stride,
+    hipLaunchKernelGGL(k_snapshot, dim3(grid_for(K, 256, 4096)), dim3(256), 0, stream, rules, ring, line, K, stride,
                        now, out);
     return hipGetLastError();
 }
diff --git a/sentinel_amd/csrc/flowline.h b/sentinel_amd/csrc/flowline.h
--- /dev/null
+++ b/sentinel_amd/csrc/flowline.h
@@ -0,0 +1,38 @@
+#pragma once
+
+#include <stddef.h>
+
+#ifdef __HIPCC__
+#define SG_HD __host__ __device__
+#else
+#define SG_HD
+#endif
+
+namespace sg {
+
+constexpr size_t kLineAlign = 128;
+constexpr size_t kLineOccBytes = 16;
+constexpr size_t kLineRuleBytes = 32;
+constexpr size_t kLineHotBytes = 16;
+SG_HD constexpr size_t line_occ_off() { return 0; }
+SG_HD constexpr size_t line_rule_off() { return line_occ_off() + kLineOccBytes; }
+SG_HD constexpr size_t line_hot_off() { return line_rule_off() + kLineRuleBytes; }
+SG_HD constexpr size_t line_bytes(int stride) {
+    return (line_hot_off() + kLineHotBytes * (size_t)stride + kLineAlign - 1) / kLineAlign * kLineAlign;
+}
+static_assert(line_rule_off() == 16 && line_hot_off() == 48, "walker line: Occ, Rule, BucketHot[stride]");
+static_assert(line_bytes(1) == 128 && line_bytes(5) == 128 && line_bytes(6) == 256 && line_bytes(10) == 256 &&
+                  line_bytes(13) == 256 && line_bytes(14) == 384,
+              "walker line size");
+
+struct LineCopy {
+    size_t off, pitch, width, rows;
+};
+SG_HD constexpr LineCopy line_copy_occ(int stride, size_t K) {
+    return LineCopy{line_occ_off(), line_bytes(stride), kLineOccBytes, K};
+}
+SG_HD constexpr LineCopy line_copy_rule(int stride, size_t K) {
+    return LineCopy{line_rule_off(), line_bytes(stride), kLineRuleBytes, K};
+}
+
+}
diff --git a/sentinel_amd/csrc/local.hip b/sentinel_amd/csrc/local.hip
--- a/sentinel_amd/csrc/local.hip
+++ b/sentinel_amd/csrc/local.hip
@@ -1195,7 +1195,8 @@
     if (ls != 0xFF && !emb_lim_try_pass(a.lim_ring + ls, t, a.lim_qps[ls])) return SG_STATUS_TOO_MANY_REQUEST;
     const Rule R = a.c3_rules[key];
     Bucket* ring = a.c3_ring + (size_t)key * a.c3_stride;
-    const Occ o = a.c3_occ[key];
+    unsigned char* line = a.c3_line + (size_t)key * a.c3_line_sz;
+    const Occ o = *reinterpret_cast<const Occ*>(line + line_occ_off());
     int64_t occ_pass = o.pass, occ_req = o.pass_req;
     const int64_t P = t / R.wl;
     const int S = R.S;
@@ -1258,12 +1259,12 @@
     }
     ring[I].start = ws;
     for (int e = 0; e < SG_NUM_EVENTS; ++e) ring[I].c[e] = cur[e];
-    store_hot(a.c3_hot + (size_t)key * a.c3_stride + I, ws, cur[SG_EV_PASS], cur[SG_EV_WAITING]);
+    store_hot(reinterpret_cast<BucketHot*>(line + line_hot_off()) + I, ws, cur[SG_EV_PASS], cur[SG_EV_WAITING]);
     if (occ_pass != o.pass || occ_req != o.pass_req) {
         Occ no;
         no.pass = occ_pass;
         no.pass_req = occ_req;
-        a.c3_occ[key] = no;
+        *reinterpret_cast<Occ*>(line + line_occ_off()) = no;
     }
     return st;
 }
```

Result: slower. 23.30 billion decisions/s (-5.4%).
